# xujiabo/SCREAM

Measured on AMD Instinct MI355X. Metric: registration pairs/sec, higher is better.
Workload: dtype f32; 1 GPU; BASELINE configs[1]: synthetic 3DMatch_test-like pairs, voxel 0.0625 m, ~5k points/cloud, batch-of-pairs=32 per GPU, A1-A10 per pair (forward 6+6 layers d_model 256, 1-NN thresh 0.1, Kabsch, RE/TE), random-init weights seed 0; lanes=1, steps_in_flight=2, parallelism=dp1 (pairs sharded, metric-row all-gather), rccl_ranks=1, gemm_backend=h2

## Files before the change

include/scream_hip.h:

```cpp
#ifndef SCREAM_HIP_H
#define SCREAM_HIP_H

#include <stdint.h>

#ifdef __cplusplus
extern "C" {
#endif

#define SCREAM_ROW_TILE 128
#define SCREAM_D_MODEL 256
#define SCREAM_NHEAD 8
#define SCREAM_HEAD_DIM 32
#define SCREAM_KV_CHUNK 256

#define SCREAM_EINVAL (-1)
#define SCREAM_EUNSUPPORTED (-2)

enum {
    SCREAM_EPI_NONE = 0,
    SCREAM_EPI_ELU1 = 1,
    SCREAM_EPI_RELU = 2,
    SCREAM_EPI_BIAS_RELU = 3,
    SCREAM_EPI_RES_LN = 4,
    SCREAM_EPI_QKV = 5
};

#define SCREAM_LAYOUT_A_FRAG 1
#define SCREAM_LAYOUT_C_FRAG 2
int scream_act_layout(const float* src, float* dst, int64_t M, int32_t to_fragment, void* stream);

const char* scream_version(void);
int scream_abi_version(void);

int scream_gemm_f32(const float* A, int64_t lda, const float* W, float* C, int64_t ldc,
                    int64_t M, int32_t N, int32_t K, int32_t epilogue, int32_t n_act,
                    const float* bias, const float* residual, int64_t ldr,
                    const float* gamma, const float* beta, void* stream);

int scream_gemm_qkv_f32(const float* A, int64_t lda, const float* W, float* Q, int64_t ldq, int64_t M,
                        int32_t N, int32_t K, int32_t n_q, const int32_t* tile_cloud,
                        const int32_t* cloud_row0, const int32_t* cloud_len, int64_t row_base,
                        float* kv_partial, void* stream);
int scream_kv_finalize(const float* kv_partial, const int32_t* cloud_row0, const int32_t* cloud_len,
                       int64_t row_base, int32_t cloud_begin, int32_t n_kv, float* kv_out, void* stream);

#define SCREAM_SPLIT_H1 1
#define SCREAM_SPLIT_H2 2
#define SCREAM_SPLIT_BF3 3
int scream_pack_w_split(const float* W, int32_t N, int32_t K, int32_t split, int32_t w_exp, void* W_packed,
                        void* stream);
int scream_gemm_split_f32(const float* A, int64_t lda, const void* W_packed, float* C, int64_t ldc, int64_t M,
                          int32_t N, int32_t K, int32_t epilogue, int32_t n_act, const float* bias,
                          const float* residual, int64_t ldr, const float* gamma, const float* beta,
                          int32_t layout, int32_t split, int32_t a_exp, int32_t w_exp, void* stream);
int scream_gemm_qkv_split_f32(const float* A, int64_t lda, const void* W_packed, float* Q, int64_t ldq,
                              int64_t M, int32_t N, int32_t K, int32_t n_q, const int32_t* tile_cloud,
                              const int32_t* cloud_row0, const int32_t* cloud_len, int64_t row_base,
                              float* kv_partial, int32_t layout, int32_t split, int32_t a_exp, int32_t w_exp,
                              int32_t k_exp, int32_t v_exp, void* stream);

int64_t scream_proj_image_bytes(int32_t N, int32_t split);
int scream_pack_proj(const float* W, int32_t N, int32_t n_q, int32_t split, int32_t w_exp, void* proj_image, void* stream);
int scream_proj_qkv_f32(const float* x, const void* proj_image, float* Q, int64_t M, int32_t N, int32_t n_q,
                        const int32_t* tile_cloud, const int32_t* cloud_row0, const int32_t* cloud_len,
                        int64_t row_base, float* kv_partial, int32_t split, int32_t a_exp, int32_t w_exp, int32_t k_exp,
                        int32_t v_exp, void* stream);

typedef struct {
    int32_t e_att, e_wm, e_m1, e_w1, e_h, e_w2;
    int32_t e_y, e_wq;
    int32_t e_x;
    int32_t e_q;
} scream_tail_exps_t;
int64_t scream_tail_image_bytes(int32_t split, int32_t with_next_q);
int64_t scream_kv_image_bytes(void);
int scream_pack_tail(const float* Wm, const float* W1, const float* W2, const float* Wq_next, int32_t q_first, int32_t split,
                     const scream_tail_exps_t* exps, void* tail_image, void* stream);
int scream_kv_finalize_image(const float* kv_partial, const int32_t* cloud_row0, const int32_t* cloud_len,
                          int64_t row_base, int32_t cloud_begin, int32_t n_kv, void* kv_image, int32_t n_layers,
                          int64_t partial_layer_stride, int64_t image_layer_stride, int32_t split, void* stream);
int scream_layer_tail_f32(const float* Q, const void* kv_image, const int32_t* tile_cloud,
                          int32_t kv_cloud_offset, const int32_t* cloud_len, const float* x,
                          const void* tail_image, const float* g1, const float* b1, const float* g2,
                          const float* b2, float* y, float* q_next, int64_t M, int32_t split,
                          const scream_tail_exps_t* exps, void* stream);

int scream_pe_embed_ln(const float* xyz, const int32_t* tile_cloud, const float* center,
                       const float* dim_t, const float* emb_w, const float* emb_b,
                       const float* gamma, const float* beta, float* feats, int64_t rows,
                       void* stream);
int scream_pe_embed_ln_frag(const float* xyz, const int32_t* tile_cloud, const float* center,
                            const float* dim_t, const float* emb_w, const float* emb_b,
                            const float* gamma, const float* beta, float* feats, int64_t rows,
                            void* stream);

int scream_kv_reduce(const float* Kf, const float* Vf, int64_t ld, int64_t row_base,
                     const int32_t* cloud_row0, const int32_t* cloud_len, int32_t cloud_begin,
                     int32_t n_kv, int32_t max_chunks, float* partial, float* kv_out, void* stream);

int scream_attn_apply(const float* Qf, int64_t ldq, const float* kv, const int32_t* tile_cloud,
                      int32_t kv_cloud_offset, const int32_t* cloud_len, float* out, int64_t ldo,
                      int64_t rows, void* stream);

int scream_coor_head(const float* X, const float* W, const float* b, float* out, int64_t rows,
                     void* stream);

typedef struct {
    const float* wqkv;
    const float* wq;
    const float* wkv;
    const float* wm;
    const float* w1;
    const float* w2;
    const float* g1; const float* b1;
    const float* g2; const float* b2;
    const void* tail;
    int32_t e_xq, e_xkv, e_wqkv, e_wq, e_wkv, e_wm_g, e_w1_g, e_w2_g;
    int32_t e_k, e_v;
    scream_tail_exps_t tail_exps;
    int32_t tail_next_q;
    const void* proj;
    int32_t tail_q_first;
    const void* proj_kv;
} scream_layer_t;

typedef struct {
    int32_t n_self;
    int32_t n_cross;
    const float* dim_t;
    const float* emb_w; const float* emb_b;
    const float* pre_g; const float* pre_b;
    const scream_layer_t* layers_host;
    const float* c0_w; const float* c0_b;
    const float* c2_w; const float* c2_b;
    const float* c4_w; const float* c4_b;
    const scream_layer_t* stem_tgt_layers_host;
    int32_t gemm_split;
    int32_t e_c0x, e_c0w, e_c2x, e_c2w;
    const float* wkv_cross;
    int32_t e_wkv_cross, e_k_cross, e_v_cross;
    const void* proj_cross;
} scream_model_t;

typedef struct {
    int32_t n_pairs;
    int64_t rows_src;
    int64_t rows_total;
    int32_t max_chunks;
    const float* xyz;
    const float* center;
    const int32_t* tile_cloud;
    const int32_t* cloud_row0;
    const int32_t* cloud_len;
} scream_batch_t;

int64_t scream_forward_workspace_bytes(int64_t rows_src, int64_t rows_total, int32_t n_pairs,
                                       int32_t max_chunks, int32_t fused_tail, int32_t n_cross_batched);

int scream_forward(const scream_model_t* model, const scream_batch_t* batch, void* workspace,
                   int64_t workspace_bytes, float* src_pred, float* feats_out, void* trace,
                   void* stream);

void* scream_trace_create(int32_t capacity);
void scream_trace_destroy(void* trace);
int scream_trace_reset(void* trace);
int scream_trace_read(void* trace, int32_t max_records, float* ms, int32_t* kind, int64_t* m,
                      int32_t* n, int32_t* k);
int scream_trace_read_starts(void* trace, int32_t max_records, float* start_ms);

int scream_nn_search(const float* query, const float* ref, const int32_t* q_row0,
                     const int32_t* q_len, const int32_t* r_row0, const int32_t* r_len,
                     const float* s, int32_t n_pairs, int32_t max_q_len, int32_t max_r_len,
                     int64_t q_rows_total, int64_t r_rows_total, float thresh, float* ref_prep,
                     uint64_t* keys, int32_t* idx, float* dmin, uint8_t* valid, void* stream);

int scream_square_distance(const float* src, const float* dst, float* out, int32_t B, int32_t N,
                           int32_t M, void* stream);

int scream_kabsch_corr(const float* src, const float* ref, const int32_t* src_row0,
                       const int32_t* src_len, const int32_t* ref_row0, const int32_t* idx,
                       const uint8_t* valid, const float* s, const float* c, int32_t n_pairs,
                       float* T_out, int32_t* n_corr, void* stream);

int scream_rigid_transform_3d(const float* A, const float* B, const float* w,
                              float weight_threshold, int32_t bs, int32_t K, float* T_out,
                              void* stream);

int scream_transformation_error(const float* T_pred, const float* T_gt, int32_t n, float* re,
                                float* te, void* stream);

int scream_point_loss(const float* src_pred, const float* src, const int32_t* src_row0, const int32_t* src_len,
                      const float* rot, const float* trans, int32_t n_pairs, float* loss, void* stream);

int64_t scream_icp_workspace_bytes(int64_t src_rows_total, int64_t ref_rows_total, int32_t n_pairs);
int scream_icp_p2p_range(const float* src, const float* ref, const int32_t* src_row0, const int32_t* src_len,
                         const int32_t* ref_row0, const int32_t* ref_len, const float* s, const float* c,
                         int32_t n_pairs, int32_t max_src_len, int32_t max_ref_len, int64_t src_rows_total,
                         int64_t ref_rows_total, float max_corr_dist, int32_t max_iter, float rel_fitness,
                         float rel_rmse, float* T, float* fitness_rmse, int32_t* iters, int32_t it_begin, int32_t it_end,
                         int32_t* done_flags, void* workspace, int64_t workspace_bytes, void* stream);
int scream_icp_p2p(const float* src, const float* ref, const int32_t* src_row0, const int32_t* src_len,
                   const int32_t* ref_row0, const int32_t* ref_len, const float* s, const float* c,
                   int32_t n_pairs, int32_t max_src_len, int32_t max_ref_len, int64_t src_rows_total,
                   int64_t ref_rows_total, float max_corr_dist, int32_t max_iter, float rel_fitness,
                   float rel_rmse, float* T, float* fitness_rmse, int32_t* iters, void* workspace,
                   int64_t workspace_bytes, void* stream);

int64_t scream_wgrad_workspace_bytes(int64_t rows, int32_t N, int32_t K);
int scream_gemm_wgrad_f32(const float* dY, int64_t ldy, const float* X, int64_t ldx, int64_t rows, int32_t N,
                          int32_t K, float* dW, int32_t accumulate, float* colsum, void* workspace,
                          int64_t workspace_bytes, void* stream);
int64_t scream_wgrad_split_workspace_bytes(int64_t rows, int32_t N, int32_t K);
int scream_gemm_wgrad_split_f32(const float* dY, int64_t ldy, const float* X, int64_t ldx, int64_t rows, int32_t N,
                                int32_t K, float* dW, int32_t accumulate, float* colsum, int32_t split, void* workspace,
                                int64_t workspace_bytes, void* stream);
int scream_ln_fwd(const float* a, const float* b, const float* gamma, const float* beta, float* y, float* mean,
                  float* rstd, int64_t rows, void* stream);
int64_t scream_ln_bwd_workspace_bytes(int64_t rows);
int scream_ln_bwd(const float* dy, const float* a, const float* b, const float* mean, const float* rstd,
                  const float* gamma, float* dz, float* dsum, float* dgamma, float* dbeta, int32_t accumulate,
                  int64_t rows, void* workspace, int64_t workspace_bytes, void* stream);
int64_t scream_attn_bwd_workspace_bytes(int32_t n_q_clouds, int32_t max_chunks);
int scream_attn_bwd(const float* Qf, int64_t ldq, int64_t q_rows, int64_t q_row_base, const float* O,
                    const float* dO, const float* Kf, const float* Vf, int64_t ldkv, int64_t kv_rows,
                    int64_t kv_row_base, const float* kv, const int32_t* tile_cloud, const int32_t* cloud_row0,
                    const int32_t* cloud_len, int32_t q_cloud_begin, int32_t n_q_clouds, int32_t kv_cloud_offset,
                    int32_t max_chunks, float* dq, int64_t lddq, float* dk, float* dv, int64_t lddkv,
                    void* workspace, int64_t workspace_bytes, void* stream);
int scream_relu_bwd(float* dy, const float* y, int64_t n, void* stream);
int scream_add_f32(float* y, const float* x, int64_t n, void* stream);
int scream_transpose_f32(const float* in, int32_t R, int32_t C, float* out, void* stream);
int scream_coor_head_bwd(const float* dout, const float* W, const float* H, float* dH, int64_t rows, void* stream);
int64_t scream_grad3_workspace_bytes(int64_t rows);
int scream_grad3(const float* w, const float* s, const float* center, const int32_t* tile_cloud, int64_t rows,
                 float* dW, int32_t transpose_w, float* col_w, float* col_s, int32_t accumulate, void* workspace,
                 int64_t workspace_bytes, void* stream);
int scream_pe_embed(const float* xyz, const int32_t* tile_cloud, const float* center, const float* dim_t,
                    const float* emb_w, const float* emb_b, float* z, int64_t rows, void* stream);

int64_t scream_render_workspace_bytes(int32_t n_pairs, int32_t n_views, int32_t w, int64_t src_rows_total);
int scream_render_depth(const float* src, const int32_t* s_row0, const int32_t* s_len, const float* tgt,
                        const int32_t* t_row0, const int32_t* t_len, int32_t n_pairs, int32_t max_s_len, int32_t max_t_len,
                        int64_t src_rows_total, const float* rot, int32_t n_views, int32_t w, float rho, float* imgs,
                        int32_t* argmax, void* workspace, int64_t workspace_bytes, void* stream);
int scream_render_depth_bwd(const float* src, const int32_t* s_row0, const int32_t* s_len, int32_t n_pairs, int32_t max_s_len,
                            int64_t src_rows_total, const float* rot, int32_t n_views, int32_t w, float rho,
                            const float* dimgs, const int32_t* argmax, void* workspace, int64_t workspace_bytes, float* dsrc,
                            void* stream);

#ifdef __cplusplus
}
#endif
#endif
```

scream_amd/_lib.py:

```python
from __future__ import annotations

import ctypes as C
import os
from typing import Optional

_HERE = os.path.dirname(os.path.abspath(__file__))
LIB_PATH = os.environ.get("SCREAM_LIB") or os.path.join(_HERE, "libscream_hip.so")
ABI_VERSION = 19

c_f32p = C.POINTER(C.c_float)
c_i32p = C.POINTER(C.c_int32)
c_u8p = C.POINTER(C.c_uint8)
c_u64p = C.POINTER(C.c_uint64)


SPLIT_H1, SPLIT_H2, SPLIT_BF3 = 1, 2, 3


class TailExpsT(C.Structure):
    _fields_ = [(n, C.c_int32) for n in ("e_att", "e_wm", "e_m1", "e_w1", "e_h", "e_w2", "e_y", "e_wq", "e_x", "e_q")]


class LayerT(C.Structure):
    _fields_ = ([(n, C.c_void_p) for n in ("wqkv", "wq", "wkv", "wm", "w1", "w2", "g1", "b1", "g2", "b2", "tail")] +
                [(n, C.c_int32) for n in ("e_xq", "e_xkv", "e_wqkv", "e_wq", "e_wkv", "e_wm_g", "e_w1_g", "e_w2_g", "e_k", "e_v")] +
                [("tail_exps", TailExpsT), ("tail_next_q", C.c_int32), ("proj", C.c_void_p), ("tail_q_first", C.c_int32), ("proj_kv", C.c_void_p)])


class ModelT(C.Structure):
    _fields_ = [("n_self", C.c_int32), ("n_cross", C.c_int32), ("dim_t", C.c_void_p), ("emb_w", C.c_void_p),
                ("emb_b", C.c_void_p), ("pre_g", C.c_void_p), ("pre_b", C.c_void_p),
                ("layers_host", C.POINTER(LayerT)), ("c0_w", C.c_void_p), ("c0_b", C.c_void_p),
                ("c2_w", C.c_void_p), ("c2_b", C.c_void_p), ("c4_w", C.c_void_p), ("c4_b", C.c_void_p),
                ("stem_tgt_layers_host", C.POINTER(LayerT)), ("gemm_split", C.c_int32),
                ("e_c0x", C.c_int32), ("e_c0w", C.c_int32), ("e_c2x", C.c_int32), ("e_c2w", C.c_int32),
                ("wkv_cross", C.c_void_p), ("e_wkv_cross", C.c_int32), ("e_k_cross", C.c_int32), ("e_v_cross", C.c_int32),
                ("proj_cross", C.c_void_p)]


class BatchT(C.Structure):
    _fields_ = [("n_pairs", C.c_int32), ("rows_src", C.c_int64), ("rows_total", C.c_int64),
                ("max_chunks", C.c_int32), ("xyz", C.c_void_p), ("center", C.c_void_p),
                ("tile_cloud", C.c_void_p), ("cloud_row0", C.c_void_p), ("cloud_len", C.c_void_p)]


V, I32, I64, F32 = C.c_void_p, C.c_int32, C.c_int64, C.c_float
SIGNATURES = {
    "scream_version": (C.c_char_p, []),
    "scream_abi_version": (C.c_int, []),
    "scream_gemm_f32": (C.c_int, [V, I64, V, V, I64, I64, I32, I32, I32, I32, V, V, I64, V, V, V]),
    "scream_gemm_qkv_f32": (C.c_int, [V, I64, V, V, I64, I64, I32, I32, I32, V, V, V, I64, V, V]),
    "scream_kv_finalize": (C.c_int, [V, V, V, I64, I32, I32, V, V]),
    "scream_pack_w_split": (C.c_int, [V, I32, I32, I32, I32, V, V]),
    "scream_gemm_split_f32": (C.c_int, [V, I64, V, V, I64, I64, I32, I32, I32, I32, V, V, I64, V, V, I32, I32, I32, I32, V]),
    "scream_gemm_qkv_split_f32": (C.c_int, [V, I64, V, V, I64, I64, I32, I32, I32, V, V, V, I64, V, I32, I32, I32, I32, I32, I32, V]),
    "scream_proj_image_bytes": (C.c_int64, [I32, I32]),
    "scream_pack_proj": (C.c_int, [V, I32, I32, I32, I32, V, V]),
    "scream_proj_qkv_f32": (C.c_int, [V, V, V, I64, I32, I32, V, V, V, I64, V, I32, I32, I32, I32, I32, V]),
    "scream_tail_image_bytes": (C.c_int64, [I32, I32]),
    "scream_kv_image_bytes": (C.c_int64, []),
    "scream_pack_tail": (C.c_int, [V, V, V, V, I32, I32, C.POINTER(TailExpsT), V, V]),
    "scream_kv_finalize_image": (C.c_int, [V, V, V, I64, I32, I32, V, I32, I64, I64, I32, V]),
    "scream_layer_tail_f32": (C.c_int, [V, V, V, I32, V, V, V, V, V, V, V, V, V, I64, I32, C.POINTER(TailExpsT), V]),
    "scream_act_layout": (C.c_int, [V, V, I64, I32, V]),
    "scream_pe_embed_ln": (C.c_int, [V, V, V, V, V, V, V, V, V, I64, V]),
    "scream_pe_embed_ln_frag": (C.c_int, [V, V, V, V, V, V, V, V, V, I64, V]),
    "scream_kv_reduce": (C.c_int, [V, V, I64, I64, V, V, I32, I32, I32, V, V, V]),
    "scream_attn_apply": (C.c_int, [V, I64, V, V, I32, V, V, I64, I64, V]),
    "scream_coor_head": (C.c_int, [V, V, V, V, I64, V]),
    "scream_forward_workspace_bytes": (C.c_int64, [I64, I64, I32, I32, I32, I32]),
    "scream_forward": (C.c_int, [C.POINTER(ModelT), C.POINTER(BatchT), V, I64, V, V, V, V]),
    "scream_trace_create": (C.c_void_p, [I32]),
    "scream_trace_destroy": (None, [V]),
    "scream_trace_reset": (C.c_int, [V]),
    "scream_trace_read": (C.c_int, [V, I32, V, V, V, V, V]),
    "scream_trace_read_starts": (C.c_int, [V, I32, V]),
    "scream_nn_search": (C.c_int, [V, V, V, V, V, V, V, I32, I32, I32, I64, I64, F32, V, V, V, V, V, V]),
    "scream_square_distance": (C.c_int, [V, V, V, I32, I32, I32, V]),
    "scream_kabsch_corr": (C.c_int, [V, V, V, V, V, V, V, V, V, I32, V, V, V]),
    "scream_rigid_transform_3d": (C.c_int, [V, V, V, F32, I32, I32, V, V]),
    "scream_transformation_error": (C.c_int, [V, V, I32, V, V, V]),
    "scream_point_loss": (C.c_int, [V, V, V, V, V, V, I32, V, V]),
    "scream_icp_workspace_bytes": (C.c_int64, [I64, I64, I32]),
    "scream_icp_p2p": (C.c_int, [V, V, V, V, V, V, V, V, I32, I32, I32, I64, I64, F32, I32, F32, F32, V, V, V, V, I64, V]),
    "scream_wgrad_workspace_bytes": (C.c_int64, [I64, I32, I32]),
    "scream_gemm_wgrad_f32": (C.c_int, [V, I64, V, I64, I64, I32, I32, V, I32, V, V, I64, V]),
    "scream_wgrad_split_workspace_bytes": (C.c_int64, [I64, I32, I32]),
    "scream_gemm_wgrad_split_f32": (C.c_int, [V, I64, V, I64, I64, I32, I32, V, I32, V, I32, V, I64, V]),
    "scream_ln_fwd": (C.c_int, [V, V, V, V, V, V, V, I64, V]),
    "scream_ln_bwd_workspace_bytes": (C.c_int64, [I64]),
    "scream_ln_bwd": (C.c_int, [V, V, V, V, V, V, V, V, V, V, I32, I64, V, I64, V]),
    "scream_attn_bwd_workspace_bytes": (C.c_int64, [I32, I32]),
    "scream_attn_bwd": (C.c_int, [V, I64, I64, I64, V, V, V, V, I64, I64, I64, V, V, V, V, I32, I32, I32, I32, V, I64, V, V, I64,
                                  V, I64, V]),
    "scream_relu_bwd": (C.c_int, [V, V, I64, V]),
    "scream_add_f32": (C.c_int, [V, V, I64, V]),
    "scream_transpose_f32": (C.c_int, [V, I32, I32, V, V]),
    "scream_coor_head_bwd": (C.c_int, [V, V, V, V, I64, V]),
    "scream_grad3_workspace_bytes": (C.c_int64, [I64]),
    "scream_grad3": (C.c_int, [V, V, V, V, I64, V, I32, V, V, I32, V, I64, V]),
    "scream_pe_embed": (C.c_int, [V, V, V, V, V, V, V, I64, V]),
    "scream_icp_p2p_range": (C.c_int, [V, V, V, V, V, V, V, V, I32, I32, I32, I64, I64, F32, I32, F32, F32, V, V, V, I32, I32, V, V, I64, V]),
    "scream_render_workspace_bytes": (C.c_int64, [I32, I32, I32, I64]),
    "scream_render_depth": (C.c_int, [V, V, V, V, V, V, I32, I32, I32, I64, V, I32, I32, F32, V, V, V, I64, V]),
    "scream_render_depth_bwd": (C.c_int, [V, V, V, I32, I32, I64, V, I32, I32, F32, V, V, V, I64, V, V]),
}

_lib: Optional[C.CDLL] = None


class ScreamHipError(RuntimeError):
    pass


def load() -> C.CDLL:
    global _lib
    if _lib is not None:
        return _lib
    if os.environ.get("SCREAM_NO_BUILD", "0") != "1" and not os.environ.get("SCREAM_LIB"):
        try:
            from . import build as _build
            _build.build()
        except Exception as e:
            if not os.path.exists(LIB_PATH):
                raise ScreamHipError("libscream_hip.so is missing and could not be built: %s" % e) from e
    if not os.path.exists(LIB_PATH):
        raise ScreamHipError("libscream_hip.so not found at %s (run `python -m scream_amd.build`)" % LIB_PATH)
    lib = C.CDLL(LIB_PATH)
    for name, (res, args) in SIGNATURES.items():
        try:
            fn = getattr(lib, name)
        except AttributeError as e:
            raise ScreamHipError("libscream_hip.so does not export %s" % name) from e
        fn.restype = res
        fn.argtypes = args
    if lib.scream_abi_version() != ABI_VERSION:
        raise ScreamHipError("libscream_hip.so ABI %d != binding ABI %d" % (lib.scream_abi_version(), ABI_VERSION))
    _lib = lib
    return lib


def check(rc: int, what: str) -> None:
    if rc == 0:
        return
    if rc == -1:
        raise ScreamHipError("%s: invalid argument (SCREAM_EINVAL)" % what)
    if rc == -2:
        raise ScreamHipError("%s: unsupported shape (SCREAM_EUNSUPPORTED)" % what)
    raise ScreamHipError("%s: HIP error %d" % (what, rc))
```

scream_amd/build.py:

```python
from __future__ import annotations

import os
import shutil
import subprocess
import sys
from concurrent.futures import ThreadPoolExecutor

HERE = os.path.dirname(os.path.abspath(__file__))
CSRC = os.path.join(HERE, "csrc")
LIB = os.path.join(HERE, "libscream_hip.so")
ARCH = "gfx950"

SOURCES = {
    "gemm_f32.hip": [],
    "gemm_split.hip": [],
    "proj_ring.hip": ["-mllvm", "-amdgpu-mfma-vgpr-form=1"],
    "tail_split.hip": ["-ffp-contract=off"],
    "embed.hip": [],
    "attention.hip": [],
    "backward.hip": [],
    "forward.hip": [],
    "nn_search.hip": ["-ffp-contract=off"],
    "kabsch.hip": ["-ffp-contract=off"],
    "icp_grid.hip": ["-ffp-contract=off"],
    "render.hip": ["-ffp-contract=off"],
}
EXTRA_DEFINES = {}
for _item in filter(None, os.environ.get("SCREAM_HIPCC_EXTRA", "").split(";")):
    EXTRA_DEFINES[_item.split(":")[0]] = _item.split(":", 1)[1].split(",")
ASM_LOADS = ("gemm_split.hip", "tail_split.hip", "proj_ring.hip")
NO_SCRATCH = {"proj_ring.hip": ("proj_ring_kernel",), "tail_split.hip": ("tail_kernelINS_7SplitH2", "tail_kernelINS_7SplitH1")}


def _hipcc() -> str:
    exe = shutil.which("hipcc") or "/opt/rocm/bin/hipcc"
    if not os.path.exists(exe):
        raise RuntimeError("hipcc not found: cannot build libscream_hip.so")
    return exe


def _stale() -> bool:
    if not os.path.exists(LIB):
        return True
    t = os.path.getmtime(LIB)
    deps = [os.path.join(CSRC, f) for f in os.listdir(CSRC)] + [os.path.join(HERE, "..", "include", "scream_hip.h"), __file__]
    return any(os.path.getmtime(d) > t for d in deps)


def build(force: bool = False, verbose: bool = False, out: str = None) -> str:
    global LIB
    if out:
        LIB, force = out, True
    if not force and not _stale():
        return LIB
    hipcc = _hipcc()
    objdir = os.path.join(HERE, "build")
    os.makedirs(objdir, exist_ok=True)
    common = [hipcc, "-O3", "-std=c++17", "--offload-arch=" + ARCH, "-fPIC", "-Wall", "-Wno-unused-function"]

    def compile_one(item):
        src, extra = item
        extra = extra + EXTRA_DEFINES.get(src, [])
        obj = os.path.join(objdir, src.replace(".hip", ".o"))
        cmd = common + extra + ["-c", os.path.join(CSRC, src), "-o", obj]
        r = subprocess.run(cmd, capture_output=True, text=True)
        if r.returncode != 0:
            raise RuntimeError("hipcc failed for %s:\n%s\n%s" % (src, " ".join(cmd), r.stderr))
        if verbose and r.stderr.strip():
            print(r.stderr, file=sys.stderr)
        return obj

    def verify_one(src):
        sys.path.insert(0, os.path.join(HERE, "..", "tools"))
        import asm_inflight_check as chk
        asm = os.path.join(objdir, src.replace(".hip", ".s"))
        cmd = common + SOURCES[src] + EXTRA_DEFINES.get(src, []) + ["-S", "--cuda-device-only", os.path.join(CSRC, src), "-o", asm]
        r = subprocess.run(cmd, capture_output=True, text=True)
        if r.returncode != 0:
            raise RuntimeError("hipcc -S failed for %s:\n%s" % (src, r.stderr))
        for name, body in chk.kernels(asm):
            if any(k in name for k in NO_SCRATCH.get(src, ())) and any(("scratch_" in l or "buffer_store" in l) for l in body):
                raise RuntimeError("%s: %s spills registers to scratch (this hipcc allocates registers differently from the one the "
                                   "kernel was written with)" % (src, name))
            bad = chk.check_kernel(name, body)
            if bad:
                raise RuntimeError("%s: %s touches a register whose asm load is still in flight (%d places, first: %s); "
                                   "this hipcc allocates registers differently from the one the kernels were written with"
                                   % (src, name, len(bad), bad[0][1]))
            sd = chk.check_store_data_hazard(name, body)
            if sd:
                raise RuntimeError("%s: %s overwrites the data of a wide store %d wait states behind it (%s ; %s)"
                                   % (src, name, sd[0][3], sd[0][1], sd[0][2]))
            mh = chk.check_mfma_asm_read_hazard(name, body)
            if mh:
                raise RuntimeError("%s: %s reads a matrix-instruction result with an asm vector instruction %d wait states behind it "
                                   "(%s ; %s)" % (src, name, mh[0][3], mh[0][2], mh[0][1]))
            hz = chk.check_scalar_base_hazard(name, body)
            if hz:
                raise RuntimeError("%s: %s uses a scalar base %d wait states after a VALU write of it (%s -> %s)"
                                   % (src, name, hz[0][3], hz[0][2], hz[0][1]))
        return src

    with ThreadPoolExecutor(max_workers=4) as ex:
        checks = [ex.submit(verify_one, src) for src in ASM_LOADS] if os.environ.get("SCREAM_BUILD_VERIFY", "1") != "0" else []
        objs = list(ex.map(compile_one, SOURCES.items()))
        for c in checks:
            c.result()
    cmd = [hipcc, "--offload-arch=" + ARCH, "-shared", "-fPIC", "-o", LIB + ".tmp"] + objs
    r = subprocess.run(cmd, capture_output=True, text=True)
    if r.returncode != 0:
        raise RuntimeError("link failed:\n%s" % r.stderr)
    os.replace(LIB + ".tmp", LIB)
    return LIB


if __name__ == "__main__":
    print(build(force="--force" in sys.argv, verbose=True))
```

scream_amd/csrc/forward.hip:

```cpp
#include <vector>

#include "common.h"

namespace {

constexpr int D = SCREAM_D_MODEL;
constexpr int KV_ELEMS = (SCREAM_HEAD_DIM + 1) * SCREAM_HEAD_DIM;

struct Workspace {
    float *x0, *x1, *q, *att, *m1, *hid, *kvp, *kv;
    char* kvimg;
    float* kvp_cross;
    char* kvimg_cross;
    int64_t kvp_cross_stride, kvimg_cross_stride;
    int64_t bytes;
};

Workspace carve(void* base, int64_t rows_src, int64_t rows_total, int32_t n_pairs, int32_t max_chunks, bool fused, int32_t n_cross_batched) {
    Workspace w;
    float* p = reinterpret_cast<float*>(base);
    auto take = [&](int64_t n) {
        float* r = p;
        p += (n + 63) / 64 * 64;
        return r;
    };
    w.x0 = take(rows_total * D);
    w.x1 = take(rows_total * D);
    w.q = take(rows_total * D);
    w.att = fused ? nullptr : take(rows_total * D);
    w.m1 = fused ? nullptr : take(rows_total * D);
    w.hid = fused ? nullptr : take(rows_total * 4 * D);
    w.kvp = take(rows_total / SCREAM_ROW_TILE * SCREAM_NHEAD * KV_ELEMS);
    w.kv = take((int64_t)2 * n_pairs * SCREAM_NHEAD * KV_ELEMS);
    w.kvimg = reinterpret_cast<char*>(take((int64_t)2 * n_pairs * scream_kv_image_bytes() / 4));
    w.kvp_cross_stride = (rows_total - rows_src) / SCREAM_ROW_TILE * SCREAM_NHEAD * KV_ELEMS;
    w.kvimg_cross_stride = (int64_t)n_pairs * scream_kv_image_bytes();
    w.kvp_cross = take(n_cross_batched * w.kvp_cross_stride);
    w.kvimg_cross = reinterpret_cast<char*>(take(n_cross_batched * w.kvimg_cross_stride / 4));
    w.bytes = (p - reinterpret_cast<float*>(base)) * (int64_t)sizeof(float);
    return w;
}

struct Trace {
    std::vector<hipEvent_t> ev;
    std::vector<int32_t> kind, n, k;
    std::vector<int64_t> m;
    int count = 0;
    int capacity = 0;
};

struct Scope {
    Trace* t;
    int slot = -1;
    hipStream_t st;
    Scope(Trace* t_, int kind, int64_t m, int n, int k, void* stream) : t(t_), st(as_stream(stream)) {
        if (!t || t->count >= t->capacity) return;
        slot = t->count++;
        t->kind[slot] = kind;
        t->m[slot] = m;
        t->n[slot] = n;
        t->k[slot] = k;
        (void)hipEventRecord(t->ev[2 * slot], st);
    }
    ~Scope() {
        if (slot >= 0) (void)hipEventRecord(t->ev[2 * slot + 1], st);
    }
};

#define TRY(call)                 \
    do {                          \
        int rc_ = (call);         \
        if (rc_ != 0) return rc_; \
    } while (0)

enum { TR_TAIL_FUSED = 7, TR_EMBED = 100, TR_KV_REDUCE = 101, TR_ATTN_APPLY = 102, TR_COOR_HEAD = 103 };

struct Ctx {
    void* st;
    Trace* tr;
    int split;
    bool frag;
};

int gemm(const Ctx& c, const float* A, int64_t lda, const float* W, float* C, int64_t ldc, int64_t M, int N, int K,
         int epi, int n_act, const float* bias, const float* res, const float* g, const float* b, int a_exp, int w_exp,
         int layout = 0) {
    Scope sc(c.tr, epi, M, N, K, c.st);
    if (c.split)
        return scream_gemm_split_f32(A, lda, W, C, ldc, M, N, K, epi, n_act, bias, res, D, g, b, layout, c.split, a_exp, w_exp, c.st);
    return scream_gemm_f32(A, lda, W, C, ldc, M, N, K, epi, n_act, bias, res, D, g, b, c.st);
}

int gemm_qkv(const Ctx& c, const float* A, const float* W, const void* proj, float* Q, int64_t M, int N, int n_q, const scream_batch_t& b,
             int64_t row_base, float* kvp, int a_exp, int w_exp, int k_exp, int v_exp) {
    Scope sc(c.tr, 5, M, N, D, c.st);
    if (proj && c.frag && (c.split == SCREAM_SPLIT_H2 || c.split == SCREAM_SPLIT_H1))
        return scream_proj_qkv_f32(A, proj, Q, M, N, n_q, b.tile_cloud, b.cloud_row0, b.cloud_len, row_base, kvp, c.split, a_exp, w_exp,
                                   k_exp, v_exp, c.st);
    if (c.split)
        return scream_gemm_qkv_split_f32(A, D, W, Q, D, M, N, D, n_q, b.tile_cloud, b.cloud_row0, b.cloud_len, row_base, kvp,
                                         c.frag ? (SCREAM_LAYOUT_A_FRAG | (n_q ? SCREAM_LAYOUT_C_FRAG : 0)) : 0, c.split, a_exp,
                                         w_exp, k_exp, v_exp, c.st);
    return scream_gemm_qkv_f32(A, D, W, Q, D, M, N, D, n_q, b.tile_cloud, b.cloud_row0, b.cloud_len, row_base, kvp, c.st);
}

int mha_tail(const Ctx& c, const scream_layer_t& L, const Workspace& w, const float* x, float* y, int64_t row0,
             int64_t rows) {
    float* att = w.att + row0 * D;
    float* m1 = w.m1 + row0 * D;
    float* hid = w.hid + row0 * 4 * D;
    const scream_tail_exps_t& e = L.tail_exps;
    TRY(gemm(c, att, D, L.wm, m1, D, rows, D, D, SCREAM_EPI_RES_LN, 0, nullptr, x, L.g1, L.b1, e.e_att, L.e_wm_g));
    TRY(gemm(c, m1, D, L.w1, hid, 4 * D, rows, 4 * D, D, SCREAM_EPI_RELU, 0, nullptr, nullptr, nullptr, nullptr, e.e_m1, L.e_w1_g));
    TRY(gemm(c, hid, 4 * D, L.w2, y, D, rows, D, 4 * D, SCREAM_EPI_RES_LN, 0, nullptr, x, L.g2, L.b2, e.e_h, L.e_w2_g));
    return 0;
}

int mha_self(const Ctx& c, const scream_layer_t& L, const scream_batch_t& b, const Workspace& w, const float* x,
             float* y, int64_t row0, int64_t rows, int32_t cloud_begin, int32_t n_clouds, bool next_q = false) {
    const float* xr = x + row0 * D;
    float* qr = w.q + row0 * D;
    float* kvp = w.kvp + row0 / SCREAM_ROW_TILE * SCREAM_NHEAD * KV_ELEMS;
    const bool qf = c.frag && L.tail_q_first;
    if (qf) TRY(gemm_qkv(c, xr, L.wkv, L.proj_kv, nullptr, rows, 2 * D, 0, b, row0, kvp, L.e_xkv, L.e_wkv, L.e_k, L.e_v));
    else TRY(gemm_qkv(c, xr, L.wqkv, L.proj, qr, rows, 3 * D, D, b, row0, kvp, L.e_xq, L.e_wqkv, L.e_k, L.e_v));
    if (c.frag) {
        {
            Scope sc(c.tr, TR_KV_REDUCE, rows, 0, 0, c.st);
            TRY(scream_kv_finalize_image(kvp, b.cloud_row0, b.cloud_len, row0, cloud_begin, n_clouds, w.kvimg, 1, 0, 0, c.split, c.st));
        }
        Scope sc(c.tr, TR_TAIL_FUSED, rows, ((next_q || qf) ? 10 : 9) * D, D, c.st);
        return scream_layer_tail_f32(qf ? nullptr : qr, w.kvimg, b.tile_cloud + row0 / SCREAM_ROW_TILE, 0, b.cloud_len, xr, L.tail, L.g1,
                                     L.b1, L.g2, L.b2, y + row0 * D, (next_q && !qf) ? qr : nullptr, rows, c.split, &L.tail_exps, c.st);
    }
    {
        Scope sc(c.tr, TR_KV_REDUCE, rows, 0, 0, c.st);
        TRY(scream_kv_finalize(kvp, b.cloud_row0, b.cloud_len, row0, cloud_begin, n_clouds, w.kv, c.st));
    }
    {
        Scope sc(c.tr, TR_ATTN_APPLY, rows, 0, 0, c.st);
        TRY(scream_attn_apply(qr, D, w.kv, b.tile_cloud + row0 / SCREAM_ROW_TILE, 0, b.cloud_len, w.att + row0 * D, D, rows,
                              c.st));
    }
    return mha_tail(c, L, w, xr, y + row0 * D, row0, rows);
}

int cross_kv_all(const Ctx& c, const scream_model_t& m, const scream_batch_t& b, const Workspace& w, const float* x_tgt) {
    const int64_t rs = b.rows_src, rt = b.rows_total - b.rows_src;
    const scream_layer_t& L0 = m.layers_host[m.n_self + 1];
    TRY(gemm_qkv(c, x_tgt, m.wkv_cross, m.proj_cross, nullptr, rt, 2 * D * m.n_cross, 0, b, rs, w.kvp_cross, L0.e_xkv, m.e_wkv_cross, m.e_k_cross,
                 m.e_v_cross));
    Scope sc(c.tr, TR_KV_REDUCE, rt, 0, 0, c.st);
    return scream_kv_finalize_image(w.kvp_cross, b.cloud_row0, b.cloud_len, rs, b.n_pairs, b.n_pairs,
                                 w.kvimg_cross - (int64_t)b.n_pairs * scream_kv_image_bytes(), m.n_cross, w.kvp_cross_stride,
                                 w.kvimg_cross_stride, c.split, c.st);
}

int mha_cross(const Ctx& c, const scream_layer_t& L, const scream_batch_t& b, const Workspace& w, const float* x_src,
              const float* x_tgt, float* y, const char* kvimg_layer, bool q_ready = false) {
    const int64_t rs = b.rows_src, rt = b.rows_total - b.rows_src;
    const bool qf = c.frag && L.tail_q_first;
    if (!q_ready && !qf)
        TRY(gemm(c, x_src, D, L.wq, w.q, D, rs, D, D, SCREAM_EPI_ELU1, D, nullptr, nullptr, nullptr, nullptr, L.e_xq, L.e_wq,
                 c.frag ? (SCREAM_LAYOUT_A_FRAG | SCREAM_LAYOUT_C_FRAG) : 0));
    if (c.frag && kvimg_layer) {
        Scope sc(c.tr, TR_TAIL_FUSED, rs, (qf ? 10 : 9) * D, D, c.st);
        return scream_layer_tail_f32(qf ? nullptr : w.q, kvimg_layer, b.tile_cloud, 0, b.cloud_len + b.n_pairs, x_src, L.tail, L.g1, L.b1, L.g2,
                                     L.b2, y, nullptr, rs, c.split, &L.tail_exps, c.st);
    }
    TRY(gemm_qkv(c, x_tgt, L.wkv, nullptr, nullptr, rt, 2 * D, 0, b, rs, w.kvp, L.e_xkv, L.e_wkv, L.e_k, L.e_v));
    if (c.frag) {
        {
            Scope sc(c.tr, TR_KV_REDUCE, rt, 0, 0, c.st);
            TRY(scream_kv_finalize_image(w.kvp, b.cloud_row0, b.cloud_len, rs, b.n_pairs, b.n_pairs, w.kvimg, 1, 0, 0, c.split, c.st));
        }
        Scope sc(c.tr, TR_TAIL_FUSED, rs, (qf ? 10 : 9) * D, D, c.st);
        return scream_layer_tail_f32(qf ? nullptr : w.q, w.kvimg, b.tile_cloud, b.n_pairs, b.cloud_len, x_src, L.tail, L.g1, L.b1, L.g2, L.b2,
                                     y, nullptr, rs, c.split, &L.tail_exps, c.st);
    }
    {
        Scope sc(c.tr, TR_KV_REDUCE, rt, 0, 0, c.st);
        TRY(scream_kv_finalize(w.kvp, b.cloud_row0, b.cloud_len, rs, b.n_pairs, b.n_pairs, w.kv, c.st));
    }
    {
        Scope sc(c.tr, TR_ATTN_APPLY, rs, 0, 0, c.st);
        TRY(scream_attn_apply(w.q, D, w.kv, b.tile_cloud, b.n_pairs, b.cloud_len, w.att, D, rs, c.st));
    }
    return mha_tail(c, L, w, x_src, y, 0, rs);
}

}

extern "C" const char* scream_version(void) { return "scream_hip gfx950 abi19"; }
extern "C" int scream_abi_version(void) { return 19; }

extern "C" void* scream_trace_create(int32_t capacity) {
    if (capacity <= 0) return nullptr;
    Trace* t = new Trace();
    t->capacity = capacity;
    t->ev.resize(2 * (size_t)capacity);
    t->kind.resize(capacity);
    t->n.resize(capacity);
    t->k.resize(capacity);
    t->m.resize(capacity);
    for (auto& e : t->ev) {
        if (hipEventCreate(&e) != hipSuccess) {
            delete t;
            return nullptr;
        }
    }
    return t;
}

extern "C" void scream_trace_destroy(void* trace) {
    Trace* t = reinterpret_cast<Trace*>(trace);
    if (!t) return;
    for (auto& e : t->ev) (void)hipEventDestroy(e);
    delete t;
}

extern "C" int scream_trace_reset(void* trace) {
    SCREAM_REQUIRE(trace, SCREAM_EINVAL);
    reinterpret_cast<Trace*>(trace)->count = 0;
    return 0;
}

extern "C" int scream_trace_read(void* trace, int32_t max_records, float* ms, int32_t* kind, int64_t* m, int32_t* n,
                                 int32_t* k) {
    SCREAM_REQUIRE(trace && ms && kind && m && n && k && max_records >= 0, SCREAM_EINVAL);
    Trace* t = reinterpret_cast<Trace*>(trace);
    const int cnt = t->count < max_records ? t->count : max_records;
    for (int i = 0; i < cnt; ++i) {
        if (hipEventElapsedTime(&ms[i], t->ev[2 * i], t->ev[2 * i + 1]) != hipSuccess) return SCREAM_EINVAL;
        kind[i] = t->kind[i];
        m[i] = t->m[i];
        n[i] = t->n[i];
        k[i] = t->k[i];
    }
    return cnt;
}

extern "C" int scream_trace_read_starts(void* trace, int32_t max_records, float* start_ms) {
    SCREAM_REQUIRE(trace && start_ms && max_records >= 0, SCREAM_EINVAL);
    Trace* t = reinterpret_cast<Trace*>(trace);
    const int cnt = t->count < max_records ? t->count : max_records;
    for (int i = 0; i < cnt; ++i)
        if (hipEventElapsedTime(&start_ms[i], t->ev[0], t->ev[2 * i]) != hipSuccess) return SCREAM_EINVAL;
    return cnt;
}

extern "C" int64_t scream_forward_workspace_bytes(int64_t rows_src, int64_t rows_total, int32_t n_pairs,
                                                  int32_t max_chunks, int32_t fused_tail, int32_t n_cross_batched) {
    if (rows_src < 0 || rows_total < rows_src || n_pairs < 0 || max_chunks < 0 || n_cross_batched < 0) return SCREAM_EINVAL;
    return carve(nullptr, rows_src, rows_total, n_pairs, max_chunks, fused_tail != 0, n_cross_batched).bytes + 256;
}

extern "C" int scream_forward(const scream_model_t* model, const scream_batch_t* batch, void* workspace,
                              int64_t workspace_bytes, float* src_pred, float* feats_out, void* trace, void* stream) {
    SCREAM_REQUIRE(model && batch && workspace && src_pred, SCREAM_EINVAL);
    const scream_model_t& m = *model;
    const scream_batch_t& b = *batch;
    SCREAM_REQUIRE(m.layers_host && m.n_self >= 0 && m.n_cross >= 0 &&
                       (m.gemm_split == 0 || m.gemm_split == SCREAM_SPLIT_H1 || m.gemm_split == SCREAM_SPLIT_H2 || m.gemm_split == SCREAM_SPLIT_BF3),
                   SCREAM_EINVAL);
    SCREAM_REQUIRE(b.n_pairs > 0 && b.rows_src > 0 && b.rows_total > b.rows_src && b.max_chunks > 0, SCREAM_EINVAL);
    SCREAM_REQUIRE(b.rows_src % SCREAM_ROW_TILE == 0 && b.rows_total % SCREAM_ROW_TILE == 0, SCREAM_EUNSUPPORTED);
    SCREAM_REQUIRE(b.xyz && b.center && b.tile_cloud && b.cloud_row0 && b.cloud_len, SCREAM_EINVAL);
    int n_layers = m.n_self + 2 * m.n_cross, n_tail = 0;
    for (int i = 0; i < n_layers; ++i) n_tail += m.layers_host[i].tail != nullptr;
    if (m.stem_tgt_layers_host)
        for (int i = 0; i < m.n_self; ++i, ++n_layers) n_tail += m.stem_tgt_layers_host[i].tail != nullptr;
    SCREAM_REQUIRE(n_tail == 0 || (n_tail == n_layers && m.gemm_split != 0), SCREAM_EINVAL);
    uintptr_t base = (reinterpret_cast<uintptr_t>(workspace) + 255) & ~(uintptr_t)255;
    const bool batched_kv = n_tail > 0 && m.wkv_cross != nullptr && m.n_cross > 0;
    const Workspace w = carve(reinterpret_cast<void*>(base), b.rows_src, b.rows_total, b.n_pairs, b.max_chunks, n_tail > 0,
                              batched_kv ? m.n_cross : 0);
    SCREAM_REQUIRE((int64_t)(base - reinterpret_cast<uintptr_t>(workspace)) + w.bytes <= workspace_bytes, SCREAM_EINVAL);
    const Ctx c{stream, reinterpret_cast<Trace*>(trace), m.gemm_split, n_tail > 0};

    const int64_t rs = b.rows_src, ra = b.rows_total;
    {
        Scope sc(c.tr, TR_EMBED, ra, 0, 0, stream);
        if (c.frag)
            TRY(scream_pe_embed_ln_frag(b.xyz, b.tile_cloud, b.center, m.dim_t, m.emb_w, m.emb_b, m.pre_g, m.pre_b, w.x0, ra, stream));
        else
            TRY(scream_pe_embed_ln(b.xyz, b.tile_cloud, b.center, m.dim_t, m.emb_w, m.emb_b, m.pre_g, m.pre_b, w.x0, ra, stream));
    }
    float* cur = w.x0;
    float* nxt = w.x1;
    for (int i = 0; i < m.n_self; ++i) {
        if (!m.stem_tgt_layers_host) {
            TRY(mha_self(c, m.layers_host[i], b, w, cur, nxt, 0, ra, 0, 2 * b.n_pairs));
        } else {
            TRY(mha_self(c, m.layers_host[i], b, w, cur, nxt, 0, rs, 0, b.n_pairs));
            TRY(mha_self(c, m.stem_tgt_layers_host[i], b, w, cur, nxt, rs, ra - rs, b.n_pairs, b.n_pairs));
        }
        float* t = cur;
        cur = nxt;
        nxt = t;
    }
    const float* x_tgt = cur + rs * D;
    if (batched_kv) TRY(cross_kv_all(c, m, b, w, x_tgt));
    for (int i = 0; i < 2 * m.n_cross; ++i) {
        const scream_layer_t& L = m.layers_host[m.n_self + i];
        if (i % 2 == 0) {
            TRY(mha_self(c, L, b, w, cur, nxt, 0, rs, 0, b.n_pairs, c.frag && L.tail_next_q));
        } else {
            const bool q_ready = c.frag && m.layers_host[m.n_self + i - 1].tail_next_q;
            TRY(mha_cross(c, L, b, w, cur, x_tgt, nxt, batched_kv ? w.kvimg_cross + (i / 2) * w.kvimg_cross_stride : nullptr, q_ready));
        }
        float* t = cur;
        cur = nxt;
        nxt = t;
    }
    float* c_mid = c.frag ? w.q : w.m1;
    float* c_out = c.frag ? nxt : w.att;
    TRY(gemm(c, cur, D, m.c0_w, c_mid, D, rs, D, D, SCREAM_EPI_BIAS_RELU, 0, m.c0_b, nullptr, nullptr, nullptr, m.e_c0x, m.e_c0w,
             c.frag ? SCREAM_LAYOUT_A_FRAG : 0));
    TRY(gemm(c, c_mid, D, m.c2_w, c_out, D, rs, D, D, SCREAM_EPI_BIAS_RELU, 0, m.c2_b, nullptr, nullptr, nullptr, m.e_c2x, m.e_c2w));
    {
        Scope sc(c.tr, TR_COOR_HEAD, rs, 0, 0, stream);
        TRY(scream_coor_head(c_out, m.c4_w, m.c4_b, src_pred, rs, stream));
    }
    if (feats_out && c.frag) {
        TRY(scream_act_layout(cur, feats_out, rs, 0, stream));
    } else if (feats_out) {
        hipError_t e = hipMemcpyAsync(feats_out, cur, (size_t)rs * D * sizeof(float), hipMemcpyDeviceToDevice,
                                      as_stream(stream));
        if (e != hipSuccess) return (int)e;
    }
    return 0;
}
```

scream_amd/csrc/tail_split.hip:

```cpp
#include <type_traits>

#include "ring.h"

#ifndef T_MIX
#define T_MIX 1
#endif
#ifndef T_RIDE0
#define T_RIDE0 3
#endif
#ifndef T_STASH
#define T_STASH 3
#endif
#ifndef T_NT
#define T_NT 7
#endif
#ifndef T_QF_DUMP
#define T_QF_DUMP 0
#endif
#ifndef T_QF_DBG
#define T_QF_DBG 0
#endif
#ifndef T_DEFER_H2
#define T_DEFER_H2 2
#endif

#ifdef T_STAMPS
#define T_STAMP_SLOTS 24
__device__ long long t_stamps[256 * 4 * T_STAMP_SLOTS];
extern "C" int scream_tail_stamps_read(long long* host) {
    return (int)hipMemcpyFromSymbol(host, HIP_SYMBOL(t_stamps), sizeof(long long) * 256 * 4 * T_STAMP_SLOTS);
}
#define TSTAMP(slot)                                                                                 \
    do {                                                                                             \
        if (stamp_on && lane == 0) t_stamps[((int)blockIdx.x * 4 + wave) * T_STAMP_SLOTS + (slot)] = __builtin_amdgcn_s_memtime(); \
    } while (0)
#define TMARK(i) marks[i] = (unsigned)__builtin_amdgcn_s_memtime()
#define TMARK2(i, prev) do { marks[prev] = marks[i]; TMARK(i); } while (0)
#define TMARKS_FLUSH()                                                                               \
    do {                                                                                             \
        if (stamp_on && lane == 0)                                                                   \
            for (int i_ = 0; i_ < 16; ++i_) t_stamps[((int)blockIdx.x * 4 + wave) * T_STAMP_SLOTS + 8 + i_] = marks[i_]; \
    } while (0)
#else
#define TSTAMP(slot) do {} while (0)
#define TMARK(i) do {} while (0)
#define TMARK2(i, prev) do {} while (0)
#define TMARKS_FLUSH() do {} while (0)
#endif

namespace {

constexpr int TAIL_STAGES = 72;
constexpr int NEXT_Q_STAGES = 8;
constexpr int KV_PLANES_BYTES = 8 * 3 * 2 * 1024;
constexpr int KV_IMAGE_BYTES = KV_PLANES_BYTES + 8 * 32 * 4;

constexpr int KV_H2_HEAD_BYTES = 2 * 2 * 1024;
constexpr int KV_H2_SCALE_OFF = 8 * KV_H2_HEAD_BYTES;
#ifndef T_APPLY_H2
#define T_APPLY_H2 1
#endif

struct HeadOps {
    f32x4 kv[6];
    f32x4 ks[4];
    f32x4 sc;
};

struct TailScales {
    float s_att;
    int e_q;
    int e_att;
    float c1;
    float eps1;
    float s_m1;
    float ch;
    float c2;
    float eps2;
    float s_y;
    float cq;
    float s_x;
    float cqf;
};

__device__ __forceinline__ constexpr int xadd_slot(int h, int g, int nd) {
    int n = 0;
    for (int c = 15 - nd; c >= 8; --c) {
        if ((c >> 1) == h - 1) continue;
        if (c == g) return n < 4 ? n : -1;
        ++n;
    }
    return -1;
}

template <class SP, bool NQ, bool QF>
__global__ __launch_bounds__(TT, 1) void tail_kernel(const float* __restrict__ Q,
                                                     const char* __restrict__ kvimg,
                                                     const int32_t* __restrict__ tile_cloud, int kv_cloud_offset,
                                                     const int32_t* __restrict__ cloud_len,
                                                     const float* __restrict__ xres,
                                                     const char* __restrict__ Wimg,
                                                     const float* __restrict__ g1, const float* __restrict__ b1,
                                                     const float* __restrict__ g2, const float* __restrict__ b2,
                                                     float* __restrict__ y,
                                                     float* q_next,
                                                     int n_tiles, TailScales sc) {
    static_assert(!NQ || SP::SCALED, "the next-layer query projection is built for the fp16 splits");
    static_assert(!QF || (SP::SCALED && !NQ), "the in-kernel query projection is built for the fp16 splits and replaces the next-layer one");
    constexpr int N_STAGES = TAIL_STAGES + ((NQ || QF) ? NEXT_Q_STAGES : 0);
    typedef typename SP::vec V;
    constexpr int NP = SP::NP;
    constexpr int STAGE = stage_bytes<SP>();
    constexpr int PIECES = wave_pieces<SP>();
    constexpr bool APPLY_H2 = SP::SCALED && T_APPLY_H2;
#ifdef T_NV_MERGE
    constexpr int NV_MERGE = T_NV_MERGE;
#else
    constexpr int NV_MERGE = SP::NPROD >= 6 ? 6 : 8;
#endif
    constexpr int ND = SP::NPROD >= 6 ? 1 : T_DEFER_H2;
    constexpr int NG = 16 - ND;
    constexpr int NSTASH = (NP == 2 && !QF) ? T_STASH : 0;
    __shared__ __attribute__((aligned(16))) char smem[T_SLOTS * STAGE + 4096 + NSTASH * 16384];
    const int tid = threadIdx.x, lane = tid & 63;
    const int wave = __builtin_amdgcn_readfirstlane(tid >> 6);
    const int half = lane >> 5;
    float* lnp = reinterpret_cast<float*>(smem + T_SLOTS * STAGE);
    f32x4* stash = reinterpret_cast<f32x4*>(smem + T_SLOTS * STAGE + 4096 + wave * (NSTASH * 4096)) + lane;
    lnp[tid] = SP::SCALED ? g1[tid] * sc.s_m1 : g1[tid];
    lnp[256 + tid] = SP::SCALED ? b1[tid] * sc.s_m1 : b1[tid];
    lnp[512 + tid] = g2[tid];
    lnp[768 + tid] = b2[tid];
    const float eps1 = SP::SCALED ? sc.eps1 : 1e-5f, eps2 = SP::SCALED ? sc.eps2 : 1e-5f;
    const unsigned v_lane16 = lane * 16, v_half16 = half * 16;
    auto dma_piece = [&](unsigned q, int u) {
        if ((T_ABLATE & 1) && q >= 2) return;
        const unsigned src = q % (unsigned)N_STAGES, slot = q % (unsigned)T_SLOTS;
        const char* sbase = Wimg + (size_t)src * STAGE + (wave * PIECES + (u & ~3)) * 1024;
        dma_1k(sbase + v_lane16, smem + slot * STAGE + (wave * PIECES + (u & ~3)) * 1024, u & 3);
    };
    unsigned q = 0;
#pragma unroll
    for (int u = 0; u < PIECES; ++u) dma_piece(0, u);
#pragma unroll
    for (int u = 0; u < PIECES; ++u) dma_piece(1, u);

    auto seg_base = [&](const float* base, int64_t grp, int seg) { return base + grp + seg * 1024; };
    auto req_q = [&](f32x4 (&qb)[4], int64_t grp, int h) {
        if (T_ABLATE & (16 | 32)) return;
        if (T_ABLATE & 2048) grp = (int64_t)wave * 32 * SCREAM_D_MODEL;
        ld_asm4<1024, (T_NT & 1) != 0>(qb, seg_base(Q, grp, h), v_lane16);
    };
    auto req_head = [&](HeadOps& o, const char* kvc, int h) {
        if (T_ABLATE & (16 | 256)) return;
        f32x4 (&kv4)[4] = reinterpret_cast<f32x4 (&)[4]>(o.kv[0]);
        if (APPLY_H2) {
            ld_asm4<1024>(kv4, kvc + h * KV_H2_HEAD_BYTES, v_lane16);
            asm volatile("global_load_dwordx4 %0, %1, %2" : "=v"(o.sc) : "v"(v_half16), "s"(kvc + KV_H2_SCALE_OFF + 32 * h));
        } else {
            const char* kp = kvc + h * (3 * 2 * 1024);
            ld_asm4<1024>(kv4, kp, v_lane16);
            ld_asm2k(o.kv[4], o.kv[5], kp + 4 * 1024, v_lane16);
        }
        ld_asm4<32>(o.ks, kvc + KV_PLANES_BYTES + 128 * h, v_half16);
    };
    auto req_x = [&](f32x4 (&xs)[4], int64_t grp, int blk, auto second) {
        if (T_ABLATE & (16 | 64)) return;
        if (T_ABLATE & 2048) grp = (int64_t)wave * 32 * SCREAM_D_MODEL;
        ld_asm4<1024, (T_NT & (decltype(second)::value ? 4 : 8)) != 0>(xs, seg_base(xres, grp, blk), v_lane16);
    };
    auto pin_head = [&](HeadOps& o) {
#pragma unroll
        for (int a = 0; a < 4; ++a) pin(o.ks[a]);
#pragma unroll
        for (int f = 0; f < (APPLY_H2 ? 4 : 6); ++f) pin(o.kv[f]);
        if (APPLY_H2) pin(o.sc);
    };
    auto add_x4 = [&](f32x16& t, const f32x4 (&xs)[4], int a, float c) {
#pragma unroll
        for (int k = 0; k < 4; ++k) {
            const float xv = (T_ABLATE & 16) ? 1.0f : xs[a][k];
            t[4 * a + k] = SP::SCALED ? __builtin_fmaf(xv, c, t[4 * a + k]) : t[4 * a + k] + xv;
        }
    };
    auto pin_x = [&](f32x4 (&xs)[4]) {
#pragma unroll
        for (int a = 0; a < 4; ++a) pin(xs[a]);
    };
    auto add_x = [&](f32x16& t, const f32x4 (&xs)[4], float c) {
#pragma unroll
        for (int a = 0; a < 4; ++a) add_x4(t, xs, a, c);
    };

    HeadOps op;
    f32x4 qA[4], qB[4];
    f32x4 xs[4], xs2[4];
    V apA[2][NP], apB[2][NP];
    f32x16 aT;
    bf16x8 qp[2][3];
    f16x8 qph[2][2];
    float Zs = 0.f;
    int tq = 0;

    auto apply_qscale = [&](const f32x4 (&qb)[4]) {
        float m = 0.f;
#pragma unroll
        for (int a = 0; a < 4; ++a)
#pragma unroll
            for (int k = 0; k < 4; ++k) m = fmaxf(m, qb[a][k]);
        m = fmaxf(m, __shfl_xor(m, 32));
        const int hb = (int)(__float_as_uint(op.sc[0]) >> 23);
        tq = min(max(14 - ((int)(__float_as_uint(m) >> 23) - 127), sc.e_q), min(127, sc.e_att + hb - 1));
    };
    auto apply_qsplit = [&](f32x4 (&qb)[4], int tile_tag, int s2) {
        f32x4 lo = qb[2 * s2], hi = qb[2 * s2 + 1];
        if (T_ABLATE & 16) lo = hi = f32x4{(float)lane, 1.0f, 0.5f, (float)tile_tag};
        if (APPLY_H2) split8s<SplitH2>(lo, hi, __uint_as_float((uint32_t)(tq + 127) << 23), qph[s2]);
        else split8<SplitBf3>(lo, hi, qp[s2]);
    };
    auto apply_mfma = [&](int s2) {
        if (APPLY_H2) {
            f16x8 w[2];
#pragma unroll
            for (int p = 0; p < 2; ++p) w[p] = __builtin_bit_cast(f16x8, op.kv[p * 2 + s2]);
            mfma_group<SplitH2, -1>(aT, w, qph[s2], s2 == 0);
        } else {
            bf16x8 w[3];
#pragma unroll
            for (int p = 0; p < 3; ++p) w[p] = __builtin_bit_cast(bf16x8, op.kv[p * 2 + s2]);
            mfma_group<SplitBf3, -1>(aT, w, qp[s2], s2 == 0);
        }
    };
    auto apply_z = [&](f32x4 (&qb)[4]) {
        float zp = 0.f;
#pragma unroll
        for (int a = 0; a < 4; ++a)
#pragma unroll
            for (int k = 0; k < 4; ++k) zp += qb[a][k] * op.ks[a][k];
        zp += __shfl_xor(zp, 32);
        Zs = 1.0f / (zp + 1e-6f);
        if (APPLY_H2) Zs *= __uint_as_float((uint32_t)(sc.e_att - tq + (int)(__float_as_uint(op.sc[0]) >> 23)) << 23);
        else if (SP::SCALED) Zs *= sc.s_att;
    };
    auto apply_split_pair = [&](int k, V (&ap)[2][NP], float S) {
        const int s2 = k >> 2, j = (2 * k) & 7;
        if constexpr (SP::SCALED && (T_MIX & 2)) {
            SP::split2s((aT[2 * k] * Zs) * S, (aT[2 * k + 1] * Zs) * S, 1.0f, j, ap[s2]);
        } else {
#pragma unroll
            for (int e = 0; e < 2; ++e) SP::split1((aT[2 * k + e] * Zs) * S, j + e, ap[s2]);
        }
    };
    auto apply_ride = [&](f32x4 (&qb)[4], int g, V (&ap)[2][NP], float S, int tile_tag) {
        if (g == 0 && APPLY_H2) apply_qscale(qb);
        if (g == 0) apply_qsplit(qb, tile_tag, 0);
        if (g == 1) apply_qsplit(qb, tile_tag, 1);
        if (g == 1) apply_mfma(0);
        if (g == 2) apply_mfma(1);
        if (g == 3) apply_z(qb);
        if (g >= 4 && g < 12) apply_split_pair(g - 4, ap, S);
    };

    V xp[QF ? 16 : 1][NP];
    f32x4 qall[QF ? 8 : 1][4];
    f32x16 hqf[2];
    auto elu_q = [&](int k, const f32x16& h, f32x4 (&dst)[4]) {
#pragma unroll
        for (int e = 0; e < 2; ++e) {
            const int i = 2 * k + e;
            dst[i >> 2][i & 3] = elu1(h[i] * sc.cqf);
        }
    };

    float dbg6[8] = {0.f, 0.f, 0.f, 0.f, 0.f, 0.f, 0.f, 0.f};
    auto xsum = [&](const V (&ap)[2][NP]) {
        unsigned c = 0;
#pragma unroll
        for (int s2 = 0; s2 < 2; ++s2)
#pragma unroll
            for (int pl = 0; pl < NP; ++pl) {
                const f32x4 w = __builtin_bit_cast(f32x4, ap[s2][pl]);
#pragma unroll
                for (int k = 0; k < 4; ++k) c ^= __builtin_bit_cast(unsigned, w[k]);
            }
        return __builtin_bit_cast(float, (c & 0x007fffffu) | 0x3f800000u);
    };
    auto asum = [&](const f32x16 (&a)[8]) {
        unsigned c = 0;
#pragma unroll
        for (int b = 0; b < 8; ++b)
#pragma unroll
            for (int e = 0; e < 16; ++e) c ^= __builtin_bit_cast(unsigned, a[b][e]);
        return __builtin_bit_cast(float, (c & 0x007fffffu) | 0x3f800000u);
    };
    int tile = blockIdx.x;
    int64_t grp = ((int64_t)tile * 128 + wave * 32) * SCREAM_D_MODEL;
    const char* kvc = nullptr;
    float S = 1.f;
    if (tile < n_tiles) {
        const int cl = tile_cloud[tile] + kv_cloud_offset;
        kvc = kvimg + (size_t)cl * KV_IMAGE_BYTES;
        S = (float)cloud_len[cl];
    }
    if (!QF && tile < n_tiles) {
#pragma unroll
        for (int h = 0; h < 2; ++h) {
            req_q(qA, grp, h);
            req_head(op, kvc, h);
            VM_WAIT(0);
            pin_x(qA);
            pin_head(op);
#pragma unroll
            for (int g = 0; g < 12; ++g) apply_ride(qA, g, h == 0 ? apA : apB, S, tile);
        }
    }

#ifdef T_STAMPS
    int tile_no = 0;
#endif
    while (tile < n_tiles) {
#ifdef T_STAMPS
        const bool stamp_on = tile_no == 1;
        ++tile_no;
        unsigned marks[16] = {};
#endif
        TSTAMP(0);
        V wfd[ND][NP];
        f32x16 acc[8];
        const int tile_next = tile + (int)gridDim.x;
        const bool has_next = tile_next < n_tiles;
        const int64_t grp_next = ((int64_t)(has_next ? tile_next : tile) * 128 + wave * 32) * SCREAM_D_MODEL;
        const char* kvc_next = kvc;
        float S_next = 1.f;
        if (has_next) {
            const int cl = tile_cloud[tile_next] + kv_cloud_offset;
            kvc_next = kvimg + (size_t)cl * KV_IMAGE_BYTES;
            S_next = (float)cloud_len[cl];
        }

        auto stage_merge = [&](auto hh, V (&ap)[2][NP], V (&ap_next)[2][NP], f32x4 (&q_cons)[4], f32x4 (&q_req)[4], auto flush) {
            constexpr int h = decltype(hh)::value;
            constexpr bool RIDE = h >= 1 && h <= 6;
            if (h == 0 && !QF) { if (NQ) ring_barrier<0>(); else lds_only_barrier(); }
            else if (QF && (T_QF_DBG & 32) && h <= 1) ring_barrier<0>();
            else ring_barrier<PIECES>();
            TMARK(h);
            __builtin_amdgcn_sched_barrier(0);
            f32x4 (&x_prev)[4] = (h & 1) ? xs : xs2;
            f32x4 (&x_req)[4] = (h & 1) ? xs2 : xs;
            if (h > 0) {
                pin_x(x_prev);
                if (h - 1 < NSTASH) {
#pragma unroll
                    for (int a = 0; a < 4; ++a) stash[((h - 1) * 4 + a) * 64] = x_prev[a];
                }
                if (RIDE) {
                    pin_head(op);
                    pin_x(q_cons);
                }
            }
            __builtin_amdgcn_sched_barrier(0);
            req_x(x_req, grp, h, std::false_type{});
            if (!QF && h + 2 < 8) req_q(q_req, grp, h + 2);
            if (h == 0) req_head(op, kvc, 2);
            __builtin_amdgcn_sched_barrier(0);
            const char* wb = smem + (q % T_SLOTS) * STAGE + lane * 16;
            V wf[T_PF][NP];
#pragma unroll
            for (int g0 = 0; g0 < T_PF - 1; ++g0)
#pragma unroll
                for (int p = 0; p < NP; ++p) wf[g0][p] = ld_frag<V>(wb + (p * 16 + g0) * 1024);
            flush();
#pragma unroll
            for (int g = 0; g < NG; ++g) {
                if (g + T_PF - 1 < 16) {
#pragma unroll
                    for (int p = 0; p < NP; ++p)
                        (g + T_PF - 1 >= NG ? wfd[g + T_PF - 1 - NG][p] : wf[(g + T_PF - 1) % T_PF][p]) = ld_frag<V>(wb + (p * 16 + g + T_PF - 1) * 1024);
                }
                if (g == 4 && RIDE && h + 2 < 8) {
                    __builtin_amdgcn_sched_barrier(0);
                    req_head(op, kvc, h + 2);
                    __builtin_amdgcn_sched_barrier(0);
                }
                if (g >= 4 && g - 4 < PIECES) dma_piece(q + 2, g - 4);
                if (PIECES == 12 && g == 14) dma_piece(q + 2, 11);
                if (RIDE && !(T_ABLATE & 512)) apply_ride(q_cons, g, ap_next, S, tile);
                if (QF && h == 0 && g < 8) elu_q(g, hqf[1], qall[QF ? 7 : 0]);
                if (h > 0) {
                    const int pc = xadd_slot(h, g, ND);
                    if (pc >= 0 && !(T_ABLATE & 1024)) add_x4(acc[h > 0 ? h - 1 : 0], x_prev, pc, sc.c1);
                }
                mfma_group<SP, (h > 0 ? NV_MERGE : 0)>(acc[g >> 1], wf[g % T_PF], ap[g & 1], h == 0 && (g & 1) == 0);
            }
            ++q;
        };
        constexpr std::integral_constant<bool, true> yes{};
        constexpr std::integral_constant<bool, false> no{};
#define HEAD(n) std::integral_constant<int, n>{}
        auto flush_none = [&]() {};
        auto flush_acc7 = [&](V (&b)[2][NP], bool first) {
#pragma unroll
            for (int i = 0; i < ND; ++i) mfma_group<SP, -1>(acc[7], wfd[i], b[(NG + i) & 1], first && ((NG + i) & 1) == 0);
        };
        auto flush_mergeA = [&]() { flush_acc7(apA, false); };
        auto flush_mergeB = [&]() { flush_acc7(apB, false); };
        auto flush_mergeA0 = [&]() { flush_acc7(apA, true); };
        if constexpr (QF) {
            {
                f32x4 raw[8][4];
                const float* xg = xres + grp + lane * 4;
                if (T_QF_DBG & 256) VM_WAIT(0);
#pragma unroll
                for (int blk = 0; blk < 8; ++blk)
#pragma unroll
                    for (int a = 0; a < 4; ++a) raw[blk][a] = ld4(xg + (blk * 4 + a) * 256);
                VM_WAIT(0);
#pragma unroll
                for (int blk = 0; blk < 8; ++blk)
#pragma unroll
                    for (int s2 = 0; s2 < 2; ++s2) split8s<SP>(raw[blk][2 * s2], raw[blk][2 * s2 + 1], sc.s_x, xp[QF ? 2 * blk + s2 : 0]);
            }
            auto stage_qf = [&](auto jj) {
                constexpr int j = decltype(jj)::value;
                constexpr int RIDE = j >= 6 ? j - 6 : -1;
                constexpr bool RIDE6 = !(T_QF_DBG & (2 | 64)), RIDE7 = !(T_QF_DBG & (2 | 128));
                constexpr bool RIDE_ON = j == 6 ? RIDE6 : RIDE7;
                if (j == 0) { if (T_QF_DBG & 1) ring_barrier<0>(); else lds_only_barrier(); }
                else if ((T_QF_DBG & 8) && j >= 6) ring_barrier<0>();
                else if ((T_QF_DBG & 16) && j >= 1 && j <= 5) ring_barrier<0>();
                else ring_barrier<PIECES>();
                __builtin_amdgcn_sched_barrier(0);
                if (RIDE >= 0 && RIDE_ON) pin_head(op);
                __builtin_amdgcn_sched_barrier(0);
                if (j == 5 && RIDE6) req_head(op, kvc, 0);
                if (j == 6 && !RIDE6 && RIDE7) req_head(op, kvc, 1);
                __builtin_amdgcn_sched_barrier(0);
                const char* wb = smem + (q % T_SLOTS) * STAGE + lane * 16;
                V wf[T_PF][NP];
#pragma unroll
                for (int g0 = 0; g0 < T_PF - 1; ++g0)
#pragma unroll
                    for (int p = 0; p < NP; ++p) wf[g0][p] = ld_frag<V>(wb + (p * 16 + g0) * 1024);
                if (j > 0) {
#pragma unroll
                    for (int i = 0; i < ND; ++i) mfma_group<SP, -1>(hqf[(j + 1) & 1], wfd[i], xp[QF ? NG + i : 0]);
                }
#pragma unroll
                for (int g = 0; g < NG; ++g) {
                    if (g + T_PF - 1 < 16) {
#pragma unroll
                        for (int p = 0; p < NP; ++p)
                            (g + T_PF - 1 >= NG ? wfd[g + T_PF - 1 - NG][p] : wf[(g + T_PF - 1) % T_PF][p]) = ld_frag<V>(wb + (p * 16 + g + T_PF - 1) * 1024);
                    }
                    if (g == 4 && RIDE == 0 && RIDE6 && RIDE7) {
                        __builtin_amdgcn_sched_barrier(0);
                        req_head(op, kvc, 1);
                        __builtin_amdgcn_sched_barrier(0);
                    }
                    if (g >= 4 && g - 4 < PIECES) dma_piece(q + 2, g - 4);
                    if (j > 0 && g < 8) elu_q(g, hqf[(j + 1) & 1], qall[QF && j > 0 ? j - 1 : 0]);
                    if (RIDE >= 0 && RIDE_ON && !(T_ABLATE & 512)) apply_ride(qall[QF && RIDE >= 0 ? RIDE : 0], g, RIDE == 0 ? apA : apB, S, tile);
                    mfma_group<SP, 8>(hqf[j & 1], wf[g % T_PF], xp[QF ? g : 0], g == 0);
                }
                ++q;
            };
            stage_qf(HEAD(0)); stage_qf(HEAD(1)); stage_qf(HEAD(2)); stage_qf(HEAD(3));
            stage_qf(HEAD(4)); stage_qf(HEAD(5)); stage_qf(HEAD(6));
            stage_qf(HEAD(7));
            if (T_QF_DUMP == 6) {
                unsigned c = 0;
#pragma unroll
                for (int h = 0; h < 7; ++h)
#pragma unroll
                    for (int a = 0; a < 4; ++a)
#pragma unroll
                        for (int k = 0; k < 4; ++k) c ^= __builtin_bit_cast(unsigned, qall[QF ? h : 0][a][k]);
                dbg6[4] = __builtin_bit_cast(float, (c & 0x007fffffu) | 0x3f800000u);
            }
            if (T_QF_DBG & (2 | 64 | 128)) {
#pragma unroll
                for (int h = 0; h < 2; ++h) {
                    if (!(T_QF_DBG & 2) && !(T_QF_DBG & (h == 0 ? 64 : 128))) continue;
                    req_head(op, kvc, h);
                    VM_WAIT(0);
                    pin_head(op);
#pragma unroll
                    for (int g = 0; g < 12; ++g) apply_ride(qall[QF ? h : 0], g, h == 0 ? apA : apB, S, tile);
                }
            }
        }
        auto flush_q7 = [&]() {
#pragma unroll
            for (int i = 0; i < ND; ++i) mfma_group<SP, -1>(hqf[1], wfd[i], xp[QF ? NG + i : 0]);
        };
#define QC(h1, q_) qall[QF ? (h1) : 0]
        if constexpr (QF) {
            stage_merge(HEAD(0), apA, apB, QC(1, qB), QC(1, qA), flush_q7);
            stage_merge(HEAD(1), apB, apA, QC(2, qA), QC(2, qB), flush_mergeA0);
            stage_merge(HEAD(2), apA, apB, QC(3, qB), QC(3, qA), flush_mergeB);
            stage_merge(HEAD(3), apB, apA, QC(4, qA), QC(4, qB), flush_mergeA);
            stage_merge(HEAD(4), apA, apB, QC(5, qB), QC(5, qA), flush_mergeB);
            stage_merge(HEAD(5), apB, apA, QC(6, qA), QC(6, qB), flush_mergeA);
            stage_merge(HEAD(6), apA, apB, QC(7, qB), QC(7, qA), flush_mergeB);
            stage_merge(HEAD(7), apB, apA, QC(7, qA), QC(7, qB), flush_mergeA);
        } else {
        stage_merge(HEAD(0), apA, apB, qB, qA, flush_none);
        stage_merge(HEAD(1), apB, apA, qA, qB, flush_mergeA0);
        stage_merge(HEAD(2), apA, apB, qB, qA, flush_mergeB);
        stage_merge(HEAD(3), apB, apA, qA, qB, flush_mergeA);
        stage_merge(HEAD(4), apA, apB, qB, qA, flush_mergeB);
        stage_merge(HEAD(5), apB, apA, qA, qB, flush_mergeA);
        stage_merge(HEAD(6), apA, apB, qB, qA, flush_mergeB);
        stage_merge(HEAD(7), apB, apA, qA, qB, flush_mergeA);
        }
#undef QC
        flush_mergeB();
        vm_wait<PIECES>();
        pin_x(xs2);
        add_x(acc[7], xs2, sc.c1);

        TSTAMP(1);
#if T_QF_DUMP
        if (QF && T_QF_DUMP != 6 && (T_QF_DUMP < 4 || q_next)) {
            float* yd = (T_QF_DUMP < 4 ? y : q_next) + grp + lane * 4;
#pragma unroll
            for (int b = 0; b < 8; ++b)
#pragma unroll
                for (int a = 0; a < 4; ++a) {
                    f32x4 o;
#pragma unroll
                    for (int k = 0; k < 4; ++k) o[k] = (T_QF_DUMP & 1) ? qall[QF ? b : 0][a][k] : acc[b][4 * a + k];
                    *reinterpret_cast<f32x4*>(yd + (b * 4 + a) * 256) = o;
                }
        }
#endif
        V mp[16][NP];
        {
            float sum = 0.f;
#pragma unroll
            for (int b = 0; b < 8; ++b)
#pragma unroll
                for (int e = 0; e < 16; ++e) sum += acc[b][e];
            sum += __shfl_xor(sum, 32);
            const float mean = sum * (1.0f / 256.0f);
            float var = 0.f;
#pragma unroll
            for (int b = 0; b < 8; ++b)
#pragma unroll
                for (int e = 0; e < 16; ++e) {
                    acc[b][e] -= mean;
                    var += acc[b][e] * acc[b][e];
                }
            var += __shfl_xor(var, 32);
            const float rstd = 1.0f / sqrtf(var * (1.0f / 256.0f) + eps1);
            const float* gp = lnp + 4 * half;
            const float* bp = lnp + 256 + 4 * half;
#pragma unroll
            for (int b = 0; b < 8; ++b)
#pragma unroll
                for (int s2 = 0; s2 < 2; ++s2) {
                    f32x4 v[2];
#pragma unroll
                    for (int a2 = 0; a2 < 2; ++a2) {
                        const int a = 2 * s2 + a2;
                        const f32x4 g4 = ld4(gp + 32 * b + 8 * a), b4 = ld4(bp + 32 * b + 8 * a);
#pragma unroll
                        for (int k = 0; k < 4; ++k) v[a2][k] = acc[b][4 * a + k] * rstd * g4[k] + b4[k];
                    }
                    if (T_MIX & 2) split8s<SP>(v[0], v[1], 1.0f, mp[2 * b + s2]); else split8<SP>(v[0], v[1], mp[2 * b + s2]);
                }
        }

        TSTAMP(2);
        if (QF && T_QF_DUMP == 6) {
            unsigned c = 0;
#pragma unroll
            for (int i = 0; i < 16; ++i)
#pragma unroll
                for (int pl = 0; pl < NP; ++pl) {
                    const f32x4 w = __builtin_bit_cast(f32x4, mp[i][pl]);
#pragma unroll
                    for (int k = 0; k < 4; ++k) c ^= __builtin_bit_cast(unsigned, w[k]);
                }
            (void)c;
        }
        f32x16 hT;
        V hpA[2][NP], hpB[2][NP];
        auto split_pair = [&](int k, V (&hout)[2][NP]) {
            const int s2 = k >> 2, j = (2 * k) & 7;
            float x0, x1;
            if (T_MIX & 1) {
                asm("v_max_f32 %0, 0, %1" : "=v"(x0) : "v"(hT[2 * k]));
                asm("v_max_f32 %0, 0, %1" : "=v"(x1) : "v"(hT[2 * k + 1]));
            } else {
                x0 = fmaxf(hT[2 * k], 0.f);
                x1 = fmaxf(hT[2 * k + 1], 0.f);
            }
            if constexpr (SP::SCALED && (T_MIX & 1)) {
                SP::split2s(x0, x1, sc.ch, j, hout[s2]);
            } else if constexpr (SP::SCALED) {
                SP::split1(x0 * sc.ch, j, hout[s2]);
                SP::split1(x1 * sc.ch, j + 1, hout[s2]);
            } else {
                SP::split1(x0, j, hout[s2]);
                SP::split1(x1, j + 1, hout[s2]);
            }
        };
        auto stage_up = [&](auto first, auto xload, auto flush) {
            constexpr int XLOAD = decltype(xload)::value;
            if (decltype(first)::value) ring_barrier<0>(); else ring_barrier<PIECES>();
            TMARK2(8, 10);
            __builtin_amdgcn_sched_barrier(0);
            if (XLOAD >= 0 && XLOAD < NSTASH) {
#pragma unroll
                for (int a = 0; a < 4; ++a) xs[a] = stash[(XLOAD * 4 + a) * 64];
            } else if (XLOAD >= 0) req_x(xs, grp, XLOAD, std::true_type{});
            __builtin_amdgcn_sched_barrier(0);
            const char* wb = smem + (q % T_SLOTS) * STAGE + lane * 16;
            V wf[T_PF][NP];
#pragma unroll
            for (int g0 = 0; g0 < T_PF - 1; ++g0)
#pragma unroll
                for (int p = 0; p < NP; ++p) wf[g0][p] = ld_frag<V>(wb + (p * 16 + g0) * 1024);
            flush();
#pragma unroll
            for (int g = 0; g < NG; ++g) {
                if (g + T_PF - 1 < 16) {
#pragma unroll
                    for (int p = 0; p < NP; ++p)
                        (g + T_PF - 1 >= NG ? wfd[g + T_PF - 1 - NG][p] : wf[(g + T_PF - 1) % T_PF][p]) = ld_frag<V>(wb + (p * 16 + g + T_PF - 1) * 1024);
                }
                if (g < PIECES) dma_piece(q + 2, g);
                mfma_group<SP>(hT, wf[g % T_PF], mp[g], g == 0);
            }
            ++q;
        };
        auto stage_down = [&](V (&hin)[2][NP], V (&hout)[2][NP], auto with_split, auto xadd, auto ride, auto flush) {
            constexpr int XADD = decltype(xadd)::value;
            constexpr int RIDE = decltype(ride)::value;
#ifdef T_PROBE_NOBAR
            __builtin_amdgcn_s_waitcnt(0x0070 | (PIECES & 15) | ((PIECES >> 4) << 14));
#else
            ring_barrier<PIECES>();
#endif
            TMARK2(9, 11);
            __builtin_amdgcn_sched_barrier(0);
            if (XADD == 0) {
                pin_x(xs);
#pragma unroll
                for (int a = 0; a < 4; ++a)
#pragma unroll
                    for (int k = 0; k < 4; ++k) {
                        const float xv = (T_ABLATE & 16) ? 1.0f : xs[a][k];
                        acc[0][4 * a + k] = SP::SCALED ? xv * sc.c2 : xv;
                    }
            } else if (XADD > 0) {
                pin_x(xs);
                add_x(acc[XADD > 0 ? XADD : 0], xs, sc.c2);
            }
            if (RIDE == 2) {
                pin_head(op);
                pin_x(qA);
            }
            __builtin_amdgcn_sched_barrier(0);
            if (RIDE == 1) {
                req_q(qA, grp_next, 0);
                req_head(op, kvc_next, 0);
            }
            __builtin_amdgcn_sched_barrier(0);
            const char* wb = smem + (q % T_SLOTS) * STAGE + lane * 16;
            V wf[T_PF][NP];
#pragma unroll
            for (int g0 = 0; g0 < T_PF - 1; ++g0)
#pragma unroll
                for (int p = 0; p < NP; ++p) wf[g0][p] = ld_frag<V>(wb + (p * 16 + g0) * 1024);
            flush();
#pragma unroll
            for (int g = 0; g < NG; ++g) {
                if (g + T_PF - 1 < 16) {
#pragma unroll
                    for (int p = 0; p < NP; ++p)
                        (g + T_PF - 1 >= NG ? wfd[g + T_PF - 1 - NG][p] : wf[(g + T_PF - 1) % T_PF][p]) = ld_frag<V>(wb + (p * 16 + g + T_PF - 1) * 1024);
                }
                if (RIDE == 2 && g == 4) {
                    __builtin_amdgcn_sched_barrier(0);
                    req_q(qA, grp_next, 1);
                    req_head(op, kvc_next, 1);
                    __builtin_amdgcn_sched_barrier(0);
                }
                if (RIDE == 2) {
                    if (g >= 4 && g - 4 < PIECES) dma_piece(q + 2, g - 4);
                    if (PIECES == 12 && g == 14) dma_piece(q + 2, 11);
                } else {
                    if (g < PIECES) dma_piece(q + 2, g);
                }
                if (RIDE == 2) apply_ride(qA, g, apA, S_next, tile_next);
                if (decltype(with_split)::value && (ND == 1 ? (g & 1) == 0 : (g >= T_RIDE0 && g < T_RIDE0 + 8))) split_pair(ND == 1 ? g >> 1 : g - T_RIDE0, hout);
                mfma_group<SP>(acc[g >> 1], wf[g % T_PF], hin[g & 1], XADD == 0 && g >= 2 && (g & 1) == 0);
            }
            ++q;
        };
        constexpr std::integral_constant<int, -1> none{};
        constexpr std::integral_constant<int, 0> ride0{};
        auto flush_up = [&]() {
#pragma unroll
            for (int i = 0; i < ND; ++i) mfma_group<SP, -1>(hT, wfd[i], mp[NG + i]);
        };
        auto flush_downA = [&]() { flush_acc7(hpA, false); };
        auto flush_downB = [&]() { flush_acc7(hpB, false); };
        auto flush_downA0 = [&]() { flush_acc7(hpA, true); };
        stage_up(yes, none, flush_none);
        flush_up();
#pragma unroll
        for (int k = 0; k < 8; ++k) split_pair(k, hpA);
#define PAIR(c, fl, flA)                                                                    \
        stage_up(no, HEAD((c) - 1), fl);                                        \
        stage_down(hpA, hpB, yes, HEAD((c) - 1), ride0, flush_up);  \
        stage_up(no, HEAD(c), flA);                                         \
        stage_down(hpB, hpA, yes, HEAD(c), ride0, flush_up);
        PAIR(1, flush_none, flush_downA0) PAIR(3, flush_downB, flush_downA) PAIR(5, flush_downB, flush_downA) PAIR(7, flush_downB, flush_downA)
#undef PAIR
        for (int c = 9; c < 31; c += 2) {
            stage_up(no, none, flush_downB);
            stage_down(hpA, hpB, yes, none, ride0, flush_up);
            stage_up(no, none, flush_downA);
            stage_down(hpB, hpA, yes, none, ride0, flush_up);
        }
        stage_up(no, none, flush_downB);
        if constexpr (QF) {
            stage_down(hpA, hpB, yes, none, ride0, flush_up);
            stage_down(hpB, hpA, no, none, ride0, flush_downA);
        } else {
        stage_down(hpA, hpB, yes, none, HEAD(1), flush_up);
        stage_down(hpB, hpA, no, none, HEAD(2), flush_downA);
        }
        flush_downB();
#undef HEAD
        TSTAMP(3);
        VM_WAIT(0);
        if (QF && T_QF_DUMP == 6) dbg6[3] = asum(acc);
        if (!QF && has_next) {
            pin_head(op);
            pin_x(qA);
#pragma unroll
            for (int g = 0; g < 12; ++g) apply_ride(qA, g, apB, S_next, tile_next);
        }

        TSTAMP(4);
        V yp[NQ ? 16 : 1][NP];
        unsigned osum_keep = 0, gsum_keep = 0;
        {
            float sum = 0.f;
#pragma unroll
            for (int b = 0; b < 8; ++b)
#pragma unroll
                for (int e = 0; e < 16; ++e) sum += acc[b][e];
            if (QF && T_QF_DUMP == 6) {
                const float p1 = __shfl_xor(sum, 32), p2 = __shfl_xor(sum, 32);
                dbg6[5] = sum; dbg6[6] = p1; dbg6[7] = (p1 == p2) ? 1.0f : 2.0f;
            }
            sum += __shfl_xor(sum, 32);
            const float mean = sum * (1.0f / 256.0f);
            float var = 0.f;
#pragma unroll
            for (int b = 0; b < 8; ++b)
#pragma unroll
                for (int e = 0; e < 16; ++e) {
                    acc[b][e] -= mean;
                    var += acc[b][e] * acc[b][e];
                }
            var += __shfl_xor(var, 32);
            const float rstd = 1.0f / sqrtf(var * (1.0f / 256.0f) + eps2);
            const float* gp = lnp + 512 + 4 * half;
            const float* bp = lnp + 768 + 4 * half;
            float* yg = y + grp + lane * 4;
            unsigned osum = 0, gsum = 0;
            if (QF && T_QF_DUMP == 6) { dbg6[0] = mean; dbg6[1] = rstd; dbg6[2] = var; }
#pragma unroll
            for (int b = 0; b < 8; ++b)
#pragma unroll
                for (int s2 = 0; s2 < 2; ++s2) {
                    f32x4 o2[2];
#pragma unroll
                    for (int a2 = 0; a2 < 2; ++a2) {
                        const int a = 2 * s2 + a2;
                        const f32x4 g4 = ld4(gp + 32 * b + 8 * a), b4 = ld4(bp + 32 * b + 8 * a);
                        f32x4 o;
#pragma unroll
                        for (int k = 0; k < 4; ++k) o[k] = acc[b][4 * a + k] * rstd * g4[k] + b4[k];
                        if (QF && T_QF_DUMP == 6) {
#pragma unroll
                            for (int k = 0; k < 4; ++k) {
                                osum ^= __builtin_bit_cast(unsigned, o[k]);
                                gsum ^= __builtin_bit_cast(unsigned, g4[k]) ^ (__builtin_bit_cast(unsigned, b4[k]) * 3u);
                            }
                        }
                        if ((!(T_ABLATE & (16 | 128)) && !(QF && T_QF_DUMP && T_QF_DUMP < 4)) || o[0] + o[1] + o[2] + o[3] == 123.456f) {
                            if (T_NT & 2) __builtin_nontemporal_store(o, reinterpret_cast<f32x4*>(yg + (b * 4 + a) * 256));
                            else *reinterpret_cast<f32x4*>(yg + (b * 4 + a) * 256) = o;
                        }
                        o2[a2] = o;
                    }
                    if (NQ) {
                        if (T_MIX & 2) split8s<SP>(o2[0], o2[1], sc.s_y, yp[NQ ? 2 * b + s2 : 0]);
                        else split8<SP>(o2[0] * sc.s_y, o2[1] * sc.s_y, yp[NQ ? 2 * b + s2 : 0]);
                    }
                }
            osum_keep = osum;
            gsum_keep = gsum;
        }
        if constexpr (NQ) {
            f32x16 hq[2];
            f32x4 oq[4];
            float* qg = q_next + grp + lane * 4;
            auto elu_pair = [&](int k, const f32x16& h) {
#pragma unroll
                for (int e = 0; e < 2; ++e) {
                    const int i = 2 * k + e;
                    const float x = h[i] * sc.cq;
                    oq[i >> 2][i & 3] = elu1(x);
                }
            };
            auto store_chunk = [&](int j) {
#pragma unroll
                for (int a = 0; a < 4; ++a)
                    if (!(T_ABLATE & (16 | 128)) || oq[a][0] == 123.456f) {
                        if (T_NT & 2) __builtin_nontemporal_store(oq[a], reinterpret_cast<f32x4*>(qg + (j * 4 + a) * 256));
                        else *reinterpret_cast<f32x4*>(qg + (j * 4 + a) * 256) = oq[a];
                    }
            };
            constexpr int PP = (PIECES + NG - 9) / (NG - 8);
            auto stage_q = [&](auto jj) {
                constexpr int j = decltype(jj)::value;
                if (j == 0) lds_only_barrier(); else ring_barrier<PIECES>();
                __builtin_amdgcn_sched_barrier(0);
                const char* wb = smem + (q % T_SLOTS) * STAGE + lane * 16;
                V wf[T_PF][NP];
#pragma unroll
                for (int g0 = 0; g0 < T_PF - 1; ++g0)
#pragma unroll
                    for (int p = 0; p < NP; ++p) wf[g0][p] = ld_frag<V>(wb + (p * 16 + g0) * 1024);
                if (j > 0) {
#pragma unroll
                    for (int i = 0; i < ND; ++i) mfma_group<SP, -1>(hq[(j + 1) & 1], wfd[i], yp[NG + i]);
                }
#pragma unroll
                for (int g = 0; g < NG; ++g) {
                    if (g + T_PF - 1 < 16) {
#pragma unroll
                        for (int p = 0; p < NP; ++p)
                            (g + T_PF - 1 >= NG ? wfd[g + T_PF - 1 - NG][p] : wf[(g + T_PF - 1) % T_PF][p]) = ld_frag<V>(wb + (p * 16 + g + T_PF - 1) * 1024);
                    }
                    if (j > 0 && g < 8) elu_pair(g, hq[(j + 1) & 1]);
                    if (g == 8) {
                        __builtin_amdgcn_sched_barrier(0);
                        if (j > 0) store_chunk(j - 1);
                        __builtin_amdgcn_sched_barrier(0);
                    }
                    if (g >= 8) {
#pragma unroll
                        for (int u = (g - 8) * PP; u < (g - 7) * PP; ++u)
                            if (u < PIECES) dma_piece(q + 2, u);
                    }
                    mfma_group<SP, 8>(hq[j & 1], wf[g % T_PF], yp[g], g == 0);
                }
                ++q;
            };
            stage_q(std::integral_constant<int, 0>{});
            stage_q(std::integral_constant<int, 1>{});
            stage_q(std::integral_constant<int, 2>{});
            stage_q(std::integral_constant<int, 3>{});
            stage_q(std::integral_constant<int, 4>{});
            stage_q(std::integral_constant<int, 5>{});
            stage_q(std::integral_constant<int, 6>{});
            stage_q(std::integral_constant<int, 7>{});
#pragma unroll
            for (int i = 0; i < ND; ++i) mfma_group<SP, -1>(hq[1], wfd[i], yp[NG + i]);
#pragma unroll
            for (int k = 0; k < 8; ++k) elu_pair(k, hq[1]);
            store_chunk(7);
        }
        if (QF && T_QF_DUMP == 6 && q_next) {
            float* qd = q_next + grp + lane * 8;
            dbg6[4] = __builtin_bit_cast(float, (osum_keep & 0x007fffffu) | 0x3f800000u);
            *reinterpret_cast<f32x4*>(qd) = f32x4{dbg6[0], dbg6[1], dbg6[2], dbg6[3]};
            *reinterpret_cast<f32x4*>(qd + 4) = f32x4{dbg6[4], dbg6[5], dbg6[6], dbg6[7]};
        }
        TSTAMP(5);
        TMARKS_FLUSH();
        tile = tile_next;
        grp = ((int64_t)tile_next * 128 + wave * 32) * SCREAM_D_MODEL;
        kvc = kvc_next;
        S = S_next;
    }
    VM_WAIT(0);
}

__global__ __launch_bounds__(256) void act_layout_kernel(const float* __restrict__ src, float* __restrict__ dst, int to_frag) {
    __shared__ float tile[32][260];
    const int t = threadIdx.x;
    const float* s = src + (int64_t)blockIdx.x * 8192;
    float* d = dst + (int64_t)blockIdx.x * 8192;
#pragma unroll
    for (int i = 0; i < 8; ++i) {
        const int e = t + 256 * i;
        const f32x4 v = *reinterpret_cast<const f32x4*>(s + e * 4);
        int row, col;
        if (to_frag) {
            row = e >> 6, col = (e & 63) * 4;
        } else {
            const int ln = e & 63, a = (e >> 6) & 3, blk = e >> 8;
            row = ln & 31, col = 32 * blk + 8 * a + 4 * (ln >> 5);
        }
        *reinterpret_cast<f32x4*>(&tile[row][col]) = v;
    }
    __syncthreads();
#pragma unroll
    for (int i = 0; i < 8; ++i) {
        const int e = t + 256 * i;
        int row, col;
        if (to_frag) {
            const int ln = e & 63, a = (e >> 6) & 3, blk = e >> 8;
            row = ln & 31, col = 32 * blk + 8 * a + 4 * (ln >> 5);
        } else {
            row = e >> 6, col = (e & 63) * 4;
        }
        *reinterpret_cast<f32x4*>(d + e * 4) = *reinterpret_cast<const f32x4*>(&tile[row][col]);
    }
}

template <class SP>
__global__ void pack_tail_kernel(const float* __restrict__ Wm, const float* __restrict__ W1, const float* __restrict__ W2,
                                 const float* __restrict__ Wq_next, int q_first, float s_wm, float s_w1, float s_w2, float s_wq,
                                 typename SP::vec* __restrict__ out) {
    const int t = blockIdx.x * blockDim.x + threadIdx.x;
    if (t >= (TAIL_STAGES + (Wq_next ? NEXT_Q_STAGES : 0)) * 16 * 64) return;
    const int lane = t & 63, frag = (t >> 6) & 15, stage_out = t >> 10;
    const int stage = !(Wq_next && q_first) ? stage_out : stage_out < NEXT_Q_STAGES ? TAIL_STAGES + stage_out : stage_out - NEXT_Q_STAGES;
    const int m = lane & 31, half = lane >> 5;
    float v[8];
    float s;
    if (stage < 8) {
        s = s_wm;
#pragma unroll
        for (int j = 0; j < 8; ++j) v[j] = Wm[(int64_t)(32 * (frag >> 1) + m) * 256 + 32 * stage + chunk_k(frag & 1, half, j)];
    } else if (stage >= TAIL_STAGES) {
        s = s_wq;
#pragma unroll
        for (int j = 0; j < 8; ++j) v[j] = Wq_next[(int64_t)(32 * (stage - TAIL_STAGES) + m) * 256 + 32 * (frag >> 1) + chunk_k(frag & 1, half, j)];
    } else {
        const int st = stage - 8;
        const bool up = st == 0 || (st < 63 && (st & 1));
        const int c = st == 0 ? 0 : st == 63 ? 31 : up ? (st + 1) / 2 : st / 2 - 1;
        s = up ? s_w1 : s_w2;
        if (up) {
#pragma unroll
            for (int j = 0; j < 8; ++j) v[j] = W1[(int64_t)(32 * c + m) * 256 + 32 * (frag >> 1) + chunk_k(frag & 1, half, j)];
        } else {
#pragma unroll
            for (int j = 0; j < 8; ++j) v[j] = W2[(int64_t)(32 * (frag >> 1) + m) * 1024 + 32 * c + chunk_k(frag & 1, half, j)];
        }
    }
    typename SP::vec p[SP::NP];
#pragma unroll
    for (int j = 0; j < 8; ++j) SP::split1(SP::SCALED ? v[j] * s : v[j], j, p);
#pragma unroll
    for (int pl = 0; pl < SP::NP; ++pl) out[(((int64_t)stage_out * SP::NP + pl) * 16 + frag) * 64 + lane] = p[pl];
}

constexpr int KVF_THREADS = 320;

template <bool H2>
__global__ __launch_bounds__(KVF_THREADS) void kv_finalize_image_kernel(const float* __restrict__ partial,
                                                                      const int32_t* __restrict__ cloud_row0,
                                                                      const int32_t* __restrict__ cloud_len, int64_t row_base,
                                                                      int cloud_begin, char* __restrict__ kvimg,
                                                                      int64_t partial_layer_stride, int64_t image_layer_stride) {
    constexpr int KV_ELEMS = (SCREAM_HEAD_DIM + 1) * SCREAM_HEAD_DIM;
    static_assert(KV_ELEMS % 4 == 0 && KV_ELEMS / 4 <= KVF_THREADS, "");
    __shared__ float wmax[KVF_THREADS / 64];
    const int i4 = threadIdx.x;
    const bool active = i4 < KV_ELEMS / 4;
    const int kvi = blockIdx.x / SCREAM_NHEAD, h = blockIdx.x % SCREAM_NHEAD;
    const int cloud = cloud_begin + kvi;
    partial += (int64_t)blockIdx.y * partial_layer_stride;
    kvimg += (int64_t)blockIdx.y * image_layer_stride;
    const int t0 = (int)((cloud_row0[cloud] - row_base) / SCREAM_ROW_TILE);
    const int nt = (cloud_len[cloud] + SCREAM_ROW_TILE - 1) / SCREAM_ROW_TILE;
    const float* p = partial + ((int64_t)t0 * SCREAM_NHEAD + h) * KV_ELEMS + 4 * (active ? i4 : 0);
    char* img = kvimg + (size_t)cloud * KV_IMAGE_BYTES;
    const float S = (float)cloud_len[cloud];
    f32x4 s8[16];
#pragma unroll
    for (int u = 0; u < 16; ++u) s8[u] = f32x4{0.f, 0.f, 0.f, 0.f};
    if (active) {
        for (int c = 0; c < nt; c += 16) {
#pragma unroll
            for (int u = 0; u < 16; ++u)
                if (c + u < nt) s8[u] += *reinterpret_cast<const f32x4*>(p + (int64_t)(c + u) * SCREAM_NHEAD * KV_ELEMS);
        }
    }
#pragma unroll
    for (int u = 0; u < 8; ++u) s8[u] += s8[u + 8];
    const f32x4 s4 = ((s8[0] + s8[1]) + (s8[2] + s8[3])) + ((s8[4] + s8[5]) + (s8[6] + s8[7]));
    const bool is_kv = 4 * i4 < 32 * 32;
    f32x4 x4;
#pragma unroll
    for (int e = 0; e < 4; ++e) x4[e] = s4[e] / S;
    float scale = 1.f;
    if (H2) {
        float m = (active && is_kv) ? fmaxf(fmaxf(fabsf(x4[0]), fabsf(x4[1])), fmaxf(fabsf(x4[2]), fabsf(x4[3]))) : 0.f;
#pragma unroll
        for (int o = 32; o >= 1; o >>= 1) m = fmaxf(m, __shfl_xor(m, o));
        if ((threadIdx.x & 63) == 0) wmax[threadIdx.x >> 6] = m;
        __syncthreads();
        m = wmax[0];
#pragma unroll
        for (int w = 1; w < KVF_THREADS / 64; ++w) m = fmaxf(m, wmax[w]);
        const uint32_t mb = __float_as_uint(m);
        int eh = 15 - ((int)(mb >> 23) - 127) - ((mb & 0x7fffffu) ? 1 : 0);
        if (!(m >= 1.17549435e-38f) || eh > 40) eh = 40;
        if (eh < -30) eh = -30;
        scale = __uint_as_float((uint32_t)(eh + 127) << 23);
        if (threadIdx.x < 8) reinterpret_cast<float*>(img + KV_H2_SCALE_OFF)[h * 8 + threadIdx.x] = __uint_as_float((uint32_t)(127 - eh) << 23);
    }
    if (!active) return;
#pragma unroll
    for (int e = 0; e < 4; ++e) {
        const int i = 4 * i4 + e;
        if (is_kv) {
            const int d = i >> 5, v = i & 31;
            const float x = x4[e];
            const int s2 = d >> 4, hf = (d >> 2) & 1, j = 4 * ((d >> 3) & 1) + (d & 3);
            if (H2) {
                const _Float16 a = (_Float16)(x * scale);
                const _Float16 b = (_Float16)__builtin_fmaf(x, scale, -(float)a);
                _Float16* base = reinterpret_cast<_Float16*>(img) + ((size_t)(h * 2) * 2 + s2) * 512 + (v + 32 * hf) * 8 + j;
                base[0] = a;
                base[2 * 512] = b;
            } else {
                const __bf16 a = (__bf16)x;
                const float r1 = x - (float)a;
                const __bf16 b = (__bf16)r1;
                const __bf16 cc = (__bf16)(r1 - (float)b);
                __bf16* base = reinterpret_cast<__bf16*>(img) + ((size_t)(h * 3) * 2 + s2) * 512 + (v + 32 * hf) * 8 + j;
                base[0] = a;
                base[2 * 512] = b;
                base[4 * 512] = cc;
            }
        } else {
            reinterpret_cast<float*>(img + KV_PLANES_BYTES)[h * 32 + (i - 32 * 32)] = s4[e];
        }
    }
}

bool split_ok(int32_t split) { return split == SCREAM_SPLIT_BF3 || split == SCREAM_SPLIT_H2 || split == SCREAM_SPLIT_H1; }

bool tail_scales(const scream_tail_exps_t* ex, TailScales* sc) {
    if (!ex) return false;
    const int es[6] = {ex->e_att, ex->e_wm, ex->e_m1, ex->e_w1, ex->e_h, ex->e_w2};
    for (int e : es)
        if (e < -40 || e > 40) return false;
    const int e1 = ex->e_wm + ex->e_att, e2 = ex->e_w2 + ex->e_h, eh = ex->e_h - ex->e_w1 - ex->e_m1;
    if (e1 < -44 || e1 > 44 || e2 < -44 || e2 > 44 || eh < -100 || eh > 100) return false;
    if (ex->e_q < -40 || ex->e_q > 40) return false;
    sc->s_att = exp2i(ex->e_att);
    sc->e_q = ex->e_q;
    sc->e_att = ex->e_att;
    sc->c1 = exp2i(e1);
    sc->eps1 = 1e-5f * exp2i(2 * e1);
    sc->s_m1 = exp2i(ex->e_m1);
    sc->ch = exp2i(eh);
    sc->c2 = exp2i(e2);
    sc->eps2 = 1e-5f * exp2i(2 * e2);
    if (ex->e_y < -40 || ex->e_y > 40 || ex->e_wq < -40 || ex->e_wq > 40) return false;
    sc->s_y = exp2i(ex->e_y);
    sc->cq = exp2i(-ex->e_y - ex->e_wq);
    if (ex->e_x < -40 || ex->e_x > 40) return false;
    sc->s_x = exp2i(ex->e_x);
    sc->cqf = exp2i(-ex->e_x - ex->e_wq);
    return true;
}

}

extern "C" int64_t scream_tail_image_bytes(int32_t split, int32_t with_next_q) {
    if (!split_ok(split) || (with_next_q && split == SCREAM_SPLIT_BF3)) return SCREAM_EINVAL;
    return (int64_t)(TAIL_STAGES + (with_next_q ? NEXT_Q_STAGES : 0)) * split * 16 * 1024;
}
extern "C" int64_t scream_kv_image_bytes(void) { return KV_IMAGE_BYTES; }

extern "C" int scream_pack_tail(const float* Wm, const float* W1, const float* W2, const float* Wq_next, int32_t q_first, int32_t split,
                                const scream_tail_exps_t* exps, void* image, void* stream) {
    SCREAM_REQUIRE(Wm && W1 && W2 && image && split_ok(split), SCREAM_EINVAL);
    SCREAM_REQUIRE(!Wq_next || split != SCREAM_SPLIT_BF3, SCREAM_EUNSUPPORTED);
    SCREAM_REQUIRE(!q_first || Wq_next, SCREAM_EINVAL);
    SCREAM_REQUIRE((reinterpret_cast<uintptr_t>(image) & 15) == 0, SCREAM_EINVAL);
    const dim3 grid((TAIL_STAGES + (Wq_next ? NEXT_Q_STAGES : 0)) * 16 * 64 / 256), block(256);
    if (split != SCREAM_SPLIT_BF3) {
        TailScales sc;
        SCREAM_REQUIRE(tail_scales(exps, &sc), SCREAM_EINVAL);
        if (split == SCREAM_SPLIT_H2)
            pack_tail_kernel<SplitH2><<<grid, block, 0, as_stream(stream)>>>(Wm, W1, W2, Wq_next, q_first, exp2i(exps->e_wm), exp2i(exps->e_w1),
                                                                             exp2i(exps->e_w2), exp2i(exps->e_wq), reinterpret_cast<f16x8*>(image));
        else
            pack_tail_kernel<SplitH1><<<grid, block, 0, as_stream(stream)>>>(Wm, W1, W2, Wq_next, q_first, exp2i(exps->e_wm), exp2i(exps->e_w1),
                                                                             exp2i(exps->e_w2), exp2i(exps->e_wq), reinterpret_cast<f16x8*>(image));
    } else {
        pack_tail_kernel<SplitBf3><<<grid, block, 0, as_stream(stream)>>>(Wm, W1, W2, nullptr, 0, 1.f, 1.f, 1.f, 1.f, reinterpret_cast<bf16x8*>(image));
    }
    SCREAM_LAUNCH_CHECK();
    return 0;
}

extern "C" int scream_kv_finalize_image(const float* kv_partial, const int32_t* cloud_row0, const int32_t* cloud_len,
                                        int64_t row_base, int32_t cloud_begin, int32_t n_kv, void* kv_image, int32_t n_layers,
                                        int64_t partial_layer_stride, int64_t image_layer_stride, int32_t split, void* stream) {
    SCREAM_REQUIRE(kv_partial && cloud_row0 && cloud_len && kv_image && split_ok(split), SCREAM_EINVAL);
    SCREAM_REQUIRE(n_kv >= 0 && cloud_begin >= 0 && row_base >= 0 && n_layers >= 1 && n_layers <= 65535, SCREAM_EINVAL);
    SCREAM_REQUIRE(n_layers == 1 || (partial_layer_stride > 0 && image_layer_stride > 0 && image_layer_stride % 16 == 0), SCREAM_EINVAL);
    SCREAM_REQUIRE(((reinterpret_cast<uintptr_t>(kv_image) | reinterpret_cast<uintptr_t>(kv_partial)) & 15) == 0 && partial_layer_stride % 4 == 0,
                   SCREAM_EINVAL);
    if (n_kv == 0) return 0;
    const dim3 grid(n_kv * SCREAM_NHEAD, n_layers), block(KVF_THREADS);
    if (split != SCREAM_SPLIT_BF3 && T_APPLY_H2)
        kv_finalize_image_kernel<true><<<grid, block, 0, as_stream(stream)>>>(kv_partial, cloud_row0, cloud_len, row_base, cloud_begin,
                                                                              reinterpret_cast<char*>(kv_image), partial_layer_stride, image_layer_stride);
    else
        kv_finalize_image_kernel<false><<<grid, block, 0, as_stream(stream)>>>(kv_partial, cloud_row0, cloud_len, row_base, cloud_begin,
                                                                               reinterpret_cast<char*>(kv_image), partial_layer_stride, image_layer_stride);
    SCREAM_LAUNCH_CHECK();
    return 0;
}

namespace {
template <class SP, bool NQ, bool QF = false>
void launch_tail(unsigned grid, hipStream_t st, const float* Q, const void* kv_image, const int32_t* tile_cloud, int32_t kv_cloud_offset,
                 const int32_t* cloud_len, const float* x, const void* tail_image, const float* g1, const float* b1, const float* g2,
                 const float* b2, float* y, float* q_next, int tiles, const TailScales& sc) {
    tail_kernel<SP, NQ, QF><<<dim3(grid), dim3(TT), 0, st>>>(Q, reinterpret_cast<const char*>(kv_image), tile_cloud, kv_cloud_offset, cloud_len, x,
                                                         reinterpret_cast<const char*>(tail_image), g1, b1, g2, b2, y, q_next, tiles, sc);
}
}

extern "C" int scream_layer_tail_f32(const float* Q, const void* kv_image, const int32_t* tile_cloud,
                                     int32_t kv_cloud_offset, const int32_t* cloud_len, const float* x,
                                     const void* tail_image, const float* g1, const float* b1, const float* g2,
                                     const float* b2, float* y, float* q_next, int64_t M, int32_t split,
                                     const scream_tail_exps_t* exps, void* stream) {
    SCREAM_REQUIRE(kv_image && tile_cloud && cloud_len && x && tail_image && g1 && b1 && g2 && b2 && y && split_ok(split), SCREAM_EINVAL);
    SCREAM_REQUIRE(Q || (split != SCREAM_SPLIT_BF3 && (!q_next || T_QF_DUMP >= 4)), SCREAM_EINVAL);
    SCREAM_REQUIRE(M >= 0 && M % SCREAM_ROW_TILE == 0, SCREAM_EUNSUPPORTED);
    SCREAM_REQUIRE(((reinterpret_cast<uintptr_t>(Q) | reinterpret_cast<uintptr_t>(kv_image) | reinterpret_cast<uintptr_t>(x) |
                     reinterpret_cast<uintptr_t>(tail_image) | reinterpret_cast<uintptr_t>(g1) | reinterpret_cast<uintptr_t>(b1) |
                     reinterpret_cast<uintptr_t>(g2) | reinterpret_cast<uintptr_t>(b2) | reinterpret_cast<uintptr_t>(y) |
                     reinterpret_cast<uintptr_t>(q_next)) & 15) == 0, SCREAM_EINVAL);
    SCREAM_REQUIRE(x != y, SCREAM_EINVAL);
    SCREAM_REQUIRE(!q_next || (split != SCREAM_SPLIT_BF3 && q_next != x && q_next != y), SCREAM_EINVAL);
    TailScales sc{1.f, 0, 0, 1.f, 1e-5f, 1.f, 1.f, 1.f, 1e-5f, 1.f, 1.f, 1.f, 1.f};
    if (split != SCREAM_SPLIT_BF3) SCREAM_REQUIRE(tail_scales(exps, &sc), SCREAM_EINVAL);
    const int64_t tiles = M / SCREAM_ROW_TILE;
    if (tiles == 0) return 0;
    SCREAM_REQUIRE(tiles < (1ll << 31), SCREAM_EUNSUPPORTED);
    const unsigned grid = tiles < T_MAX_GRID ? (unsigned)tiles : (unsigned)T_MAX_GRID;
    hipStream_t st = as_stream(stream);
#define TAIL_ARGS grid, st, Q, kv_image, tile_cloud, kv_cloud_offset, cloud_len, x, tail_image, g1, b1, g2, b2, y, q_next, (int)tiles, sc
    if (split == SCREAM_SPLIT_H2) {
        if (!Q) launch_tail<SplitH2, false, true>(TAIL_ARGS);
        else if (q_next) launch_tail<SplitH2, true>(TAIL_ARGS);
        else launch_tail<SplitH2, false>(TAIL_ARGS);
    } else if (split == SCREAM_SPLIT_H1) {
        if (!Q) launch_tail<SplitH1, false, true>(TAIL_ARGS);
        else if (q_next) launch_tail<SplitH1, true>(TAIL_ARGS);
        else launch_tail<SplitH1, false>(TAIL_ARGS);
    } else {
        launch_tail<SplitBf3, false>(TAIL_ARGS);
    }
#undef TAIL_ARGS
    SCREAM_LAUNCH_CHECK();
    return 0;
}

extern "C" int scream_act_layout(const float* src, float* dst, int64_t M, int32_t to_fragment, void* stream) {
    SCREAM_REQUIRE(src && dst && src != dst, SCREAM_EINVAL);
    SCREAM_REQUIRE(M >= 0 && M % 32 == 0 && M / 32 < (1ll << 31), SCREAM_EUNSUPPORTED);
    SCREAM_REQUIRE(((reinterpret_cast<uintptr_t>(src) | reinterpret_cast<uintptr_t>(dst)) & 15) == 0, SCREAM_EINVAL);
    if (M == 0) return 0;
    act_layout_kernel<<<dim3((unsigned)(M / 32)), dim3(256), 0, as_stream(stream)>>>(src, dst, to_fragment ? 1 : 0);
    SCREAM_LAUNCH_CHECK();
    return 0;
}
```

scream_amd/model.py:

```python
from __future__ import annotations

import ctypes as C
import os
from typing import List, Optional, Sequence, Tuple

import torch
from torch import nn

from . import _lib, ops, scales
from .packing import PackedBatch
from .render import RegistrationRender

D_MODEL = 256
NHEAD = 8


class _MHAParams(nn.Module):

    def __init__(self, d_model: int, nhead: int = NHEAD):
        super().__init__()
        self.q_proj = nn.Linear(d_model, d_model, bias=False)
        self.k_proj = nn.Linear(d_model, d_model, bias=False)
        self.v_proj = nn.Linear(d_model, d_model, bias=False)
        self.merge = nn.Linear(d_model, d_model, bias=False)
        self.mlp = nn.Sequential(nn.Linear(d_model, d_model * 4, bias=False), nn.ReLU(True),
                                 nn.Linear(d_model * 4, d_model, bias=False))
        self.norm1 = nn.LayerNorm(d_model)
        self.norm2 = nn.LayerNorm(d_model)


class _CrossParams(nn.Module):

    def __init__(self, d_model: int, nhead: int = NHEAD):
        super().__init__()
        self.layer = _MHAParams(d_model, nhead)
        for p in self.parameters():
            if p.dim() > 1:
                nn.init.xavier_uniform_(p)


def pe_dim_t(d_model: int = D_MODEL) -> torch.Tensor:
    npf = d_model // 3 // 2 * 2
    i = torch.arange(npf, dtype=torch.float32)
    return 10000 ** (2 * torch.trunc(torch.div(i, 2)) / npf)


class _Pack:

    def __init__(self, backend, sig, mt, layers, keep, fused, n_cross_batched, event, streams):
        self.backend, self.sig, self.mt, self.layers, self.keep = backend, sig, mt, layers, keep
        self.fused, self.n_cross_batched, self.event, self.streams = fused, n_cross_batched, event, streams


class PointTransformer(nn.Module):
    def __init__(self, d_model: int = 256, self_layer_num: int = 6, cross_layer_num: int = 6):
        super().__init__()
        if d_model != D_MODEL:
            raise NotImplementedError("the gfx950 kernels are built for d_model=256 (8 heads x 32), the only "
                                      "configuration the reference evaluates (evaluate_3d_match.py:188)")
        self.embedding = nn.Conv1d(3, d_model, kernel_size=1, stride=1)
        self.pre_norm = nn.LayerNorm(d_model)
        self.self_layer_num = self_layer_num
        self.cross_layer_num = cross_layer_num
        self.stem = nn.ModuleList([_MHAParams(d_model) for _ in range(self_layer_num)])
        self.cross = nn.ModuleList()
        for _ in range(cross_layer_num):
            self.cross.append(_MHAParams(d_model))
            self.cross.append(_CrossParams(d_model))
        self.coor_mlp = nn.Sequential(nn.Conv1d(d_model, d_model, 1), nn.ReLU(), nn.Conv1d(d_model, d_model, 1),
                                      nn.ReLU(), nn.Conv1d(d_model, 3, 1))
        self.generator = RegistrationRender(rho=24, w=64)
        self._packs = {}
        self._ws = None

    def _layer_modules(self) -> List[_MHAParams]:
        mods = list(self.stem)
        for i, m in enumerate(self.cross):
            mods.append(m if i % 2 == 0 else m.layer)
        return mods

    def _stem_tgt_modules(self) -> Optional[List[_MHAParams]]:
        return None

    gemm_backend = os.environ.get("SCREAM_GEMM", "h2")

    TRAIN_BACKENDS = ("f32", "split")
    _train_backend_default = os.environ.get("SCREAM_TRAIN_GEMM", "f32")

    @classmethod
    def _check_train_backend(cls, value):
        if value not in cls.TRAIN_BACKENDS:
            raise ValueError("train_backend must be one of %s, got %r" % (", ".join(repr(b) for b in cls.TRAIN_BACKENDS), value))
        return value

    @property
    def train_backend(self) -> str:
        return self.__dict__.get("_train_backend", type(self)._train_backend_default)

    @train_backend.setter
    def train_backend(self, value: str) -> None:
        self.__dict__["_train_backend"] = self._check_train_backend(value)

    fused_tail = os.environ.get("SCREAM_FUSED_TAIL", "1") != "0"

    batched_cross_kv = os.environ.get("SCREAM_BATCHED_CROSS_KV", "1") != "0"

    fuse_next_q = os.environ.get("SCREAM_FUSE_NEXT_Q", "1") != "0"

    ring_proj = os.environ.get("SCREAM_RING_PROJ", "1") != "0"

    q_first = os.environ.get("SCREAM_Q_FIRST", "0") == "1"

    def _fused_cfg(self, split) -> bool:
        return bool(split and self.fused_tail)

    def _signature(self):
        return (self.fused_tail, self.batched_cross_kv, self.fuse_next_q, self.ring_proj, self.q_first) + tuple((p.data_ptr(), p._version) for p in self.parameters())

    def _layer_inputs(self):
        ln = lambda n: (n.weight, n.bias)
        mods, tgt_mods = self._layer_modules(), self._stem_tgt_modules()
        ns = self.self_layer_num
        pre = ln(self.pre_norm)
        ins, prev = [], pre
        for i in range(ns):
            ins.append((prev, prev))
            prev = ln(mods[i].norm2)
        src_in = prev
        tgt_ins, prev_t = [], pre
        for m in (tgt_mods or []):
            tgt_ins.append((prev_t, prev_t))
            prev_t = ln(m.norm2)
        tgt_in = prev_t if tgt_mods else src_in
        for j in range(2 * self.cross_layer_num):
            ins.append((src_in, src_in if j % 2 == 0 else tgt_in))
            src_in = ln(mods[ns + j].norm2)
        return ins, tgt_ins, src_in

    def _pack_weights(self, backend: Optional[str] = None) -> "_Pack":
        backend = self.gemm_backend if backend is None else backend
        if backend not in ("h2", "x3", "f32", "h1"):
            raise ValueError("gemm_backend must be 'h2', 'x3', 'f32' or 'h1', got %r" % (backend,))
        sig = self._signature()
        if self._packs and next(iter(self._packs.values())).sig != sig:
            torch.cuda.synchronize(self.embedding.weight.device) if self.embedding.weight.is_cuda else None
            self._packs = {}
        pk = self._packs.get(backend)
        if pk is not None:
            return pk
        try:
            pk = self._build_pack(backend, sig)
        except scales.ScaleRangeError as e:
            if backend != "h2":
                raise
            import warnings
            warnings.warn("scream_amd: gemm_backend 'h2' cannot carry these weights (%s); using 'x3' (bf16 x 3 split, scale free, "
                          "same fp32-level accuracy at twice the matrix instructions)" % (e,), RuntimeWarning, stacklevel=3)
            pk = self._pack_weights("x3")
        self._packs[backend] = pk
        return pk

    def _build_pack(self, backend: str, sig) -> "_Pack":
        dev = self.embedding.weight.device
        if dev.type != "cuda":
            raise _lib.ScreamHipError("PointTransformer must be on the MI355X (net.to('cuda:0')) before forward; "
                                      "scream_amd has no CPU path")
        keep = []

        def dev_f32(t):
            t = t.detach().to(device=dev, dtype=torch.float32).contiguous()
            keep.append(t)
            return t.data_ptr()

        split = {"h2": _lib.SPLIT_H2, "x3": _lib.SPLIT_BF3, "f32": 0, "h1": _lib.SPLIT_H1}[backend]
        fp16_split = split in (_lib.SPLIT_H2, _lib.SPLIT_H1)

        def dev_mat(t):
            if not split:
                return dev_f32(t), 0
            pw = ops.pack_w(t.detach().to(device=dev, dtype=torch.float32), split)
            keep.append(pw.data)
            return pw.data_ptr(), pw.w_exp

        mods = self._layer_modules()
        tgt_mods = self._stem_tgt_modules() or []
        ins, tgt_ins, coor_in = self._layer_inputs()
        layers = (_lib.LayerT * len(mods))()
        tgt_layers = (_lib.LayerT * max(len(tgt_mods), 1))()
        ns = self.self_layer_num
        qf = bool(fp16_split and self.fused_tail and self.q_first)
        if qf:
            import warnings
            warnings.warn("scream_amd: q_first is experimental -- its layer-tail kernel is not repeatable bit for bit when other kernels run "
                          "beside it (profiles/r04_qf_experiment.txt); do not use it for results")
        next_cross = {id(mods[i]): i + 1 for i in range(ns, len(mods) - 1, 2)} if (fp16_split and self.fused_tail and self.fuse_next_q and not qf) else {}
        for L, m, (in_q, in_kv) in list(zip(layers, mods, ins)) + list(zip(tgt_layers, tgt_mods, tgt_ins)):
            k, v = m.k_proj.weight, m.v_proj.weight
            wkv = torch.cat([k[:128], v[:128], k[128:], v[128:]], dim=0)
            L.wqkv, L.e_wqkv = dev_mat(torch.cat([m.q_proj.weight, wkv], dim=0))
            L.proj = None
            if fp16_split and self.fused_tail and self.ring_proj:
                pp = ops.pack_proj(torch.cat([m.q_proj.weight, wkv], dim=0).detach().to(device=dev, dtype=torch.float32), 256, split, L.e_wqkv)
                keep.append(pp.data)
                L.proj = pp.data_ptr()
            L.wq, L.e_wq = dev_mat(m.q_proj.weight)
            L.wkv, L.e_wkv = dev_mat(wkv)
            ex = scales.layer_exps(m, in_q, in_kv) if fp16_split else {}
            L.e_xq, L.e_xkv, L.e_k, L.e_v = ex.get("e_xq", 0), ex.get("e_xkv", 0), ex.get("e_k", 0), ex.get("e_v", 0)
            wq_next = None
            if id(m) in next_cross:
                nxt = next_cross[id(m)]
                wq_next = mods[nxt].q_proj.weight
                ex.update(e_y=scales.exp_for(scales.ln_bound(*ins[nxt][0])), e_wq=scales.w_exp(wq_next))
            if qf:
                ex.update(e_x=ex["e_xq"], e_wq=scales.w_exp(m.q_proj.weight))
            L.tail_exps = ops.tail_exps(**ex)
            L.tail = None
            L.tail_next_q = int(wq_next is not None)
            L.tail_q_first, L.proj_kv = int(qf), None
            if qf and self.ring_proj:
                pp = ops.pack_proj(wkv.detach().to(device=dev, dtype=torch.float32), 0, split, L.e_wkv)
                keep.append(pp.data)
                L.proj_kv = pp.data_ptr()
            if split and self.fused_tail:
                f32 = lambda t: t.detach().to(device=dev, dtype=torch.float32)
                img = ops.pack_tail(f32(m.merge.weight), f32(m.mlp[0].weight), f32(m.mlp[2].weight), split, L.tail_exps,
                                    Wq_next=None if wq_next is None else f32(wq_next), Wq_own=f32(m.q_proj.weight) if qf else None)
                keep.append(img.data)
                L.tail = img.data_ptr()
                L.wm, L.w1, L.w2 = None, None, None
            else:
                L.wm, L.e_wm_g = dev_mat(m.merge.weight)
                L.w1, L.e_w1_g = dev_mat(m.mlp[0].weight)
                L.w2, L.e_w2_g = dev_mat(m.mlp[2].weight)
            L.g1, L.b1 = dev_f32(m.norm1.weight), dev_f32(m.norm1.bias)
            L.g2, L.b2 = dev_f32(m.norm2.weight), dev_f32(m.norm2.bias)
        mt = _lib.ModelT()
        mt.n_self, mt.n_cross = self.self_layer_num, self.cross_layer_num
        mt.dim_t = dev_f32(pe_dim_t())
        mt.emb_w = dev_f32(self.embedding.weight[:, :, 0])
        mt.emb_b = dev_f32(self.embedding.bias)
        mt.pre_g, mt.pre_b = dev_f32(self.pre_norm.weight), dev_f32(self.pre_norm.bias)
        mt.layers_host = C.cast(layers, C.POINTER(_lib.LayerT))
        mt.stem_tgt_layers_host = C.cast(tgt_layers, C.POINTER(_lib.LayerT)) if tgt_mods else None
        mt.gemm_split = split
        c0w, c2w = self.coor_mlp[0].weight[:, :, 0], self.coor_mlp[2].weight[:, :, 0]
        (mt.c0_w, mt.e_c0w), mt.c0_b = dev_mat(c0w), dev_f32(self.coor_mlp[0].bias)
        (mt.c2_w, mt.e_c2w), mt.c2_b = dev_mat(c2w), dev_f32(self.coor_mlp[2].bias)
        mt.c4_w, mt.c4_b = dev_f32(self.coor_mlp[4].weight[:, :, 0]), dev_f32(self.coor_mlp[4].bias)
        mt.wkv_cross, mt.proj_cross = None, None
        if self._fused_cfg(split) and self.batched_cross_kv and self.cross_layer_num > 0:
            cross = [m for i, m in enumerate(self.cross) if i % 2 == 1]
            stack = torch.cat([torch.cat([c.layer.k_proj.weight[:128], c.layer.v_proj.weight[:128], c.layer.k_proj.weight[128:],
                                          c.layer.v_proj.weight[128:]], dim=0) for c in cross], dim=0)
            mt.wkv_cross, mt.e_wkv_cross = dev_mat(stack)
            if fp16_split and self.ring_proj:
                pp = ops.pack_proj(stack.detach().to(device=dev, dtype=torch.float32), 0, split, mt.e_wkv_cross)
                keep.append(pp.data)
                mt.proj_cross = pp.data_ptr()
            cross_L = [layers[self.self_layer_num + 2 * j + 1] for j in range(self.cross_layer_num)]
            mt.e_k_cross, mt.e_v_cross = min(L.e_k for L in cross_L), min(L.e_v for L in cross_L)
        if fp16_split:
            mt.e_c0x = scales.exp_for(scales.ln_bound(*coor_in))
            mt.e_c2x = scales.exp_for(scales.lin_bound(c0w, *coor_in, bias=self.coor_mlp[0].bias))
        event = torch.cuda.Event()
        event.record(torch.cuda.current_stream(dev))
        return _Pack(backend, sig, mt, (layers, tgt_layers), keep, self._fused_cfg(split), self.cross_layer_num if mt.wkv_cross else 0,
                     event, {torch.cuda.current_stream(dev).cuda_stream})

    def forward_packed(self, batch: PackedBatch, return_feats: bool = False, trace=None, backend: Optional[str] = None):
        pk = self._pack_weights(backend)
        mt = pk.mt
        lib = _lib.load()
        dev = batch.xyz.device
        if ops._stream() not in pk.streams:
            torch.cuda.current_stream(dev).wait_event(pk.event)
            pk.streams.add(ops._stream())
        need = lib.scream_forward_workspace_bytes(batch.rows_src, batch.rows_total, batch.n_pairs, batch.max_chunks, int(pk.fused),
                                                  pk.n_cross_batched)
        if self._ws is None:
            self._ws = {}
        key = (dev, ops._stream())
        ws = self._ws.get(key)
        if ws is None or ws.numel() < need:
            ws = self._ws[key] = torch.empty(need, device=dev, dtype=torch.uint8)
        bt = _lib.BatchT()
        bt.n_pairs, bt.rows_src, bt.rows_total, bt.max_chunks = batch.n_pairs, batch.rows_src, batch.rows_total, batch.max_chunks
        bt.xyz, bt.center = ops._p(batch.xyz), ops._p(batch.center)
        bt.tile_cloud = ops._p(batch.tile_cloud, torch.int32)
        bt.cloud_row0 = ops._p(batch.cloud_row0, torch.int32)
        bt.cloud_len = ops._p(batch.cloud_len, torch.int32)
        src_pred = torch.empty(batch.rows_src, 3, device=dev, dtype=torch.float32)
        feats = torch.empty(batch.rows_src, D_MODEL, device=dev, dtype=torch.float32) if return_feats else None
        _lib.check(lib.scream_forward(C.byref(mt), C.byref(bt), ws.data_ptr(), ws.numel(),
                                      src_pred.data_ptr(), feats.data_ptr() if return_feats else None,
                                      trace, ops._stream()), "scream_forward")
        return (src_pred, feats) if return_feats else src_pred

    def forward_batch(self, srcs: Sequence[torch.Tensor], tgts: Sequence[torch.Tensor],
                      centers: Optional[Sequence[Optional[torch.Tensor]]] = None) -> List[torch.Tensor]:
        batch = PackedBatch.from_pairs(srcs, tgts, centers)
        return [t.clone() for t in batch.unpack_src(self.forward_packed(batch))]

    def train(self, mode: bool = True):
        if mode:
            self._check_train_backend(self.train_backend)
        super().train(mode)
        self._grad_train = bool(mode)
        return self

    def _trains(self) -> bool:
        return getattr(self, "_grad_train", False) and torch.is_grad_enabled()

    def forward_packed_train(self, batch: PackedBatch) -> torch.Tensor:
        if type(self) not in (PointTransformer, DEMTransformer):
            raise NotImplementedError("training is implemented for PointTransformer and DEMTransformer only")
        from . import train as _train
        return _train.apply(self, batch)

    def forward(self, src, tgt, src_center=None, s=1, get_imgs=False, get_transform=False, filter=None):
        if self._trains():
            return self._forward_train(src, tgt, src_center, s, get_imgs, get_transform, filter)
        with torch.no_grad():
            return self._forward_infer(src, tgt, src_center, s, get_imgs, get_transform, filter)

    def _forward_train(self, src, tgt, src_center, s, get_imgs, get_transform, filter):
        assert src.shape[0] == 1, "batch size must 1"
        assert tgt.shape[0] == 1, "batch size must 1"
        center = None if src_center is None else src_center.reshape(3)
        batch = PackedBatch.from_pairs([src[0].detach()], [tgt[0].detach()], [None if center is None else center.detach()])
        src_ = self.forward_packed_train(batch)[: src.shape[1]].unsqueeze(0)
        imgs = self.generator(src_[0], tgt[0].detach()) if get_imgs else None
        transform = None
        if get_transform:
            from .geometry import register_from_prediction
            with torch.no_grad():
                ref = tgt[0] if filter is None else filter[0]
                transform = register_from_prediction(src[0], src_[0].detach(), ref, float(s), 0.075)
        return src_, imgs, transform

    def _forward_infer(self, src, tgt, src_center=None, s=1, get_imgs=False, get_transform=False, filter=None):
        assert src.shape[0] == 1, "batch size must 1"
        assert tgt.shape[0] == 1, "batch size must 1"
        center = None if src_center is None else src_center.reshape(3)
        batch = PackedBatch.from_pairs([src[0]], [tgt[0]], [center])
        src_ = self.forward_packed(batch)[: src.shape[1]].unsqueeze(0).clone()
        imgs = self.generator(src_[0], tgt[0]) if get_imgs else None
        transform = None
        if get_transform:
            from .geometry import register_from_prediction
            ref = tgt[0] if filter is None else filter[0]
            transform = register_from_prediction(src[0], src_[0], ref, float(s), 0.075)
        return src_, imgs, transform

    def loss(self, src_pred, src_pcd, rot_gt, trans_gt):
        reg = (torch.matmul(rot_gt, src_pcd.permute([0, 2, 1])) + trans_gt).permute([0, 2, 1])
        return torch.mean(torch.sum(torch.abs(src_pred - reg), dim=-1), dim=1).mean(dim=0)


class DEMTransformer(PointTransformer):

    def __init__(self, d_model: int = 256, self_layer_num: int = 6, cross_layer_num: int = 6):
        nn.Module.__init__(self)
        if d_model != D_MODEL:
            raise NotImplementedError("the gfx950 kernels are built for d_model=256")
        self.embedding = nn.Conv1d(3, d_model, kernel_size=1, stride=1)
        self.pre_norm = nn.LayerNorm(d_model)
        self.self_layer_num = self_layer_num
        self.cross_layer_num = cross_layer_num
        self.stem_dsm = nn.ModuleList([_MHAParams(d_model) for _ in range(self_layer_num)])
        self.stem_dem = nn.ModuleList([_MHAParams(d_model) for _ in range(self_layer_num)])
        self.cross = nn.ModuleList()
        for _ in range(cross_layer_num):
            self.cross.append(_MHAParams(d_model))
            self.cross.append(_CrossParams(d_model))
        self.coor_mlp = nn.Sequential(nn.Conv1d(d_model, d_model, 1), nn.ReLU(), nn.Conv1d(d_model, d_model, 1),
                                      nn.ReLU(), nn.Conv1d(d_model, 3, 1))
        self.generator = RegistrationRender(rho=24, w=64, view="single")
        self._packs = {}
        self._ws = None

    def _layer_modules(self) -> List[_MHAParams]:
        mods = list(self.stem_dsm)
        for i, m in enumerate(self.cross):
            mods.append(m if i % 2 == 0 else m.layer)
        return mods

    def _stem_tgt_modules(self) -> Optional[List[_MHAParams]]:
        return list(self.stem_dem)

    def forward(self, dsm, dem_coarse, get_imgs=False):
        if self._trains():
            return self._forward_train(dsm, dem_coarse, get_imgs)
        with torch.no_grad():
            return self._forward_infer(dsm, dem_coarse, get_imgs)

    def _forward_train(self, dsm, dem_coarse, get_imgs=False):
        assert dsm.shape[0] == 1, "batch size must 1"
        assert dem_coarse.shape[0] == 1, "batch size must 1"
        zero = torch.zeros(3, device=dsm.device)
        batch = PackedBatch.from_pairs([dsm[0].detach()], [dem_coarse[0].detach()], [zero])
        dem_ = self.forward_packed_train(batch)[: dsm.shape[1]].unsqueeze(0)
        imgs = self.generator(dem_[0], dem_coarse[0].detach()) if get_imgs else None
        return dem_, imgs

    def _forward_infer(self, dsm, dem_coarse, get_imgs=False):
        assert dsm.shape[0] == 1, "batch size must 1"
        assert dem_coarse.shape[0] == 1, "batch size must 1"
        zero = torch.zeros(3, device=dsm.device)
        batch = PackedBatch.from_pairs([dsm[0]], [dem_coarse[0]], [zero])
        dem_ = self.forward_packed(batch)[: dsm.shape[1]].unsqueeze(0).clone()
        imgs = self.generator(dem_[0], dem_coarse[0]) if get_imgs else None
        return dem_, imgs

    def forward_batch(self, dsms, dems, centers=None):
        zero = torch.zeros(3, device=dsms[0].device)
        return super().forward_batch(dsms, dems, [zero] * len(dsms))

    def loss(self, dem_pred, dem):
        return torch.mean(torch.sum(torch.abs(dem_pred - dem), dim=-1), dim=1).mean(dim=0)
```

scream_amd/ops.py:

```python
from __future__ import annotations

import ctypes as C
import os
from dataclasses import dataclass
from typing import Optional, Tuple

import torch

from . import _lib, scales
from ._lib import SPLIT_BF3, SPLIT_H1, SPLIT_H2, check

EPI_NONE, EPI_ELU1, EPI_RELU, EPI_BIAS_RELU, EPI_RES_LN, EPI_QKV = 0, 1, 2, 3, 4, 5
ROW_TILE = 128
KV_CHUNK = 256
KV_ELEMS = 33 * 32
D_MODEL = 256


def _stream() -> int:
    return torch.cuda.current_stream().cuda_stream


def _p(t: Optional[torch.Tensor], dtype=torch.float32) -> Optional[int]:
    if t is None:
        return None
    if not t.is_cuda:
        raise _lib.ScreamHipError("scream_amd ops need tensors on the MI355X (got device %s); there is no CPU path" % t.device)
    if t.dtype != dtype:
        raise TypeError("expected %s, got %s" % (dtype, t.dtype))
    if not t.is_contiguous():
        raise ValueError("tensor must be contiguous")
    return t.data_ptr()


def gemm_f32(A: torch.Tensor, W: torch.Tensor, epilogue: int = EPI_NONE, n_act: int = 0,
             bias: Optional[torch.Tensor] = None, residual: Optional[torch.Tensor] = None,
             gamma: Optional[torch.Tensor] = None, beta: Optional[torch.Tensor] = None,
             out: Optional[torch.Tensor] = None) -> torch.Tensor:
    M, K = A.shape
    N = W.shape[0]
    assert W.shape[1] == K
    if out is None:
        out = torch.empty(M, N, device=A.device, dtype=torch.float32)
    lib = _lib.load()
    check(lib.scream_gemm_f32(_p(A), A.stride(0), _p(W), _p(out), out.stride(0), M, N, K, epilogue, n_act,
                              _p(bias), _p(residual), residual.stride(0) if residual is not None else 0,
                              _p(gamma), _p(beta), _stream()), "scream_gemm_f32")
    return out


@dataclass
class PackedW:
    data: torch.Tensor
    split: int
    w_exp: int
    N: int
    K: int
    row_l1: Optional[torch.Tensor] = None

    def data_ptr(self) -> int:
        return self.data.data_ptr()


@dataclass
class PackedTail:
    data: torch.Tensor
    split: int
    exps: _lib.TailExpsT
    next_q: bool = False
    q_first: bool = False

    def data_ptr(self) -> int:
        return self.data.data_ptr()


def default_split() -> int:
    return SPLIT_BF3 if os.environ.get("SCREAM_GEMM", "h2") == "x3" else SPLIT_H2


def pack_w(W: torch.Tensor, split: Optional[int] = None, w_exp: Optional[int] = None) -> PackedW:
    split = default_split() if split is None else split
    W = W.detach().to(torch.float32).contiguous()
    N, K = W.shape
    if split in (SPLIT_H2, SPLIT_H1) and w_exp is None:
        w_exp = scales.w_exp(W)
    w_exp = int(w_exp or 0)
    dt = torch.float16 if split in (SPLIT_H2, SPLIT_H1) else torch.bfloat16
    out = torch.empty(split, K // 32, N, 32, device=W.device, dtype=dt)
    check(_lib.load().scream_pack_w_split(_p(W), N, K, split, w_exp, _p(out, dt), _stream()), "scream_pack_w_split")
    return PackedW(out, split, w_exp, N, K, W.abs().sum(dim=1).cpu() if split != SPLIT_BF3 else None)


LAYOUT_A_FRAG, LAYOUT_C_FRAG = 1, 2


def act_layout(X: torch.Tensor, to_fragment: bool) -> torch.Tensor:
    M = X.shape[0]
    assert X.shape[1] == D_MODEL
    out = torch.empty_like(X)
    check(_lib.load().scream_act_layout(_p(X), _p(out), M, int(to_fragment), _stream()), "scream_act_layout")
    return out


def _a_exp(A: torch.Tensor, Wp, a_exp: Optional[int]) -> int:
    if Wp.split == SPLIT_BF3:
        return 0
    return scales.exp_for(A.abs().max().item()) if a_exp is None else int(a_exp)


def gemm_split(A: torch.Tensor, Wp: PackedW, epilogue: int = EPI_NONE, n_act: int = 0,
               bias: Optional[torch.Tensor] = None, residual: Optional[torch.Tensor] = None,
               gamma: Optional[torch.Tensor] = None, beta: Optional[torch.Tensor] = None,
               out: Optional[torch.Tensor] = None, layout: int = 0, a_exp: Optional[int] = None) -> torch.Tensor:
    M, K = A.shape
    assert K == Wp.K
    if out is None:
        out = torch.empty(M, Wp.N, device=A.device, dtype=torch.float32)
    check(_lib.load().scream_gemm_split_f32(_p(A), A.stride(0), Wp.data_ptr(), _p(out), out.stride(0), M, Wp.N, K,
                                            epilogue, n_act, _p(bias), _p(residual),
                                            residual.stride(0) if residual is not None else 0, _p(gamma), _p(beta), layout,
                                            Wp.split, _a_exp(A, Wp, a_exp), Wp.w_exp, _stream()),
          "scream_gemm_split_f32")
    return out


def tail_exps(**kw) -> _lib.TailExpsT:
    e = _lib.TailExpsT()
    for k in ("e_att", "e_wm", "e_m1", "e_w1", "e_h", "e_w2", "e_y", "e_wq", "e_x", "e_q"):
        setattr(e, k, int(kw.get(k, 0)))
    return e


def pack_tail(Wm: torch.Tensor, W1: torch.Tensor, W2: torch.Tensor, split: Optional[int] = None,
              exps: Optional[_lib.TailExpsT] = None, Wq_next: Optional[torch.Tensor] = None,
              Wq_own: Optional[torch.Tensor] = None) -> PackedTail:
    assert Wq_next is None or Wq_own is None
    q_first = Wq_own is not None
    Wq_next = Wq_own if q_first else Wq_next
    split = default_split() if split is None else split
    Wm, W1, W2 = (w.detach().to(torch.float32).contiguous() for w in (Wm, W1, W2))
    assert Wm.shape == (D_MODEL, D_MODEL) and W1.shape == (4 * D_MODEL, D_MODEL) and W2.shape == (D_MODEL, 4 * D_MODEL)
    if split != SPLIT_BF3 and exps is None:
        raise ValueError("pack_tail on an fp16 split needs the operand exponents (scream_amd/scales.py)")
    exps = exps if exps is not None else tail_exps()
    lib = _lib.load()
    if Wq_next is not None:
        Wq_next = Wq_next.detach().to(torch.float32).contiguous()
        assert Wq_next.shape == (D_MODEL, D_MODEL)
    nbytes = lib.scream_tail_image_bytes(split, int(Wq_next is not None))
    if nbytes < 0:
        raise _lib.ScreamHipError("scream_tail_image_bytes returned %d (a next-layer query projection needs an fp16 split)" % nbytes)
    out = torch.empty(nbytes, device=Wm.device, dtype=torch.uint8)
    check(lib.scream_pack_tail(_p(Wm), _p(W1), _p(W2), _p(Wq_next), int(q_first), split, C.byref(exps), _p(out, torch.uint8), _stream()), "scream_pack_tail")
    return PackedTail(out, split, exps, Wq_next is not None and not q_first, q_first)


def kv_finalize_image(partial: torch.Tensor, cloud_row0, cloud_len, row_base: int, cloud_begin: int, n_kv: int,
                   n_clouds: int, out: Optional[torch.Tensor] = None, split: Optional[int] = None) -> torch.Tensor:
    split = default_split() if split is None else split
    lib = _lib.load()
    L = partial.shape[0] if partial.dim() == 4 else 1
    img = lib.scream_kv_image_bytes()
    if out is None:
        out = torch.zeros((L, n_clouds, img) if partial.dim() == 4 else (n_clouds, img), device=partial.device, dtype=torch.uint8)
    check(lib.scream_kv_finalize_image(_p(partial), _p(cloud_row0, torch.int32), _p(cloud_len, torch.int32), row_base,
                                    cloud_begin, n_kv, _p(out, torch.uint8), L, partial[0].numel() if L > 1 else 0,
                                    n_clouds * img if L > 1 else 0, split, _stream()), "scream_kv_finalize_image")
    return out


def layer_tail(Q: torch.Tensor, kv_image: torch.Tensor, tile_cloud, kv_cloud_offset: int, cloud_len, x: torch.Tensor,
               tail: PackedTail, g1, b1, g2, b2, out: Optional[torch.Tensor] = None,
               q_next: Optional[torch.Tensor] = None) -> torch.Tensor:
    M = x.shape[0]
    assert x.shape[1] == D_MODEL and (Q is None or x.shape == Q.shape)
    assert (Q is None) == tail.q_first, "Q = None goes with an image that carries this layer's own query stages (pack_tail(Wq_own=...))"
    assert (q_next is not None) == tail.next_q, "q_next goes with an image that carries the next layer's query stages"
    if out is None:
        out = torch.empty(M, D_MODEL, device=x.device, dtype=torch.float32)
    check(_lib.load().scream_layer_tail_f32(_p(Q), _p(kv_image, torch.uint8), _p(tile_cloud, torch.int32),
                                            kv_cloud_offset, _p(cloud_len, torch.int32), _p(x),
                                            tail.data_ptr(), _p(g1), _p(b1), _p(g2), _p(b2), _p(out), _p(q_next),
                                            M, tail.split, C.byref(tail.exps), _stream()), "scream_layer_tail_f32")
    return out


def gemm_qkv(A: torch.Tensor, W, n_q: int, tile_cloud, cloud_row0, cloud_len, row_base: int, layout: int = 0,
             a_exp: Optional[int] = None, k_exp: Optional[int] = None, v_exp: Optional[int] = None):
    M, K = A.shape
    sp = isinstance(W, PackedW)
    N = W.N if sp else W.shape[0]
    Q = torch.empty(M, n_q, device=A.device, dtype=torch.float32) if n_q else None
    L = (N - n_q) // 512
    part = torch.empty((L, M // ROW_TILE, 8, KV_ELEMS) if L > 1 else (M // ROW_TILE, 8, KV_ELEMS), device=A.device, dtype=torch.float32)
    args = (_p(A), A.stride(0), W.data_ptr() if sp else _p(W), _p(Q), n_q, M, N, K, n_q,
            _p(tile_cloud, torch.int32), _p(cloud_row0, torch.int32), _p(cloud_len, torch.int32), row_base, _p(part))
    if sp:
        if W.split != SPLIT_BF3 and (k_exp is None or v_exp is None):
            amax = float(A.abs().max().item())
            rl = W.row_l1[n_q:].view(-1, 2, 128)
            k_exp = scales.exp_for(1.0 + amax * float(rl[:, 0].max())) if k_exp is None else k_exp
            v_exp = scales.exp_for(amax * float(rl[:, 1].max())) if v_exp is None else v_exp
        check(_lib.load().scream_gemm_qkv_split_f32(*args, layout, W.split, _a_exp(A, W, a_exp), W.w_exp, int(k_exp or 0),
                                                    int(v_exp or 0), _stream()),
              "scream_gemm_qkv_split_f32")
    else:
        assert layout == 0
        check(_lib.load().scream_gemm_qkv_f32(*args, _stream()), "scream_gemm_qkv")
    return Q, part


@dataclass
class PackedProj:
    data: torch.Tensor
    split: int
    w_exp: int
    N: int
    n_q: int
    row_l1: Optional[torch.Tensor] = None

    def data_ptr(self) -> int:
        return self.data.data_ptr()


def pack_proj(W: torch.Tensor, n_q: int, split: Optional[int] = None, w_exp: Optional[int] = None) -> PackedProj:
    split = SPLIT_H2 if split is None else split
    W = W.detach().to(torch.float32).contiguous()
    N, K = W.shape
    assert K == D_MODEL
    w_exp = scales.w_exp(W) if w_exp is None else int(w_exp)
    nbytes = _lib.load().scream_proj_image_bytes(N, split)
    if nbytes <= 0:
        raise _lib.ScreamHipError("scream_proj_image_bytes(%d, %d) = %d" % (N, split, nbytes))
    out = torch.empty(nbytes, device=W.device, dtype=torch.uint8)
    check(_lib.load().scream_pack_proj(_p(W), N, n_q, split, w_exp, _p(out, torch.uint8), _stream()), "scream_pack_proj")
    return PackedProj(out, split, w_exp, N, n_q, W.abs().sum(dim=1).cpu())


def proj_qkv(x_frag: torch.Tensor, P: PackedProj, tile_cloud, cloud_row0, cloud_len, row_base: int,
             a_exp: Optional[int] = None, k_exp: Optional[int] = None, v_exp: Optional[int] = None):
    M = x_frag.shape[0]
    Q = torch.empty(M, D_MODEL, device=x_frag.device, dtype=torch.float32) if P.n_q else None
    L = (P.N - P.n_q) // 512
    part = torch.empty((L, M // ROW_TILE, 8, KV_ELEMS) if L > 1 else (M // ROW_TILE, 8, KV_ELEMS), device=x_frag.device, dtype=torch.float32)
    if a_exp is None or k_exp is None or v_exp is None:
        amax = float(x_frag.abs().max().item())
        rl = P.row_l1[P.n_q:].view(-1, 2, 128)
        a_exp = scales.exp_for(amax) if a_exp is None else a_exp
        k_exp = scales.exp_for(1.0 + amax * float(rl[:, 0].max())) if k_exp is None else k_exp
        v_exp = scales.exp_for(amax * float(rl[:, 1].max())) if v_exp is None else v_exp
    check(_lib.load().scream_proj_qkv_f32(_p(x_frag), P.data_ptr(), _p(Q), M, P.N, P.n_q, _p(tile_cloud, torch.int32),
                                          _p(cloud_row0, torch.int32), _p(cloud_len, torch.int32), row_base, _p(part), P.split,
                                          int(a_exp), P.w_exp, int(k_exp), int(v_exp), _stream()), "scream_proj_qkv_f32")
    return Q, part


def kv_finalize(part, cloud_row0, cloud_len, row_base: int, cloud_begin: int, n_kv: int, n_clouds: int) -> torch.Tensor:
    kv = torch.zeros(n_clouds, 8, KV_ELEMS, device=part.device, dtype=torch.float32)
    check(_lib.load().scream_kv_finalize(_p(part), _p(cloud_row0, torch.int32), _p(cloud_len, torch.int32), row_base,
                                         cloud_begin, n_kv, _p(kv), _stream()), "scream_kv_finalize")
    return kv


def pe_embed_ln(xyz, tile_cloud, center, dim_t, emb_w, emb_b, gamma, beta, frag: bool = False) -> torch.Tensor:
    rows = xyz.shape[0]
    feats = torch.empty(rows, D_MODEL, device=xyz.device, dtype=torch.float32)
    lib = _lib.load()
    fn, name = (lib.scream_pe_embed_ln_frag, "scream_pe_embed_ln_frag") if frag else (lib.scream_pe_embed_ln, "scream_pe_embed_ln")
    check(fn(_p(xyz), _p(tile_cloud, torch.int32), _p(center), _p(dim_t), _p(emb_w),
             _p(emb_b), _p(gamma), _p(beta), _p(feats), rows, _stream()), name)
    return feats


def kv_reduce(Kf: torch.Tensor, Vf: torch.Tensor, ld: int, row_base: int, cloud_row0, cloud_len, cloud_begin: int,
              n_kv: int, max_chunks: int, n_clouds: int) -> torch.Tensor:
    dev = Kf.device
    partial = torch.empty(max(n_kv * max_chunks * 8 * KV_ELEMS, 1), device=dev, dtype=torch.float32)
    kv = torch.zeros(n_clouds, 8, KV_ELEMS, device=dev, dtype=torch.float32)
    for t in (Kf, Vf):
        if not t.is_cuda or t.dtype != torch.float32:
            raise TypeError("kv_reduce needs fp32 device tensors")
    check(_lib.load().scream_kv_reduce(Kf.data_ptr(), Vf.data_ptr(), ld, row_base, _p(cloud_row0, torch.int32),
                                       _p(cloud_len, torch.int32), cloud_begin, n_kv, max_chunks, _p(partial),
                                       _p(kv), _stream()), "scream_kv_reduce")
    return kv


def attn_apply(Qf: torch.Tensor, ldq: int, kv, tile_cloud, kv_cloud_offset: int, cloud_len, rows: int) -> torch.Tensor:
    out = torch.empty(rows, D_MODEL, device=kv.device, dtype=torch.float32)
    check(_lib.load().scream_attn_apply(Qf.data_ptr(), ldq, _p(kv), _p(tile_cloud, torch.int32), kv_cloud_offset,
                                        _p(cloud_len, torch.int32), _p(out), D_MODEL, rows, _stream()),
          "scream_attn_apply")
    return out


def coor_head(X: torch.Tensor, W: torch.Tensor, b: torch.Tensor) -> torch.Tensor:
    rows = X.shape[0]
    out = torch.empty(rows, 3, device=X.device, dtype=torch.float32)
    check(_lib.load().scream_coor_head(_p(X), _p(W), _p(b), _p(out), rows, _stream()), "scream_coor_head")
    return out


def nn_search(query: torch.Tensor, ref: torch.Tensor, q_row0, q_len, r_row0, r_len, s: torch.Tensor,
              max_q_len: int, max_r_len: int, thresh: float) -> Tuple[torch.Tensor, torch.Tensor, torch.Tensor]:
    dev = query.device
    qn, rn = query.shape[0], ref.shape[0]
    n_pairs = s.shape[0]
    ref_prep = torch.empty(max(rn, 1), 4, device=dev, dtype=torch.float32)
    keys = torch.empty(max(qn, 1), device=dev, dtype=torch.int64)
    idx = torch.empty(qn, device=dev, dtype=torch.int32)
    dmin = torch.empty(qn, device=dev, dtype=torch.float32)
    valid = torch.empty(qn, device=dev, dtype=torch.uint8)
    check(_lib.load().scream_nn_search(_p(query), _p(ref), _p(q_row0, torch.int32), _p(q_len, torch.int32),
                                       _p(r_row0, torch.int32), _p(r_len, torch.int32), _p(s), n_pairs, max_q_len,
                                       max_r_len, qn, rn, float(thresh), _p(ref_prep), _p(keys, torch.int64),
                                       _p(idx, torch.int32), _p(dmin), _p(valid, torch.uint8), _stream()),
          "scream_nn_search")
    return idx, dmin, valid


def render_workspace(n_pairs: int, n_views: int, w: int, src_rows_total: int, device) -> torch.Tensor:
    need = _lib.load().scream_render_workspace_bytes(n_pairs, n_views, w, src_rows_total)
    if need < 0:
        raise _lib.ScreamHipError("scream_render_workspace_bytes(%d, %d, %d, %d): invalid argument" % (n_pairs, n_views, w, src_rows_total))
    return torch.empty(max(need, 16), device=device, dtype=torch.uint8)


def render_depth(src: torch.Tensor, s_row0, s_len, tgt: torch.Tensor, t_row0, t_len, max_s_len: int, max_t_len: int,
                 rot: torch.Tensor, w: int, rho: float, workspace: Optional[torch.Tensor] = None) -> Tuple[torch.Tensor, torch.Tensor]:
    n_pairs, V = s_row0.shape[0], rot.shape[0]
    dev = src.device
    if workspace is None:
        workspace = render_workspace(n_pairs, V, w, src.shape[0], dev)
    imgs = torch.empty(n_pairs, V, 2, w, w, device=dev, dtype=torch.float32)
    argmax = torch.empty(n_pairs, V, 2, w, w, device=dev, dtype=torch.int32)
    check(_lib.load().scream_render_depth(_p(src), _p(s_row0, torch.int32), _p(s_len, torch.int32), _p(tgt), _p(t_row0, torch.int32),
                                          _p(t_len, torch.int32), n_pairs, int(max_s_len), int(max_t_len), src.shape[0],
                                          _p(rot.reshape(V, 9)), V, int(w), float(rho), _p(imgs), _p(argmax, torch.int32),
                                          _p(workspace, torch.uint8), workspace.numel(), _stream()), "scream_render_depth")
    return imgs, argmax


def render_depth_bwd(dimgs: torch.Tensor, argmax: torch.Tensor, src: torch.Tensor, s_row0, s_len, max_s_len: int,
                     rot: torch.Tensor, w: int, rho: float, workspace: torch.Tensor) -> torch.Tensor:
    n_pairs, V = s_row0.shape[0], rot.shape[0]
    dsrc = torch.zeros(src.shape[0], 3, device=src.device, dtype=torch.float32)
    check(_lib.load().scream_render_depth_bwd(_p(src), _p(s_row0, torch.int32), _p(s_len, torch.int32), n_pairs, int(max_s_len),
                                              src.shape[0], _p(rot.reshape(V, 9)), V, int(w), float(rho), _p(dimgs),
                                              _p(argmax, torch.int32), _p(workspace, torch.uint8), workspace.numel(), _p(dsrc),
                                              _stream()), "scream_render_depth_bwd")
    return dsrc


def kabsch_corr(src, ref, src_row0, src_len, ref_row0, idx, valid, s, c) -> Tuple[torch.Tensor, torch.Tensor]:
    n_pairs = s.shape[0]
    T = torch.empty(n_pairs, 4, 4, device=src.device, dtype=torch.float32)
    n_corr = torch.empty(n_pairs, device=src.device, dtype=torch.int32)
    check(_lib.load().scream_kabsch_corr(_p(src), _p(ref), _p(src_row0, torch.int32), _p(src_len, torch.int32),
                                         _p(ref_row0, torch.int32), _p(idx, torch.int32), _p(valid, torch.uint8),
                                         _p(s), _p(c), n_pairs, _p(T), _p(n_corr, torch.int32), _stream()),
          "scream_kabsch_corr")
    return T, n_corr


def rigid_transform_3d_dense(A: torch.Tensor, B: torch.Tensor, w: Optional[torch.Tensor], thr: float) -> torch.Tensor:
    bs, K = A.shape[0], A.shape[1]
    T = torch.empty(bs, 4, 4, device=A.device, dtype=torch.float32)
    check(_lib.load().scream_rigid_transform_3d(_p(A) if K else None, _p(B) if K else None, _p(w), float(thr), bs, K,
                                                _p(T), _stream()), "scream_rigid_transform_3d")
    return T


def transformation_error_batched(T_pred: torch.Tensor, T_gt: torch.Tensor) -> Tuple[torch.Tensor, torch.Tensor]:
    n = T_pred.shape[0]
    re = torch.empty(n, device=T_pred.device, dtype=torch.float32)
    te = torch.empty(n, device=T_pred.device, dtype=torch.float32)
    check(_lib.load().scream_transformation_error(_p(T_pred), _p(T_gt), n, _p(re), _p(te), _stream()),
          "scream_transformation_error")
    return re, te


def point_loss(src_pred: torch.Tensor, src: torch.Tensor, src_row0, src_len, rot: torch.Tensor, trans: torch.Tensor) -> torch.Tensor:
    B = rot.shape[0]
    out = torch.empty(B, device=src_pred.device, dtype=torch.float32)
    check(_lib.load().scream_point_loss(_p(src_pred), _p(src), _p(src_row0, torch.int32), _p(src_len, torch.int32),
                                        _p(rot.reshape(B, 9).contiguous()), _p(trans.reshape(B, 3).contiguous()), B, _p(out), _stream()),
          "scream_point_loss")
    return out


def icp_p2p(src, ref, src_row0, src_len, ref_row0, ref_len, s, c, T_init, max_src_len: int, max_ref_len: int,
            max_corr_dist: float, max_iter: int = 30, rel_fitness: float = 1e-6, rel_rmse: float = 1e-6):
    lib = _lib.load()
    n_pairs = s.shape[0]
    dev = src.device
    T = T_init.detach().clone().contiguous().float()
    fr = torch.empty(n_pairs, 2, device=dev, dtype=torch.float32)
    iters = torch.empty(n_pairs, device=dev, dtype=torch.int32)
    need = lib.scream_icp_workspace_bytes(src.shape[0], ref.shape[0], n_pairs)
    ws = torch.empty(need, device=dev, dtype=torch.uint8)
    check(lib.scream_icp_p2p(_p(src), _p(ref), _p(src_row0, torch.int32), _p(src_len, torch.int32),
                             _p(ref_row0, torch.int32), _p(ref_len, torch.int32), _p(s), _p(c), n_pairs, max_src_len,
                             max_ref_len, src.shape[0], ref.shape[0], float(max_corr_dist), int(max_iter),
                             float(rel_fitness), float(rel_rmse), _p(T), _p(fr), _p(iters, torch.int32),
                             ws.data_ptr(), need, _stream()), "scream_icp_p2p")
    return T, fr, iters


ICP_ASYNC_ITERS = 64


class IcpRun:

    def __init__(self, src, ref, src_row0, src_len, ref_row0, ref_len, s, c, T_init, max_src_len: int, max_ref_len: int,
                 max_corr_dist: float, max_iter: int, rel_fitness: float = 1e-6, rel_rmse: float = 1e-6):
        self.lib = _lib.load()
        n = s.shape[0]
        dev = src.device
        self.n, self.max_iter, self.next_it = n, int(max_iter), 0
        self.T = T_init.detach().clone().contiguous().float()
        self.fr = torch.empty(n, 2, device=dev, dtype=torch.float32)
        self.iters = torch.empty(n, device=dev, dtype=torch.int32)
        self.flags = torch.zeros(n, device=dev, dtype=torch.int32)
        self.flags_host = torch.zeros(n, dtype=torch.int32, pin_memory=True)
        need = self.lib.scream_icp_workspace_bytes(src.shape[0], ref.shape[0], n)
        self.ws = torch.empty(need, device=dev, dtype=torch.uint8)
        self._keep = (src, ref, src_row0, src_len, ref_row0, ref_len, s, c)
        self._args = (_p(src), _p(ref), _p(src_row0, torch.int32), _p(src_len, torch.int32), _p(ref_row0, torch.int32),
                      _p(ref_len, torch.int32), _p(s), _p(c), n, int(max_src_len), int(max_ref_len), src.shape[0], ref.shape[0],
                      float(max_corr_dist), int(max_iter), float(rel_fitness), float(rel_rmse), _p(self.T), _p(self.fr),
                      _p(self.iters, torch.int32))
        self.event = None

    @property
    def launches_left(self) -> int:
        return self.max_iter + 2 - self.next_it

    def advance(self, n_launches: int) -> None:
        end = min(self.next_it + int(n_launches), self.max_iter + 2)
        check(self.lib.scream_icp_p2p_range(*self._args, self.next_it, end, _p(self.flags, torch.int32), self.ws.data_ptr(),
                                            self.ws.numel(), _stream()), "scream_icp_p2p_range")
        self.next_it = end
        self.flags_host.copy_(self.flags, non_blocking=True)
        self.event = torch.cuda.Event()
        self.event.record(torch.cuda.current_stream(self.T.device))

    def all_stopped(self) -> bool:
        self.event.synchronize()
        return self.launches_left == 0 or bool(self.flags_host.all())
```

Baseline: 1863 pairs/s.

## Fuse coordinate MLP into last cross-layer fused tail kernel

Appends the coordinate-head MLP (two 256x256 bias+ReLU layers plus the 3-output projection) as extra stages of the last cross layer's fused tail kernel. It runs in a separately compiled translation unit and streams packed fp16-split weights through the existing ring. This removes two standalone GEMM launches, the coor_head kernel, and the round trips of the intermediate activations through global memory, and it can skip writing y when features are not needed. In exchange the kernel uses more LDS and registers, has a longer stage pipeline, and adds fp16-split quantization scales for the coordinate layers.

```diff
diff --git a/include/scream_hip.h b/include/scream_hip.h
--- a/include/scream_hip.h
+++ b/include/scream_hip.h
@@ -84,6 +84,21 @@
                           const void* tail_image, const float* g1, const float* b1, const float* g2,
                           const float* b2, float* y, float* q_next, int64_t M, int32_t split,
                           const scream_tail_exps_t* exps, void* stream);
+
+typedef struct {
+    const float* b0; const float* b2;
+    const float* w4; const float* b4;
+    float* src_pred;
+    const int32_t* cloud_row0; const int32_t* cloud_len;
+    int32_t e_c0x, e_c0w, e_c2x, e_c2w;
+} scream_coor_tail_t;
+int64_t scream_tail_coor_image_bytes(int32_t split);
+int scream_pack_tail_coor(const float* Wm, const float* W1, const float* W2, const float* Wc0, const float* Wc2, int32_t split,
+                          const scream_tail_exps_t* exps, const scream_coor_tail_t* coor, void* tail_image, void* stream);
+int scream_layer_tail_coor_f32(const float* Q, const void* kv_image, const int32_t* tile_cloud, int32_t kv_cloud_offset,
+                               const int32_t* cloud_len, const float* x, const void* tail_image, const float* g1, const float* b1,
+                               const float* g2, const float* b2, float* y, const scream_coor_tail_t* coor, int64_t M, int32_t split,
+                               const scream_tail_exps_t* exps, void* stream);
 
 int scream_pe_embed_ln(const float* xyz, const int32_t* tile_cloud, const float* center,
                        const float* dim_t, const float* emb_w, const float* emb_b,
diff --git a/scream_amd/_lib.py b/scream_amd/_lib.py
--- a/scream_amd/_lib.py
+++ b/scream_amd/_lib.py
@@ -19,6 +19,11 @@
 
 class TailExpsT(C.Structure):
     _fields_ = [(n, C.c_int32) for n in ("e_att", "e_wm", "e_m1", "e_w1", "e_h", "e_w2", "e_y", "e_wq", "e_x", "e_q")]
+
+
+class CoorTailT(C.Structure):
+    _fields_ = ([(n, C.c_void_p) for n in ("b0", "b2", "w4", "b4", "src_pred", "cloud_row0", "cloud_len")] +
+                [(n, C.c_int32) for n in ("e_c0x", "e_c0w", "e_c2x", "e_c2w")])
 
 
 class LayerT(C.Structure):
@@ -62,6 +67,9 @@
     "scream_pack_tail": (C.c_int, [V, V, V, V, I32, I32, C.POINTER(TailExpsT), V, V]),
     "scream_kv_finalize_image": (C.c_int, [V, V, V, I64, I32, I32, V, I32, I64, I64, I32, V]),
     "scream_layer_tail_f32": (C.c_int, [V, V, V, I32, V, V, V, V, V, V, V, V, V, I64, I32, C.POINTER(TailExpsT), V]),
+    "scream_tail_coor_image_bytes": (C.c_int64, [I32]),
+    "scream_pack_tail_coor": (C.c_int, [V, V, V, V, V, I32, C.POINTER(TailExpsT), C.POINTER(CoorTailT), V, V]),
+    "scream_layer_tail_coor_f32": (C.c_int, [V, V, V, I32, V, V, V, V, V, V, V, V, C.POINTER(CoorTailT), I64, I32, C.POINTER(TailExpsT), V]),
     "scream_act_layout": (C.c_int, [V, V, I64, I32, V]),
     "scream_pe_embed_ln": (C.c_int, [V, V, V, V, V, V, V, V, V, I64, V]),
     "scream_pe_embed_ln_frag": (C.c_int, [V, V, V, V, V, V, V, V, V, I64, V]),
diff --git a/scream_amd/build.py b/scream_amd/build.py
--- a/scream_amd/build.py
+++ b/scream_amd/build.py
@@ -16,6 +16,7 @@
     "gemm_split.hip": [],
     "proj_ring.hip": ["-mllvm", "-amdgpu-mfma-vgpr-form=1"],
     "tail_split.hip": ["-ffp-contract=off"],
+    "tail_coor.hip": ["-ffp-contract=off"],
     "embed.hip": [],
     "attention.hip": [],
     "backward.hip": [],
@@ -28,8 +29,9 @@
 EXTRA_DEFINES = {}
 for _item in filter(None, os.environ.get("SCREAM_HIPCC_EXTRA", "").split(";")):
     EXTRA_DEFINES[_item.split(":")[0]] = _item.split(":", 1)[1].split(",")
-ASM_LOADS = ("gemm_split.hip", "tail_split.hip", "proj_ring.hip")
-NO_SCRATCH = {"proj_ring.hip": ("proj_ring_kernel",), "tail_split.hip": ("tail_kernelINS_7SplitH2", "tail_kernelINS_7SplitH1")}
+ASM_LOADS = ("gemm_split.hip", "tail_split.hip", "tail_coor.hip", "proj_ring.hip")
+NO_SCRATCH = {"proj_ring.hip": ("proj_ring_kernel",), "tail_split.hip": ("tail_kernelINS_7SplitH2", "tail_kernelINS_7SplitH1"),
+              "tail_coor.hip": ("tail_kernelINS_7SplitH2", "tail_kernelINS_7SplitH1")}
 
 
 def _hipcc() -> str:
diff --git a/scream_amd/csrc/forward.hip b/scream_amd/csrc/forward.hip
--- a/scream_amd/csrc/forward.hip
+++ b/scream_amd/csrc/forward.hip
@@ -157,14 +157,17 @@
 }
 
 int mha_cross(const Ctx& c, const scream_layer_t& L, const scream_batch_t& b, const Workspace& w, const float* x_src,
-              const float* x_tgt, float* y, const char* kvimg_layer, bool q_ready = false) {
+              const float* x_tgt, float* y, const char* kvimg_layer, bool q_ready = false, const scream_coor_tail_t* coor = nullptr) {
     const int64_t rs = b.rows_src, rt = b.rows_total - b.rows_src;
     const bool qf = c.frag && L.tail_q_first;
     if (!q_ready && !qf)
         TRY(gemm(c, x_src, D, L.wq, w.q, D, rs, D, D, SCREAM_EPI_ELU1, D, nullptr, nullptr, nullptr, nullptr, L.e_xq, L.e_wq,
                  c.frag ? (SCREAM_LAYOUT_A_FRAG | SCREAM_LAYOUT_C_FRAG) : 0));
     if (c.frag && kvimg_layer) {
-        Scope sc(c.tr, TR_TAIL_FUSED, rs, (qf ? 10 : 9) * D, D, c.st);
+        Scope sc(c.tr, TR_TAIL_FUSED, rs, (coor ? 11 : qf ? 10 : 9) * D, D, c.st);
+        if (coor)
+            return scream_layer_tail_coor_f32(w.q, kvimg_layer, b.tile_cloud, 0, b.cloud_len + b.n_pairs, x_src, L.tail, L.g1, L.b1, L.g2, L.b2, y,
+                                              coor, rs, c.split, &L.tail_exps, c.st);
         return scream_layer_tail_f32(qf ? nullptr : w.q, kvimg_layer, b.tile_cloud, 0, b.cloud_len + b.n_pairs, x_src, L.tail, L.g1, L.b1, L.g2,
                                      L.b2, y, nullptr, rs, c.split, &L.tail_exps, c.st);
     }
@@ -174,7 +177,10 @@
             Scope sc(c.tr, TR_KV_REDUCE, rt, 0, 0, c.st);
             TRY(scream_kv_finalize_image(w.kvp, b.cloud_row0, b.cloud_len, rs, b.n_pairs, b.n_pairs, w.kvimg, 1, 0, 0, c.split, c.st));
         }
-        Scope sc(c.tr, TR_TAIL_FUSED, rs, (qf ? 10 : 9) * D, D, c.st);
+        Scope sc(c.tr, TR_TAIL_FUSED, rs, (coor ? 11 : qf ? 10 : 9) * D, D, c.st);
+        if (coor)
+            return scream_layer_tail_coor_f32(w.q, w.kvimg, b.tile_cloud, b.n_pairs, b.cloud_len, x_src, L.tail, L.g1, L.b1, L.g2, L.b2, y, coor, rs,
+                                              c.split, &L.tail_exps, c.st);
         return scream_layer_tail_f32(qf ? nullptr : w.q, w.kvimg, b.tile_cloud, b.n_pairs, b.cloud_len, x_src, L.tail, L.g1, L.b1, L.g2, L.b2,
                                      y, nullptr, rs, c.split, &L.tail_exps, c.st);
     }
@@ -300,6 +306,12 @@
         nxt = t;
     }
     const float* x_tgt = cur + rs * D;
+    const bool coor_tail = !m.c0_w && !m.c2_w;
+    SCREAM_REQUIRE(!coor_tail || (c.frag && m.n_cross > 0 && (c.split == SCREAM_SPLIT_H2 || c.split == SCREAM_SPLIT_H1) &&
+                                  !m.layers_host[m.n_self + 2 * m.n_cross - 1].tail_q_first),
+                   SCREAM_EINVAL);
+    SCREAM_REQUIRE(coor_tail || (m.c0_w && m.c2_w), SCREAM_EINVAL);
+    const scream_coor_tail_t coor{m.c0_b, m.c2_b, m.c4_w, m.c4_b, src_pred, b.cloud_row0, b.cloud_len, m.e_c0x, m.e_c0w, m.e_c2x, m.e_c2w};
     if (batched_kv) TRY(cross_kv_all(c, m, b, w, x_tgt));
     for (int i = 0; i < 2 * m.n_cross; ++i) {
         const scream_layer_t& L = m.layers_host[m.n_self + i];
@@ -307,18 +319,20 @@
             TRY(mha_self(c, L, b, w, cur, nxt, 0, rs, 0, b.n_pairs, c.frag && L.tail_next_q));
         } else {
             const bool q_ready = c.frag && m.layers_host[m.n_self + i - 1].tail_next_q;
-            TRY(mha_cross(c, L, b, w, cur, x_tgt, nxt, batched_kv ? w.kvimg_cross + (i / 2) * w.kvimg_cross_stride : nullptr, q_ready));
+            const bool last = coor_tail && i == 2 * m.n_cross - 1;
+            TRY(mha_cross(c, L, b, w, cur, x_tgt, last && !feats_out ? nullptr : nxt,
+                          batched_kv ? w.kvimg_cross + (i / 2) * w.kvimg_cross_stride : nullptr, q_ready, last ? &coor : nullptr));
         }
         float* t = cur;
         cur = nxt;
         nxt = t;
     }
-    float* c_mid = c.frag ? w.q : w.m1;
-    float* c_out = c.frag ? nxt : w.att;
-    TRY(gemm(c, cur, D, m.c0_w, c_mid, D, rs, D, D, SCREAM_EPI_BIAS_RELU, 0, m.c0_b, nullptr, nullptr, nullptr, m.e_c0x, m.e_c0w,
-             c.frag ? SCREAM_LAYOUT_A_FRAG : 0));
-    TRY(gemm(c, c_mid, D, m.c2_w, c_out, D, rs, D, D, SCREAM_EPI_BIAS_RELU, 0, m.c2_b, nullptr, nullptr, nullptr, m.e_c2x, m.e_c2w));
-    {
+    if (!coor_tail) {
+        float* c_mid = c.frag ? w.q : w.m1;
+        float* c_out = c.frag ? nxt : w.att;
+        TRY(gemm(c, cur, D, m.c0_w, c_mid, D, rs, D, D, SCREAM_EPI_BIAS_RELU, 0, m.c0_b, nullptr, nullptr, nullptr, m.e_c0x, m.e_c0w,
+                 c.frag ? SCREAM_LAYOUT_A_FRAG : 0));
+        TRY(gemm(c, c_mid, D, m.c2_w, c_out, D, rs, D, D, SCREAM_EPI_BIAS_RELU, 0, m.c2_b, nullptr, nullptr, nullptr, m.e_c2x, m.e_c2w));
         Scope sc(c.tr, TR_COOR_HEAD, rs, 0, 0, stream);
         TRY(scream_coor_head(c_out, m.c4_w, m.c4_b, src_pred, rs, stream));
     }
diff --git a/scream_amd/csrc/tail_coor.hip b/scream_amd/csrc/tail_coor.hip
--- /dev/null
+++ b/scream_amd/csrc/tail_coor.hip
@@ -0,0 +1,2 @@
+#define SCREAM_TAIL_COOR_TU 1
+#include "tail_split.hip"
diff --git a/scream_amd/csrc/tail_split.hip b/scream_amd/csrc/tail_split.hip
--- a/scream_amd/csrc/tail_split.hip
+++ b/scream_amd/csrc/tail_split.hip
@@ -24,6 +24,9 @@
 #define T_DEFER_H2 2
 #endif
 
+#if defined(T_STAMPS) && defined(SCREAM_TAIL_COOR_TU)
+#undef T_STAMPS
+#endif
 #ifdef T_STAMPS
 #define T_STAMP_SLOTS 24
 __device__ long long t_stamps[256 * 4 * T_STAMP_SLOTS];
@@ -52,6 +55,8 @@
 
 constexpr int TAIL_STAGES = 72;
 constexpr int NEXT_Q_STAGES = 8;
+constexpr int COOR_STAGES = 16;
+constexpr int COOR_LDS_FLOATS = 256 + 256 + 3 * 256 + 4;
 constexpr int KV_PLANES_BYTES = 8 * 3 * 2 * 1024;
 constexpr int KV_IMAGE_BYTES = KV_PLANES_BYTES + 8 * 32 * 4;
 
@@ -81,6 +86,18 @@
     float cq;
     float s_x;
     float cqf;
+    float s_c2;
+    float cc2;
+};
+
+struct CoorArgs {
+    const float* b0;
+    const float* b2;
+    const float* w4;
+    const float* b4;
+    float* out;
+    const int32_t* row0;
+    const int32_t* len;
 };
 
 __device__ __forceinline__ constexpr int xadd_slot(int h, int g, int nd) {
@@ -93,7 +110,7 @@
     return -1;
 }
 
-template <class SP, bool NQ, bool QF>
+template <class SP, bool NQ, bool QF, bool CM = false>
 __global__ __launch_bounds__(TT, 1) void tail_kernel(const float* __restrict__ Q,
                                                      const char* __restrict__ kvimg,
                                                      const int32_t* __restrict__ tile_cloud, int kv_cloud_offset,
@@ -104,10 +121,11 @@
                                                      const float* __restrict__ g2, const float* __restrict__ b2,
                                                      float* __restrict__ y,
                                                      float* q_next,
-                                                     int n_tiles, TailScales sc) {
+                                                     int n_tiles, TailScales sc, CoorArgs ca) {
+    static_assert(!CM || (SP::SCALED && !NQ && !QF), "the coordinate MLP rides behind the plain tail of an fp16 split");
     static_assert(!NQ || SP::SCALED, "the next-layer query projection is built for the fp16 splits");
     static_assert(!QF || (SP::SCALED && !NQ), "the in-kernel query projection is built for the fp16 splits and replaces the next-layer one");
-    constexpr int N_STAGES = TAIL_STAGES + ((NQ || QF) ? NEXT_Q_STAGES : 0);
+    constexpr int N_STAGES = TAIL_STAGES + ((NQ || QF) ? NEXT_Q_STAGES : 0) + (CM ? COOR_STAGES : 0);
     typedef typename SP::vec V;
     constexpr int NP = SP::NP;
     constexpr int STAGE = stage_bytes<SP>();
@@ -121,7 +139,8 @@
     constexpr int ND = SP::NPROD >= 6 ? 1 : T_DEFER_H2;
     constexpr int NG = 16 - ND;
     constexpr int NSTASH = (NP == 2 && !QF) ? T_STASH : 0;
-    __shared__ __attribute__((aligned(16))) char smem[T_SLOTS * STAGE + 4096 + NSTASH * 16384];
+    constexpr int COOR_OFF = T_SLOTS * STAGE + 4096 + NSTASH * 16384;
+    __shared__ __attribute__((aligned(16))) char smem[COOR_OFF + (CM ? COOR_LDS_FLOATS * 4 : 0)];
     const int tid = threadIdx.x, lane = tid & 63;
     const int wave = __builtin_amdgcn_readfirstlane(tid >> 6);
     const int half = lane >> 5;
@@ -131,6 +150,14 @@
     lnp[256 + tid] = SP::SCALED ? b1[tid] * sc.s_m1 : b1[tid];
     lnp[512 + tid] = g2[tid];
     lnp[768 + tid] = b2[tid];
+    if constexpr (CM) {
+        float* cw = reinterpret_cast<float*>(smem + COOR_OFF);
+        cw[tid] = ca.b0[tid];
+        cw[256 + tid] = ca.b2[tid];
+#pragma unroll
+        for (int c = 0; c < 3; ++c) cw[512 + 256 * c + tid] = ca.w4[256 * c + tid];
+        if (tid < 3) cw[1280 + tid] = ca.b4[tid];
+    }
     const float eps1 = SP::SCALED ? sc.eps1 : 1e-5f, eps2 = SP::SCALED ? sc.eps2 : 1e-5f;
     const unsigned v_lane16 = lane * 16, v_half16 = half * 16;
     auto dma_piece = [&](unsigned q, int u) {
@@ -341,7 +368,7 @@
         auto stage_merge = [&](auto hh, V (&ap)[2][NP], V (&ap_next)[2][NP], f32x4 (&q_cons)[4], f32x4 (&q_req)[4], auto flush) {
             constexpr int h = decltype(hh)::value;
             constexpr bool RIDE = h >= 1 && h <= 6;
-            if (h == 0 && !QF) { if (NQ) ring_barrier<0>(); else lds_only_barrier(); }
+            if (h == 0 && !QF) { if (NQ || CM) ring_barrier<0>(); else lds_only_barrier(); }
             else if (QF && (T_QF_DBG & 32) && h <= 1) ring_barrier<0>();
             else ring_barrier<PIECES>();
             TMARK(h);
@@ -748,7 +775,7 @@
         }
 
         TSTAMP(4);
-        V yp[NQ ? 16 : 1][NP];
+        V yp[(NQ || CM) ? 16 : 1][NP];
         unsigned osum_keep = 0, gsum_keep = 0;
         {
             float sum = 0.f;
@@ -796,15 +823,15 @@
                                 gsum ^= __builtin_bit_cast(unsigned, g4[k]) ^ (__builtin_bit_cast(unsigned, b4[k]) * 3u);
                             }
                         }
-                        if ((!(T_ABLATE & (16 | 128)) && !(QF && T_QF_DUMP && T_QF_DUMP < 4)) || o[0] + o[1] + o[2] + o[3] == 123.456f) {
+                        if (((!(T_ABLATE & (16 | 128)) && !(QF && T_QF_DUMP && T_QF_DUMP < 4)) || o[0] + o[1] + o[2] + o[3] == 123.456f) && (!CM || y)) {
                             if (T_NT & 2) __builtin_nontemporal_store(o, reinterpret_cast<f32x4*>(yg + (b * 4 + a) * 256));
                             else *reinterpret_cast<f32x4*>(yg + (b * 4 + a) * 256) = o;
                         }
                         o2[a2] = o;
                     }
-                    if (NQ) {
-                        if (T_MIX & 2) split8s<SP>(o2[0], o2[1], sc.s_y, yp[NQ ? 2 * b + s2 : 0]);
-                        else split8<SP>(o2[0] * sc.s_y, o2[1] * sc.s_y, yp[NQ ? 2 * b + s2 : 0]);
+                    if (NQ || CM) {
+                        if (T_MIX & 2) split8s<SP>(o2[0], o2[1], sc.s_y, yp[(NQ || CM) ? 2 * b + s2 : 0]);
+                        else split8<SP>(o2[0] * sc.s_y, o2[1] * sc.s_y, yp[(NQ || CM) ? 2 * b + s2 : 0]);
                     }
                 }
             osum_keep = osum;
@@ -881,6 +908,103 @@
             for (int k = 0; k < 8; ++k) elu_pair(k, hq[1]);
             store_chunk(7);
         }
+        if constexpr (CM) {
+            static_assert(ND == 2, "stage 8 reads cp[14], cp[15] in its deferred groups only");
+            f32x16 hc[2];
+            V cp[16][NP];
+            float s3[3] = {0.f, 0.f, 0.f};
+            const float* cpar = reinterpret_cast<const float*>(smem + COOR_OFF);
+            const float* cpl = cpar + 4 * half;
+            typedef float f32x2 __attribute__((ext_vector_type(2)));
+            auto relu1 = [&](float v) {
+                float r;
+                if (T_MIX & 1) asm("v_max_f32 %0, 0, %1" : "=v"(r) : "v"(v));
+                else r = fmaxf(v, 0.f);
+                return r;
+            };
+            auto ride_c0 = [&](int k, const f32x16& h, int jc) {
+                const int i = 2 * k, off = 32 * jc + 8 * (i >> 2) + (i & 3);
+                const f32x2 b = *reinterpret_cast<const f32x2*>(cpl + off);
+                const float x0 = relu1(__builtin_fmaf(h[i], sc.cq, b[0])), x1 = relu1(__builtin_fmaf(h[i + 1], sc.cq, b[1]));
+                SP::split2s(x0, x1, sc.s_c2, i & 7, cp[2 * jc + (k >> 2)]);
+            };
+            auto ride_c2 = [&](int k, const f32x16& h, int jc) {
+                const int i = 2 * k, off = 32 * jc + 8 * (i >> 2) + (i & 3);
+                const f32x2 b = *reinterpret_cast<const f32x2*>(cpl + 256 + off);
+                const float x0 = relu1(__builtin_fmaf(h[i], sc.cc2, b[0])), x1 = relu1(__builtin_fmaf(h[i + 1], sc.cc2, b[1]));
+#pragma unroll
+                for (int c = 0; c < 3; ++c) {
+                    const f32x2 w = *reinterpret_cast<const f32x2*>(cpl + 512 + 256 * c + off);
+                    s3[c] = __builtin_fmaf(x0, w[0], s3[c]);
+                    s3[c] = __builtin_fmaf(x1, w[1], s3[c]);
+                }
+            };
+            auto stage_c = [&](auto ss) {
+                constexpr int s = decltype(ss)::value;
+                if (s == 0) lds_only_barrier(); else ring_barrier<PIECES>();
+                __builtin_amdgcn_sched_barrier(0);
+                const char* wb = smem + (q % T_SLOTS) * STAGE + lane * 16;
+                V wf[T_PF][NP];
+#pragma unroll
+                for (int g0 = 0; g0 < T_PF - 1; ++g0)
+#pragma unroll
+                    for (int p = 0; p < NP; ++p) wf[g0][p] = ld_frag<V>(wb + (p * 16 + g0) * 1024);
+                if (s > 0) {
+#pragma unroll
+                    for (int i = 0; i < ND; ++i) {
+                        if (s <= 8) mfma_group<SP, -1>(hc[(s + 1) & 1], wfd[i], yp[NG + i]);
+                        else mfma_group<SP, -1>(hc[(s + 1) & 1], wfd[i], cp[NG + i]);
+                    }
+                }
+#pragma unroll
+                for (int g = 0; g < NG; ++g) {
+                    if (g + T_PF - 1 < 16) {
+#pragma unroll
+                        for (int p = 0; p < NP; ++p)
+                            (g + T_PF - 1 >= NG ? wfd[g + T_PF - 1 - NG][p] : wf[(g + T_PF - 1) % T_PF][p]) = ld_frag<V>(wb + (p * 16 + g + T_PF - 1) * 1024);
+                    }
+                    if (g < PIECES) dma_piece(q + 2, g);
+                    if (s > 0 && g >= T_RIDE0 && g < T_RIDE0 + 8) {
+                        if (s <= 8) ride_c0(g - T_RIDE0, hc[(s + 1) & 1], s > 0 ? s - 1 : 0);
+                        else ride_c2(g - T_RIDE0, hc[(s + 1) & 1], s > 8 ? s - 9 : 0);
+                    }
+                    if (s < 8) mfma_group<SP, 8>(hc[s & 1], wf[g % T_PF], yp[g], g == 0);
+                    else mfma_group<SP, 8>(hc[s & 1], wf[g % T_PF], cp[g], g == 0);
+                }
+                ++q;
+            };
+            stage_c(std::integral_constant<int, 0>{});
+            stage_c(std::integral_constant<int, 1>{});
+            stage_c(std::integral_constant<int, 2>{});
+            stage_c(std::integral_constant<int, 3>{});
+            stage_c(std::integral_constant<int, 4>{});
+            stage_c(std::integral_constant<int, 5>{});
+            stage_c(std::integral_constant<int, 6>{});
+            stage_c(std::integral_constant<int, 7>{});
+            stage_c(std::integral_constant<int, 8>{});
+            stage_c(std::integral_constant<int, 9>{});
+            stage_c(std::integral_constant<int, 10>{});
+            stage_c(std::integral_constant<int, 11>{});
+            stage_c(std::integral_constant<int, 12>{});
+            stage_c(std::integral_constant<int, 13>{});
+            stage_c(std::integral_constant<int, 14>{});
+            stage_c(std::integral_constant<int, 15>{});
+#pragma unroll
+            for (int i = 0; i < ND; ++i) mfma_group<SP, -1>(hc[1], wfd[i], cp[NG + i]);
+#pragma unroll
+            for (int k = 0; k < 8; ++k) ride_c2(k, hc[1], 7);
+            const int cl_row = tile_cloud[tile];
+            const int row_end = ca.row0[cl_row] + ca.len[cl_row];
+            const int64_t row = (int64_t)tile * 128 + wave * 32 + (lane & 31);
+            float o3[3];
+#pragma unroll
+            for (int c = 0; c < 3; ++c) o3[c] = (s3[c] + __shfl_xor(s3[c], 32)) + cpar[1280 + c];
+            if (half == 0 && row < row_end) {
+                float* op3 = ca.out + row * 3;
+#pragma unroll
+                for (int c = 0; c < 3; ++c) op3[c] = o3[c];
+            }
+        }
         if (QF && T_QF_DUMP == 6 && q_next) {
             float* qd = q_next + grp + lane * 8;
             dbg6[4] = __builtin_bit_cast(float, (osum_keep & 0x007fffffu) | 0x3f800000u);
@@ -896,6 +1020,37 @@
     }
     VM_WAIT(0);
 }
+
+}
+
+namespace scream_detail {
+int launch_tail_coor(int split, unsigned grid, hipStream_t st, const float* Q, const void* kv_image, const int32_t* tile_cloud,
+                     int32_t kv_cloud_offset, const int32_t* cloud_len, const float* x, const void* tail_image, const float* g1,
+                     const float* b1, const float* g2, const float* b2, float* y, int tiles, const void* scales, const void* coor_args);
+}
+
+#ifdef SCREAM_TAIL_COOR_TU
+int scream_detail::launch_tail_coor(int split, unsigned grid, hipStream_t st, const float* Q, const void* kv_image, const int32_t* tile_cloud,
+                                    int32_t kv_cloud_offset, const int32_t* cloud_len, const float* x, const void* tail_image, const float* g1,
+                                    const float* b1, const float* g2, const float* b2, float* y, int tiles, const void* scales,
+                                    const void* coor_args) {
+    const TailScales& sc = *reinterpret_cast<const TailScales*>(scales);
+    const CoorArgs& ca = *reinterpret_cast<const CoorArgs*>(coor_args);
+    const char* kvi = reinterpret_cast<const char*>(kv_image);
+    const char* img = reinterpret_cast<const char*>(tail_image);
+    if (split == SCREAM_SPLIT_H2)
+        tail_kernel<SplitH2, false, false, true><<<dim3(grid), dim3(TT), 0, st>>>(Q, kvi, tile_cloud, kv_cloud_offset, cloud_len, x, img, g1, b1, g2,
+                                                                                  b2, y, nullptr, tiles, sc, ca);
+    else if (split == SCREAM_SPLIT_H1)
+        tail_kernel<SplitH1, false, false, true><<<dim3(grid), dim3(TT), 0, st>>>(Q, kvi, tile_cloud, kv_cloud_offset, cloud_len, x, img, g1, b1, g2,
+                                                                                  b2, y, nullptr, tiles, sc, ca);
+    else
+        return SCREAM_EUNSUPPORTED;
+    return 0;
+}
+#else
+
+namespace {
 
 __global__ __launch_bounds__(256) void act_layout_kernel(const float* __restrict__ src, float* __restrict__ dst, int to_frag) {
     __shared__ float tile[32][260];
@@ -932,10 +1087,10 @@
 
 template <class SP>
 __global__ void pack_tail_kernel(const float* __restrict__ Wm, const float* __restrict__ W1, const float* __restrict__ W2,
-                                 const float* __restrict__ Wq_next, int q_first, float s_wm, float s_w1, float s_w2, float s_wq,
-                                 typename SP::vec* __restrict__ out) {
+                                 const float* __restrict__ Wq_next, const float* __restrict__ Wc2, int q_first, float s_wm, float s_w1,
+                                 float s_w2, float s_wq, float s_wc2, typename SP::vec* __restrict__ out) {
     const int t = blockIdx.x * blockDim.x + threadIdx.x;
-    if (t >= (TAIL_STAGES + (Wq_next ? NEXT_Q_STAGES : 0)) * 16 * 64) return;
+    if (t >= (TAIL_STAGES + (Wq_next ? NEXT_Q_STAGES : 0) + (Wc2 ? NEXT_Q_STAGES : 0)) * 16 * 64) return;
     const int lane = t & 63, frag = (t >> 6) & 15, stage_out = t >> 10;
     const int stage = !(Wq_next && q_first) ? stage_out : stage_out < NEXT_Q_STAGES ? TAIL_STAGES + stage_out : stage_out - NEXT_Q_STAGES;
     const int m = lane & 31, half = lane >> 5;
@@ -945,6 +1100,10 @@
         s = s_wm;
 #pragma unroll
         for (int j = 0; j < 8; ++j) v[j] = Wm[(int64_t)(32 * (frag >> 1) + m) * 256 + 32 * stage + chunk_k(frag & 1, half, j)];
+    } else if (stage >= TAIL_STAGES + NEXT_Q_STAGES) {
+        s = s_wc2;
+#pragma unroll
+        for (int j = 0; j < 8; ++j) v[j] = Wc2[(int64_t)(32 * (stage - TAIL_STAGES - NEXT_Q_STAGES) + m) * 256 + 32 * (frag >> 1) + chunk_k(frag & 1, half, j)];
     } else if (stage >= TAIL_STAGES) {
         s = s_wq;
 #pragma unroll
@@ -1091,27 +1250,58 @@
 }
 extern "C" int64_t scream_kv_image_bytes(void) { return KV_IMAGE_BYTES; }
 
-extern "C" int scream_pack_tail(const float* Wm, const float* W1, const float* W2, const float* Wq_next, int32_t q_first, int32_t split,
-                                const scream_tail_exps_t* exps, void* image, void* stream) {
+namespace {
+int pack_tail_any(const float* Wm, const float* W1, const float* W2, const float* Wq_next, const float* Wc2, int32_t q_first, int32_t split,
+                  const scream_tail_exps_t* exps, int32_t e_wc2, void* image, void* stream) {
     SCREAM_REQUIRE(Wm && W1 && W2 && image && split_ok(split), SCREAM_EINVAL);
     SCREAM_REQUIRE(!Wq_next || split != SCREAM_SPLIT_BF3, SCREAM_EUNSUPPORTED);
     SCREAM_REQUIRE(!q_first || Wq_next, SCREAM_EINVAL);
+    SCREAM_REQUIRE(!Wc2 || (Wq_next && !q_first && e_wc2 >= -40 && e_wc2 <= 40), SCREAM_EINVAL);
     SCREAM_REQUIRE((reinterpret_cast<uintptr_t>(image) & 15) == 0, SCREAM_EINVAL);
-    const dim3 grid((TAIL_STAGES + (Wq_next ? NEXT_Q_STAGES : 0)) * 16 * 64 / 256), block(256);
+    const dim3 grid((TAIL_STAGES + (Wq_next ? NEXT_Q_STAGES : 0) + (Wc2 ? NEXT_Q_STAGES : 0)) * 16 * 64 / 256), block(256);
     if (split != SCREAM_SPLIT_BF3) {
         TailScales sc;
         SCREAM_REQUIRE(tail_scales(exps, &sc), SCREAM_EINVAL);
         if (split == SCREAM_SPLIT_H2)
-            pack_tail_kernel<SplitH2><<<grid, block, 0, as_stream(stream)>>>(Wm, W1, W2, Wq_next, q_first, exp2i(exps->e_wm), exp2i(exps->e_w1),
-                                                                             exp2i(exps->e_w2), exp2i(exps->e_wq), reinterpret_cast<f16x8*>(image));
+            pack_tail_kernel<SplitH2><<<grid, block, 0, as_stream(stream)>>>(Wm, W1, W2, Wq_next, Wc2, q_first, exp2i(exps->e_wm), exp2i(exps->e_w1),
+                                                                             exp2i(exps->e_w2), exp2i(exps->e_wq), exp2i(e_wc2),
+                                                                             reinterpret_cast<f16x8*>(image));
         else
-            pack_tail_kernel<SplitH1><<<grid, block, 0, as_stream(stream)>>>(Wm, W1, W2, Wq_next, q_first, exp2i(exps->e_wm), exp2i(exps->e_w1),
-                                                                             exp2i(exps->e_w2), exp2i(exps->e_wq), reinterpret_cast<f16x8*>(image));
+            pack_tail_kernel<SplitH1><<<grid, block, 0, as_stream(stream)>>>(Wm, W1, W2, Wq_next, Wc2, q_first, exp2i(exps->e_wm), exp2i(exps->e_w1),
+                                                                             exp2i(exps->e_w2), exp2i(exps->e_wq), exp2i(e_wc2),
+                                                                             reinterpret_cast<f16x8*>(image));
     } else {
-        pack_tail_kernel<SplitBf3><<<grid, block, 0, as_stream(stream)>>>(Wm, W1, W2, nullptr, 0, 1.f, 1.f, 1.f, 1.f, reinterpret_cast<bf16x8*>(image));
+        pack_tail_kernel<SplitBf3><<<grid, block, 0, as_stream(stream)>>>(Wm, W1, W2, nullptr, nullptr, 0, 1.f, 1.f, 1.f, 1.f, 1.f,
+                                                                          reinterpret_cast<bf16x8*>(image));
     }
     SCREAM_LAUNCH_CHECK();
     return 0;
+}
+
+scream_tail_exps_t coor_exps(const scream_tail_exps_t& ex, const scream_coor_tail_t& c) {
+    scream_tail_exps_t e = ex;
+    e.e_y = c.e_c0x;
+    e.e_wq = c.e_c0w;
+    return e;
+}
+}
+
+extern "C" int scream_pack_tail(const float* Wm, const float* W1, const float* W2, const float* Wq_next, int32_t q_first, int32_t split,
+                                const scream_tail_exps_t* exps, void* image, void* stream) {
+    return pack_tail_any(Wm, W1, W2, Wq_next, nullptr, q_first, split, exps, 0, image, stream);
+}
+
+extern "C" int64_t scream_tail_coor_image_bytes(int32_t split) {
+    if (split != SCREAM_SPLIT_H2 && split != SCREAM_SPLIT_H1) return SCREAM_EINVAL;
+    return (int64_t)(TAIL_STAGES + COOR_STAGES) * split * 16 * 1024;
+}
+
+extern "C" int scream_pack_tail_coor(const float* Wm, const float* W1, const float* W2, const float* Wc0, const float* Wc2, int32_t split,
+                                     const scream_tail_exps_t* exps, const scream_coor_tail_t* coor, void* image, void* stream) {
+    SCREAM_REQUIRE(Wc0 && Wc2 && exps && coor, SCREAM_EINVAL);
+    SCREAM_REQUIRE(split == SCREAM_SPLIT_H2 || split == SCREAM_SPLIT_H1, SCREAM_EUNSUPPORTED);
+    const scream_tail_exps_t e = coor_exps(*exps, *coor);
+    return pack_tail_any(Wm, W1, W2, Wc0, Wc2, 0, split, &e, coor->e_c2w, image, stream);
 }
 
 extern "C" int scream_kv_finalize_image(const float* kv_partial, const int32_t* cloud_row0, const int32_t* cloud_len,
@@ -1138,18 +1328,18 @@
 template <class SP, bool NQ, bool QF = false>
 void launch_tail(unsigned grid, hipStream_t st, const float* Q, const void* kv_image, const int32_t* tile_cloud, int32_t kv_cloud_offset,
                  const int32_t* cloud_len, const float* x, const void* tail_image, const float* g1, const float* b1, const float* g2,
-                 const float* b2, float* y, float* q_next, int tiles, const TailScales& sc) {
+                 const float* b2, float* y, float* q_next, int tiles, const TailScales& sc, const CoorArgs& ca) {
     tail_kernel<SP, NQ, QF><<<dim3(grid), dim3(TT), 0, st>>>(Q, reinterpret_cast<const char*>(kv_image), tile_cloud, kv_cloud_offset, cloud_len, x,
-                                                         reinterpret_cast<const char*>(tail_image), g1, b1, g2, b2, y, q_next, tiles, sc);
-}
-}
-
-extern "C" int scream_layer_tail_f32(const float* Q, const void* kv_image, const int32_t* tile_cloud,
-                                     int32_t kv_cloud_offset, const int32_t* cloud_len, const float* x,
-                                     const void* tail_image, const float* g1, const float* b1, const float* g2,
-                                     const float* b2, float* y, float* q_next, int64_t M, int32_t split,
-                                     const scream_tail_exps_t* exps, void* stream) {
-    SCREAM_REQUIRE(kv_image && tile_cloud && cloud_len && x && tail_image && g1 && b1 && g2 && b2 && y && split_ok(split), SCREAM_EINVAL);
+                                                             reinterpret_cast<const char*>(tail_image), g1, b1, g2, b2, y, q_next, tiles, sc, ca);
+}
+
+int layer_tail_any(const float* Q, const void* kv_image, const int32_t* tile_cloud, int32_t kv_cloud_offset, const int32_t* cloud_len,
+                   const float* x, const void* tail_image, const float* g1, const float* b1, const float* g2, const float* b2, float* y,
+                   float* q_next, const scream_coor_tail_t* coor, int64_t M, int32_t split, const scream_tail_exps_t* exps, void* stream) {
+    SCREAM_REQUIRE(kv_image && tile_cloud && cloud_len && x && tail_image && g1 && b1 && g2 && b2 && (y || coor) && split_ok(split), SCREAM_EINVAL);
+    SCREAM_REQUIRE(!coor || (Q && !q_next && exps && (split == SCREAM_SPLIT_H2 || split == SCREAM_SPLIT_H1) && coor->b0 && coor->b2 && coor->w4 &&
+                             coor->b4 && coor->src_pred && coor->cloud_row0 && coor->cloud_len),
+                   SCREAM_EINVAL);
     SCREAM_REQUIRE(Q || (split != SCREAM_SPLIT_BF3 && (!q_next || T_QF_DUMP >= 4)), SCREAM_EINVAL);
     SCREAM_REQUIRE(M >= 0 && M % SCREAM_ROW_TILE == 0, SCREAM_EUNSUPPORTED);
     SCREAM_REQUIRE(((reinterpret_cast<uintptr_t>(Q) | reinterpret_cast<uintptr_t>(kv_image) | reinterpret_cast<uintptr_t>(x) |
@@ -1157,16 +1347,33 @@
                      reinterpret_cast<uintptr_t>(g2) | reinterpret_cast<uintptr_t>(b2) | reinterpret_cast<uintptr_t>(y) |
                      reinterpret_cast<uintptr_t>(q_next)) & 15) == 0, SCREAM_EINVAL);
     SCREAM_REQUIRE(x != y, SCREAM_EINVAL);
+    scream_tail_exps_t ex_c;
+    CoorArgs ca{nullptr, nullptr, nullptr, nullptr, nullptr, nullptr, nullptr};
+    if (coor) {
+        SCREAM_REQUIRE(((reinterpret_cast<uintptr_t>(coor->b0) | reinterpret_cast<uintptr_t>(coor->b2) | reinterpret_cast<uintptr_t>(coor->w4) |
+                         reinterpret_cast<uintptr_t>(coor->b4) | reinterpret_cast<uintptr_t>(coor->src_pred)) & 3) == 0, SCREAM_EINVAL);
+        SCREAM_REQUIRE(coor->e_c2x >= -40 && coor->e_c2x <= 40 && coor->e_c2w >= -40 && coor->e_c2w <= 40, SCREAM_EINVAL);
+        ex_c = coor_exps(*exps, *coor);
+        exps = &ex_c;
+        ca = CoorArgs{coor->b0, coor->b2, coor->w4, coor->b4, coor->src_pred, coor->cloud_row0, coor->cloud_len};
+    }
     SCREAM_REQUIRE(!q_next || (split != SCREAM_SPLIT_BF3 && q_next != x && q_next != y), SCREAM_EINVAL);
-    TailScales sc{1.f, 0, 0, 1.f, 1e-5f, 1.f, 1.f, 1.f, 1e-5f, 1.f, 1.f, 1.f, 1.f};
+    TailScales sc{1.f, 0, 0, 1.f, 1e-5f, 1.f, 1.f, 1.f, 1e-5f, 1.f, 1.f, 1.f, 1.f, 1.f, 1.f};
     if (split != SCREAM_SPLIT_BF3) SCREAM_REQUIRE(tail_scales(exps, &sc), SCREAM_EINVAL);
+    if (coor) {
+        sc.s_c2 = exp2i(coor->e_c2x);
+        sc.cc2 = exp2i(-coor->e_c2x - coor->e_c2w);
+    }
     const int64_t tiles = M / SCREAM_ROW_TILE;
     if (tiles == 0) return 0;
     SCREAM_REQUIRE(tiles < (1ll << 31), SCREAM_EUNSUPPORTED);
     const unsigned grid = tiles < T_MAX_GRID ? (unsigned)tiles : (unsigned)T_MAX_GRID;
     hipStream_t st = as_stream(stream);
-#define TAIL_ARGS grid, st, Q, kv_image, tile_cloud, kv_cloud_offset, cloud_len, x, tail_image, g1, b1, g2, b2, y, q_next, (int)tiles, sc
-    if (split == SCREAM_SPLIT_H2) {
+#define TAIL_ARGS grid, st, Q, kv_image, tile_cloud, kv_cloud_offset, cloud_len, x, tail_image, g1, b1, g2, b2, y, q_next, (int)tiles, sc, ca
+    if (coor) {
+        SCREAM_REQUIRE(scream_detail::launch_tail_coor(split, grid, st, Q, kv_image, tile_cloud, kv_cloud_offset, cloud_len, x, tail_image, g1, b1, g2,
+                                                       b2, y, (int)tiles, &sc, &ca) == 0, SCREAM_EUNSUPPORTED);
+    } else if (split == SCREAM_SPLIT_H2) {
         if (!Q) launch_tail<SplitH2, false, true>(TAIL_ARGS);
         else if (q_next) launch_tail<SplitH2, true>(TAIL_ARGS);
         else launch_tail<SplitH2, false>(TAIL_ARGS);
@@ -1181,6 +1388,25 @@
     SCREAM_LAUNCH_CHECK();
     return 0;
 }
+}
+
+extern "C" int scream_layer_tail_f32(const float* Q, const void* kv_image, const int32_t* tile_cloud,
+                                     int32_t kv_cloud_offset, const int32_t* cloud_len, const float* x,
+                                     const void* tail_image, const float* g1, const float* b1, const float* g2,
+                                     const float* b2, float* y, float* q_next, int64_t M, int32_t split,
+                                     const scream_tail_exps_t* exps, void* stream) {
+    return layer_tail_any(Q, kv_image, tile_cloud, kv_cloud_offset, cloud_len, x, tail_image, g1, b1, g2, b2, y, q_next, nullptr, M, split, exps,
+                          stream);
+}
+
+extern "C" int scream_layer_tail_coor_f32(const float* Q, const void* kv_image, const int32_t* tile_cloud, int32_t kv_cloud_offset,
+                                          const int32_t* cloud_len, const float* x, const void* tail_image, const float* g1, const float* b1,
+                                          const float* g2, const float* b2, float* y, const scream_coor_tail_t* coor, int64_t M,
+                                          int32_t split, const scream_tail_exps_t* exps, void* stream) {
+    SCREAM_REQUIRE(coor, SCREAM_EINVAL);
+    return layer_tail_any(Q, kv_image, tile_cloud, kv_cloud_offset, cloud_len, x, tail_image, g1, b1, g2, b2, y, nullptr, coor, M, split, exps,
+                          stream);
+}
 
 extern "C" int scream_act_layout(const float* src, float* dst, int64_t M, int32_t to_fragment, void* stream) {
     SCREAM_REQUIRE(src && dst && src != dst, SCREAM_EINVAL);
@@ -1191,3 +1417,4 @@
     SCREAM_LAUNCH_CHECK();
     return 0;
 }
+#endif
diff --git a/scream_amd/model.py b/scream_amd/model.py
--- a/scream_amd/model.py
+++ b/scream_amd/model.py
@@ -111,11 +111,13 @@
 
     q_first = os.environ.get("SCREAM_Q_FIRST", "0") == "1"
 
+    coor_tail = os.environ.get("SCREAM_COOR_TAIL", "1") != "0"
+
     def _fused_cfg(self, split) -> bool:
         return bool(split and self.fused_tail)
 
     def _signature(self):
-        return (self.fused_tail, self.batched_cross_kv, self.fuse_next_q, self.ring_proj, self.q_first) + tuple((p.data_ptr(), p._version) for p in self.parameters())
+        return (self.fused_tail, self.batched_cross_kv, self.fuse_next_q, self.ring_proj, self.q_first, self.coor_tail) + tuple((p.data_ptr(), p._version) for p in self.parameters())
 
     def _layer_inputs(self):
         ln = lambda n: (n.weight, n.bias)
@@ -193,6 +195,13 @@
             import warnings
             warnings.warn("scream_amd: q_first is experimental -- its layer-tail kernel is not repeatable bit for bit when other kernels run "
                           "beside it (profiles/r04_qf_experiment.txt); do not use it for results")
+        c0w, c2w = self.coor_mlp[0].weight[:, :, 0], self.coor_mlp[2].weight[:, :, 0]
+        coor = None
+        if fp16_split and self.fused_tail and self.coor_tail and not qf and self.cross_layer_num > 0:
+            coor = _lib.CoorTailT()
+            coor.e_c0x = scales.exp_for(scales.ln_bound(*coor_in))
+            coor.e_c2x = scales.exp_for(scales.lin_bound(c0w, *coor_in, bias=self.coor_mlp[0].bias))
+            coor.e_c0w, coor.e_c2w = scales.w_exp(c0w), scales.w_exp(c2w)
         next_cross = {id(mods[i]): i + 1 for i in range(ns, len(mods) - 1, 2)} if (fp16_split and self.fused_tail and self.fuse_next_q and not qf) else {}
         for L, m, (in_q, in_kv) in list(zip(layers, mods, ins)) + list(zip(tgt_layers, tgt_mods, tgt_ins)):
             k, v = m.k_proj.weight, m.v_proj.weight
@@ -225,7 +234,8 @@
             if split and self.fused_tail:
                 f32 = lambda t: t.detach().to(device=dev, dtype=torch.float32)
                 img = ops.pack_tail(f32(m.merge.weight), f32(m.mlp[0].weight), f32(m.mlp[2].weight), split, L.tail_exps,
-                                    Wq_next=None if wq_next is None else f32(wq_next), Wq_own=f32(m.q_proj.weight) if qf else None)
+                                    Wq_next=None if wq_next is None else f32(wq_next), Wq_own=f32(m.q_proj.weight) if qf else None,
+                                    coor=(f32(c0w), f32(c2w), coor) if coor is not None and m is mods[-1] else None)
                 keep.append(img.data)
                 L.tail = img.data_ptr()
                 L.wm, L.w1, L.w2 = None, None, None
@@ -244,9 +254,11 @@
         mt.layers_host = C.cast(layers, C.POINTER(_lib.LayerT))
         mt.stem_tgt_layers_host = C.cast(tgt_layers, C.POINTER(_lib.LayerT)) if tgt_mods else None
         mt.gemm_split = split
-        c0w, c2w = self.coor_mlp[0].weight[:, :, 0], self.coor_mlp[2].weight[:, :, 0]
-        (mt.c0_w, mt.e_c0w), mt.c0_b = dev_mat(c0w), dev_f32(self.coor_mlp[0].bias)
-        (mt.c2_w, mt.e_c2w), mt.c2_b = dev_mat(c2w), dev_f32(self.coor_mlp[2].bias)
+        if coor is not None:
+            (mt.c0_w, mt.e_c0w), (mt.c2_w, mt.e_c2w) = (None, coor.e_c0w), (None, coor.e_c2w)
+        else:
+            (mt.c0_w, mt.e_c0w), (mt.c2_w, mt.e_c2w) = dev_mat(c0w), dev_mat(c2w)
+        mt.c0_b, mt.c2_b = dev_f32(self.coor_mlp[0].bias), dev_f32(self.coor_mlp[2].bias)
         mt.c4_w, mt.c4_b = dev_f32(self.coor_mlp[4].weight[:, :, 0]), dev_f32(self.coor_mlp[4].bias)
         mt.wkv_cross, mt.proj_cross = None, None
         if self._fused_cfg(split) and self.batched_cross_kv and self.cross_layer_num > 0:
diff --git a/scream_amd/ops.py b/scream_amd/ops.py
--- a/scream_amd/ops.py
+++ b/scream_amd/ops.py
@@ -69,6 +69,7 @@
     exps: _lib.TailExpsT
     next_q: bool = False
     q_first: bool = False
+    coor: bool = False
 
     def data_ptr(self) -> int:
         return self.data.data_ptr()
@@ -133,8 +134,9 @@
 
 def pack_tail(Wm: torch.Tensor, W1: torch.Tensor, W2: torch.Tensor, split: Optional[int] = None,
               exps: Optional[_lib.TailExpsT] = None, Wq_next: Optional[torch.Tensor] = None,
-              Wq_own: Optional[torch.Tensor] = None) -> PackedTail:
+              Wq_own: Optional[torch.Tensor] = None, coor=None) -> PackedTail:
     assert Wq_next is None or Wq_own is None
+    assert coor is None or (Wq_next is None and Wq_own is None)
     q_first = Wq_own is not None
     Wq_next = Wq_own if q_first else Wq_next
     split = default_split() if split is None else split
@@ -144,6 +146,16 @@
         raise ValueError("pack_tail on an fp16 split needs the operand exponents (scream_amd/scales.py)")
     exps = exps if exps is not None else tail_exps()
     lib = _lib.load()
+    if coor is not None:
+        Wc0, Wc2 = (w.detach().to(torch.float32).contiguous() for w in coor[:2])
+        assert Wc0.shape == (D_MODEL, D_MODEL) and Wc2.shape == (D_MODEL, D_MODEL)
+        nbytes = lib.scream_tail_coor_image_bytes(split)
+        if nbytes < 0:
+            raise _lib.ScreamHipError("scream_tail_coor_image_bytes returned %d (the coordinate MLP rides on an fp16 split only)" % nbytes)
+        out = torch.empty(nbytes, device=Wm.device, dtype=torch.uint8)
+        check(lib.scream_pack_tail_coor(_p(Wm), _p(W1), _p(W2), _p(Wc0), _p(Wc2), split, C.byref(exps), C.byref(coor[2]),
+                                        _p(out, torch.uint8), _stream()), "scream_pack_tail_coor")
+        return PackedTail(out, split, exps, coor=True)
     if Wq_next is not None:
         Wq_next = Wq_next.detach().to(torch.float32).contiguous()
         assert Wq_next.shape == (D_MODEL, D_MODEL)
@@ -176,6 +188,7 @@
     assert x.shape[1] == D_MODEL and (Q is None or x.shape == Q.shape)
     assert (Q is None) == tail.q_first, "Q = None goes with an image that carries this layer's own query stages (pack_tail(Wq_own=...))"
     assert (q_next is not None) == tail.next_q, "q_next goes with an image that carries the next layer's query stages"
+    assert not tail.coor, "an image with the coordinate MLP's stages is run by scream_forward (scream_layer_tail_coor_f32)"
     if out is None:
         out = torch.empty(M, D_MODEL, device=x.device, dtype=torch.float32)
     check(_lib.load().scream_layer_tail_f32(_p(Q), _p(kv_image, torch.uint8), _p(tile_cloud, torch.int32),
```

Result: no change. 1873 pairs/s (median of 6 runs) (+0.5%).
